# VeeraKarthick609/ImageCaptioner

Hardware: NVIDIA B200
Metric: kd_train_samples_per_sec (higher is better)
Workload: dtype bf16

## Files before the change

### imagecaptioner_b200/csrc/api.cu

```cuda
#include <stdlib.h>
#include "gemm.cuh"
#include "loss_kernels.cuh"
#include "decoder_kernels.cuh"
#include "recurrent.cuh"
#include "recur_cluster.cuh"
#include "refine_kernels.cuh"
#include "mha_mma.cuh"
#include "optim_kernels.cuh"

using namespace b2c;

namespace {

constexpr int MAXL = B2C_MAX_LAYERS;
constexpr int COLSUM_RS = 160;

int check_device() {
  static int cached = 1;
  if (cached <= 0) return cached;
  int dev = 0;
  B2C_CUDA(cudaGetDevice(&dev));
  int major = 0;
  B2C_CUDA(cudaDeviceGetAttribute(&major, cudaDevAttrComputeCapabilityMajor, dev));
  if (major != 10) { cached = B2C_EARCH; return set_err(B2C_EARCH, "b2c kernels are built for sm_100a only; device has compute capability major %d", major); }
// ... 184 lines not shown
    const int gx = cdiv(cols, 256);
    int rs = (int)((rows + 31) / 32); if (rs > 592 / gx) rs = 592 / gx; if (rs > COLSUM_RS) rs = COLSUM_RS; if (rs < 1) rs = 1;
    colsum_vec_kernel<T, false><<<dim3(gx, rs), 256, 0, st>>>(const_cast<T*>(A), (const T*)nullptr, rows, cols, 1.f, partial);
    B2C_LAUNCH_CHECK("colsum_vec_kernel");
    colsum_final_kernel<<<cdiv(cols, 256), 256, 0, st>>>(partial, rs, cols, out, out2, unperm_h);
    B2C_LAUNCH_CHECK("colsum_final_kernel");
    return 0;
  }
  int rs = (int)((rows + 255) / 256); if (rs > COLSUM_RS) rs = COLSUM_RS; if (rs < 1) rs = 1;
  colsum_partial_kernel<T><<<dim3(cdiv(cols, 32), rs), 256, 0, st>>>(A, rows, cols, ld, partial);
  B2C_LAUNCH_CHECK("colsum_partial_kernel");
  colsum_final_kernel<<<cdiv(cols, 256), 256, 0, st>>>(partial, rs, cols, out, out2, unperm_h);
  B2C_LAUNCH_CHECK("colsum_final_kernel");
  return 0;
}

template <typename K> int set_smem(K kern, size_t bytes) {
  B2C_CHECK_ARG(bytes <= 227 * 1024, "kernel needs %zu bytes of shared memory (> 227 KB): shape too large for this path", bytes);
  if (bytes > 48 * 1024) B2C_CUDA(cudaFuncSetAttribute(kern, cudaFuncAttributeMaxDynamicSharedMemorySize, (int)bytes));
  return 0;
}

template <typename T>
int attn_fwd(cudaStream_t st, const B2CShape& s, const float* P, const T* F, const float* u, T* ctx, long ldctx, float* attw,
             long ldu = 0, float* u_save = nullptr) {
  if (ldu == 0) ldu = s.E;
  const size_t smem = (size_t)s.S * s.E * sizeof(T) + (size_t)(s.E + s.S) * 4;
  const int nq = s.S <= ATT_MAXTOK * (ATT_THREADS / 32) ? cdiv(s.E / 4, 32) : 4;
#define B2C_ATT_(NQ, KA) do { B2C_TRY(set_smem(attn_step_fwd_kernel<T, NQ, KA>, smem)); \
    B2C_CUDA(launch_pdl(attn_step_fwd_kernel<T, NQ, KA>, dim3(s.B), dim3(ATT_THREADS), smem, st, P, F, u, ldu, s.S, s.E, ctx, ldctx, attw, u_save)); } while (0)
  if (nq == 1) B2C_ATT_(1, 4); else if (nq == 2) B2C_ATT_(2, 4); else if (nq == 3) B2C_ATT_(3, ATT_MAXTOK); else B2C_ATT_(0, ATT_MAXTOK);
#undef B2C_ATT_
  B2C_LAUNCH_CHECK("attn_step_fwd_kernel");
  return 0;
}

template <typename T>
int attn_bwd(cudaStream_t st, int B, int S, int E, const float* P, const T* F, const float* u, const float* attw, const float* dctx, long lddctx,
             float* ds, T* du) {
  const size_t smem = (size_t)S * E * sizeof(T) + (size_t)(E + 2 * S) * 4;
  constexpr int PB = 13;
#define B2C_ATTB(PB, SMALL) do { B2C_TRY(set_smem(attn_step_bwd_kernel<T, PB, SMALL>, smem)); \
    B2C_CUDA(launch_pdl(attn_step_bwd_kernel<T, PB, SMALL>, dim3(B), dim3(ATT_THREADS), smem, st, P, F, u, (long)E, attw, dctx, lddctx, S, E, ds, du, (long)E)); } while (0)
  if (E <= 256) B2C_ATTB(PB, true); else B2C_ATTB(PB, false);
#undef B2C_ATTB
  B2C_LAUNCH_CHECK("attn_step_bwd_kernel");
  return 0;
}

template <typename T>
int lstm_layer_fwd(cudaStream_t st, const B2CShape& s, const Weights<T>& w, int k, const T* xh_t, const T* addend,
                   const float* c_prev, float* c_out, T* gates_out, T* h_rec, T* h_next, T* h_top,
                   const B2CDropout& dr, long row_base, const float* rec32 = nullptr, long ld_rec32 = 0) {
  const int in = in_dim(s, k), ld = in + s.H;
  LstmEpi le{};
  le.addend32 = rec32; le.ld_addend32 = ld_rec32;
  le.enabled = 1; le.H = s.H; le.addend = addend; le.bias = (k == 0) ? nullptr : w.bcat[k];
  le.c_prev = c_prev; le.c_out = c_out; le.gates_out = gates_out;
  le.h_rec = h_rec; le.ld_rec = ld; le.h_next = h_next; le.ld_next = 2 * s.H; le.h_top = h_top; le.ld_top = s.H;
  le.drop_p = dr.p; le.seed = dr.seed; le.site = (unsigned)k; le.row_base = row_base; le.seed_dev = (const unsigned long long*)dr.seed_dev;
  return gemm_lstm<T>(st, s.B, s.H, rec32 ? in : ld, xh_t, ld, w.Wcat[k], ld, le);
}

constexpr int MAX_SUB = 5;
struct SubStreams { cudaStream_t s[MAX_SUB]; cudaEvent_t fork; cudaEvent_t join[MAX_SUB]; cudaEvent_t ev[4]; };
constexpr int MAX_DEVICES = 64;
int get_substreams(SubStreams** out) {
  static SubStreams all[MAX_DEVICES]; static bool all_ready[MAX_DEVICES] = {false};
  int dev = 0;
  B2C_CUDA(cudaGetDevice(&dev));
  B2C_CHECK_ARG(dev >= 0 && dev < MAX_DEVICES, "device index %d outside [0,%d)", dev, MAX_DEVICES);
  SubStreams& ss = all[dev]; bool& ready = all_ready[dev];
  if (!ready) {
    for (int i = 0; i < MAX_SUB; ++i) {
      B2C_CUDA(cudaStreamCreateWithFlags(&ss.s[i], cudaStreamNonBlocking));
      B2C_CUDA(cudaEventCreateWithFlags(&ss.join[i], cudaEventDisableTiming));
    }
    B2C_CUDA(cudaEventCreateWithFlags(&ss.fork, cudaEventDisableTiming));
    for (int i = 0; i < 4; ++i) B2C_CUDA(cudaEventCreateWithFlags(&ss.ev[i], cudaEventDisableTiming));
    ready = true;
  }
  *out = &ss;
  return 0;
}
inline int pick_sub_batches(int B) {
  static int want = -1;
  if (want < 0) { const char* e = getenv("B2C_SUB_BATCHES"); want = e ? atoi(e) : 1; if (want != 2 && want != 4) want = 1; }
  if (want > 1 && B >= 32 * want && B % want == 0) return want;
  return 1;
}
struct SubPlan { int ns; cudaStream_t st[MAX_SUB]; int b0[MAX_SUB]; int bn[MAX_SUB]; SubStreams* ss; cudaStream_t main; };
int fork_subs(SubPlan& sp, int B, cudaStream_t st) {
  sp.ns = pick_sub_batches(B); sp.main = st; sp.ss = nullptr;
  if (sp.ns == 1) { sp.st[0] = st; sp.b0[0] = 0; sp.bn[0] = B; return 0; }
  B2C_TRY(get_substreams(&sp.ss));
  B2C_CUDA(cudaEventRecord(sp.ss->fork, st));
  for (int i = 0; i < sp.ns; ++i) {
    sp.st[i] = sp.ss->s[i]; sp.bn[i] = B / sp.ns; sp.b0[i] = i * sp.bn[i];
    B2C_CUDA(cudaStreamWaitEvent(sp.st[i], sp.ss->fork, 0));
  }
  return 0;
}
int join_subs(SubPlan& sp) {
  if (sp.ns == 1) return 0;
  for (int i = 0; i < sp.ns; ++i) {
    B2C_CUDA(cudaEventRecord(sp.ss->join[i], sp.st[i]));
    B2C_CUDA(cudaStreamWaitEvent(sp.main, sp.ss->join[i], 0));
  }
  return 0;
}

struct RecurTrace { unsigned long long* dev; size_t n; int grid, T; };
inline RecurTrace& recur_trace_state() { static RecurTrace t{nullptr, 0, 0, 0}; return t; }
inline unsigned long long* recur_trace_buffer(size_t n) {
  static const bool on = getenv("B2C_RECUR_TRACE") != nullptr;
  if (!on) return nullptr;
  RecurTrace& t = recur_trace_state();
  if (t.n < n) { if (t.dev) cudaFree(t.dev); t.dev = nullptr; if (cudaMalloc(&t.dev, n * 8) != cudaSuccess) { t.n = 0; return nullptr; } t.n = n; }
  return t.dev;
}

template <typename T> int recur_forward(cudaStream_t, const B2CShape&, const RecurPlan&, const TrainWs<T>&, const T*, T*, float*, const B2CDropout&) {
  return set_err(B2C_EINVAL, "the persistent recurrence kernel is bf16 only");
}
template <>
int recur_forward<bf16>(cudaStream_t st, const B2CShape& s, const RecurPlan& pl, const TrainWs<bf16>& W, const bf16* feats, bf16* hid_top, float* attw,
                        const B2CDropout& dr) {
  RecurMaps maps; RecurParams p{};
  p.B = s.B; p.T = s.T; p.S = s.S; p.E = s.E; p.H = s.H; p.L = s.L;
  p.tiles_m = pl.tiles_m; p.tiles_n = pl.tiles_n; p.u_tiles_n = pl.u_tiles_n; p.n_fbuf = pl.n_fbuf; p.f_resident = pl.f_resident; p.tmem_cols = pl.tmem_cols;
  p.P = W.P; p.EP = W.EP; p.F = feats; p.u = W.u; p.attw = attw; p.G0 = W.G0; p.hid_top = hid_top;
  p.trace = recur_trace_buffer((size_t)pl.grid * s.T * 16);
  for (int k = 0; k < s.L; ++k) {
    const int in = in_dim(s, k), ld = in + s.H;
    p.xh[k] = W.xh[k]; p.ld[k] = ld; p.in[k] = in; p.bias[k] = (k == 0) ? nullptr : W.w.bcat[k]; p.c[k] = W.c[k]; p.gates[k] = W.gates[k];
    B2C_TRY(make_tmap_bf16_3d(&maps.a[k], W.xh[k], ld, s.B, s.T + 1, ld, TC_BM));
    B2C_TRY(make_tmap_bf16(&maps.w[k], W.w.Wcat[k], ld, 4 * s.H, ld, RC_BN));
  }
  for (int k = s.L; k < RC_MAXL; ++k) { maps.a[k] = maps.a[0]; maps.w[k] = maps.w[0]; }
  B2C_TRY(make_tmap_bf16(&maps.wh, W.w.Wh, s.H, s.E, s.H, RC_BNU));
  p.drop_p = dr.p; p.seed = dr.seed; p.seed_dev = (const unsigned long long*)dr.seed_dev;
  { const char* e = getenv("B2C_RECUR_EARLY"); p.early = (e && e[0] == '0') ? 0 : 1; }
  { const char* e = getenv("B2C_RECUR_EPNC"); p.ep_nc = (e && e[0] == '1') ? 1 : 0; }
  p.barrier = W.sync; p.flags = W.sync + 128;
  B2C_CHECK_ARG(pl.grid <= 160, "unexpected grid %d", pl.grid);
  B2C_CUDA(cudaMemsetAsync(W.sync, 0, (128 + 160 * 32) * sizeof(unsigned int), st));
  void (*kern)(const RecurMaps, const RecurParams) = pl.nq == 1 ? recur_fwd_kernel<1> : (pl.nq == 2 ? recur_fwd_kernel<2> : recur_fwd_kernel<3>);
  B2C_CUDA(cudaFuncSetAttribute(kern, cudaFuncAttributeMaxDynamicSharedMemorySize, (int)pl.smem));
  cudaLaunchConfig_t cfg{};
  cfg.gridDim = dim3(pl.grid); cfg.blockDim = dim3(RC_THREADS); cfg.dynamicSmemBytes = pl.smem; cfg.stream = st;
  cudaLaunchAttribute attr[1];
  attr[0].id = cudaLaunchAttributeCooperative; attr[0].val.cooperative = 1;
  cfg.attrs = attr; cfg.numAttrs = 1;
  B2C_CUDA(cudaLaunchKernelEx(&cfg, kern, maps, p));
  B2C_LAUNCH_CHECK("recur_fwd_kernel");
  recur_trace_state().grid = pl.grid; recur_trace_state().T = s.T;
  return 0;
}

template <typename T> int cluster_forward(cudaStream_t, const B2CShape&, int, const TrainWs<T>&, const T*, T*, float*) {
  return set_err(B2C_EINVAL, "the cluster recurrence kernel is bf16 only");
}
template <>
int cluster_forward<bf16>(cudaStream_t st, const B2CShape& s, int ncl, const TrainWs<bf16>& W, const bf16* feats, bf16* hid_top, float* attw) {
  ClusterMaps maps; ClusterParams p{};
  p.B = s.B; p.T = s.T; p.S = s.S; p.ncl = ncl;
  p.P = W.P; p.EP = W.EP; p.F = feats; p.u = W.u; p.attw = attw; p.xh0 = W.xh[0]; p.xh1 = W.xh[1];
  p.G0T = W.G0T; p.bias1 = W.w.bcat[1]; p.c0 = W.c[0]; p.c1 = W.c[1]; p.gates0 = W.gates[0]; p.gates1 = W.gates[1]; p.hid_top = hid_top;
  p.trace = recur_trace_buffer((size_t)ncl * CR_CL * s.T * 8);
  const long rows = (long)(s.T + 1) * s.B;
  B2C_TRY(make_tmap_bf16(&maps.w0, W.w.Wcat[0], CR_E + CR_H, 4 * CR_H, CR_E + CR_H, 128));
  B2C_TRY(make_tmap_bf16(&maps.w1, W.w.Wcat[1], 2 * CR_H, 4 * CR_H, 2 * CR_H, 128));
  B2C_TRY(make_tmap_bf16(&maps.wh, W.w.Wh, CR_H, CR_E, CR_H, CR_UCOLS));
  B2C_TRY(make_tmap_bf16(&maps.h0, W.xh[0], CR_E + CR_H, rows, CR_E + CR_H, CR_RMAX));
  B2C_TRY(make_tmap_bf16(&maps.h1, W.xh[1], 2 * CR_H, rows, 2 * CR_H, CR_RMAX));
  B2C_TRY(make_tmap_bf16(&maps.ctx, W.xh[0], CR_E + CR_H, rows, CR_E + CR_H, CR_SPC));
  B2C_CUDA(cudaFuncSetAttribute(recur_cluster_fwd_kernel, cudaFuncAttributeMaxDynamicSharedMemorySize, CR_SMEM_BYTES));
  cudaLaunchConfig_t cfg{};
  cfg.gridDim = dim3(ncl * CR_CL); cfg.blockDim = dim3(CR_THREADS); cfg.dynamicSmemBytes = CR_SMEM_BYTES; cfg.stream = st;
  cudaLaunchAttribute attr[1];
  attr[0].id = cudaLaunchAttributeClusterDimension; attr[0].val.clusterDim.x = CR_CL; attr[0].val.clusterDim.y = 1; attr[0].val.clusterDim.z = 1;
  cfg.attrs = attr; cfg.numAttrs = 1;
  B2C_CUDA(cudaLaunchKernelEx(&cfg, recur_cluster_fwd_kernel, maps, p));
  B2C_LAUNCH_CHECK("recur_cluster_fwd_kernel");
  recur_trace_state().grid = ncl * CR_CL; recur_trace_state().T = s.T;
  return 0;
}

template <typename T>
int decoder_prepare_impl(const B2CShape& s, const B2CParams& p, const int64_t* cap, void* ws, size_t ws_bytes, cudaStream_t st) {
  TrainWs<T> W; W.carve(ws, s);
  B2C_CHECK_ARG(ws_bytes >= W.bytes, "workspace too small: %zu < %zu", ws_bytes, W.bytes);
  const int B = s.B, Tn = s.T, E = s.E, H = s.H, L = s.L, V = s.V;
  const long TB = (long)Tn * B;
  B2C_TRY(pack_params<T>(s, p, W.w, st));
  embedding_gather_kernel<T><<<ew_grid(TB * E / 4), 256, 0, st>>>(p.embedding, cap, TB, E, V, W.emb, E);
  B2C_LAUNCH_CHECK("embedding_gather_kernel");
  for (int k = 0; k < L; ++k) {
    B2C_CUDA(cudaMemsetAsync(W.xh[k], 0, (size_t)B * (in_dim(s, k) + H) * sizeof(T), st));
    B2C_CUDA(cudaMemsetAsync(W.c[k], 0, (size_t)B * H * sizeof(float), st));
  }
  B2C_TRY((gemm<T, T>(st, (int)TB, 4 * H, E, W.emb, E, 0, W.w.We, E, 0, W.G0, 4 * H, 0.f, W.w.bx)));
  if constexpr (sizeof(T) == 2) {
    if (const int ncl = cluster_plan(s)) {
      g0_cluster_layout_kernel<<<dim3(4 * H / 64, ncl, Tn), 256, 0, st>>>(reinterpret_cast<const bf16*>(W.G0), B, Tn, ncl, reinterpret_cast<bf16*>(W.G0T));
      B2C_LAUNCH_CHECK("g0_cluster_layout_kernel");
    }
  }
  return 0;
}

template <typename T>
int set_initial_state_impl(const B2CShape& s, const float* h0, const float* c0, void* ws, size_t ws_bytes, cudaStream_t st) {
  TrainWs<T> W; W.carve(ws, s);
  B2C_CHECK_ARG(ws_bytes >= W.bytes, "workspace too small: %zu < %zu", ws_bytes, W.bytes);
  for (int k = 0; k < s.L; ++k) {
    const int in = in_dim(s, k);
    initial_state_kernel<T><<<ew_grid((long)s.B * s.H), 256, 0, st>>>(h0 + (size_t)k * s.B * s.H, c0 + (size_t)k * s.B * s.H, s.B, s.H,
                                                                     W.xh[k] + in, in + s.H, W.c[k]);
    B2C_LAUNCH_CHECK("initial_state_kernel");
  }
  return 0;
}

struct EvalOut { const float* teacher; const int64_t* targets; float temperature; float* row_kl; float* row_ce; int* argmax; };

template <typename T>
int decoder_forward_impl(const B2CShape& s, const B2CParams& p, const T* feats, const int64_t* cap, T* logits, T* hid_top,
                         float* attw, void* ws, size_t ws_bytes, const B2CDropout& dr, cudaStream_t st, bool prepared,
                         const EvalOut* ev = nullptr) {
  TrainWs<T> W; W.carve(ws, s);
  B2C_CHECK_ARG(ws_bytes >= W.bytes, "workspace too small: %zu < %zu", ws_bytes, W.bytes);
  const int B = s.B, Tn = s.T, S = s.S, E = s.E, H = s.H, L = s.L, V = s.V;
  const long TB = (long)Tn * B;
  if (!prepared) B2C_TRY(decoder_prepare_impl<T>(s, p, cap, ws, ws_bytes, st));
  B2C_TRY((gemm<T, float>(st, B * S, E, E, feats, E, 0, W.w.Wf, E, 0, W.P, E, 0.f, p.attn_b)));
  const int inL = in_dim(s, L - 1), ldL = inL + H;
  SubPlan sp;
  B2C_TRY(fork_subs(sp, B, st));
  pdl_full_dependency_next();
  static const bool merge_rec = []() { const char* e = getenv("B2C_MERGE_REC"); return !(e && e[0] == '0'); }();
  RecurPlan rplan{}; rplan.ok = false;
  int ncl = 0;
  if (sizeof(T) == 2 && sp.ns == 1 && !(dr.p > 0.f)) ncl = cluster_plan(s);
  if (ncl > 0) { B2C_TRY(cluster_forward<T>(st, s, ncl, W, feats, hid_top, attw)); rplan.ok = true; }
  else {
  if (sizeof(T) == 2 && sp.ns == 1) rplan = recur_plan(s);
  if (rplan.ok) B2C_TRY(recur_forward<T>(st, s, rplan, W, feats, hid_top, attw, dr));
  }
  for (int t = 0; t < (rplan.ok ? 0 : Tn); ++t) {
    for (int i = 0; i < sp.ns; ++i) {
      cudaStream_t ss = sp.st[i];
      const long b0 = sp.b0[i];
      B2CShape sh = s; sh.B = sp.bn[i];
      const long row = (long)t * B + b0;
      const T* q = W.xh[L - 1] + row * ldL + inL;
      float* u_t = W.u + row * E;
      const bool merged = merge_rec && sizeof(T) == 2;
      const long ldur = E + 4 * H;
      float* ur = W.UR + b0 * ldur;
      if (merged) {
        B2C_TRY((gemm<T, float>(ss, sh.B, E + 4 * H, H, q, ldL, 0, W.w.Wuh, H, 0, ur, ldur)));
        B2C_TRY(attn_fwd<T>(ss, sh, W.P + b0 * S * E, feats + b0 * S * E, ur, W.xh[0] + row * (E + H), E + H, attw + row * S, ldur, u_t));
      } else {
        B2C_TRY((gemm<T, float>(ss, sh.B, E, H, q, ldL, 0, W.w.Wh, H, 0, u_t, E)));
        B2C_TRY(attn_fwd<T>(ss, sh, W.P + b0 * S * E, feats + b0 * S * E, u_t, W.xh[0] + row * (E + H), E + H, attw + row * S));
      }
      for (int k = 0; k < L; ++k) {
        const int in = in_dim(s, k), ld = in + H;
        const bool rec = merged && k == L - 1;
        B2C_TRY(lstm_layer_fwd<T>(ss, sh, W.w, k, W.xh[k] + row * ld, k == 0 ? W.G0 + row * 4 * H : (const T*)nullptr,
                                  W.c[k] + row * H, W.c[k] + (row + B) * H,
                                  W.gates[k] + row * 4 * H, W.xh[k] + (row + B) * ld + in,
                                  k + 1 < L ? W.xh[k + 1] + row * 2 * H : nullptr, k == L - 1 ? hid_top + row * H : nullptr,
                                  dr, row, rec ? ur + E : nullptr, ldur));
      }
    }
  }
  B2C_TRY(join_subs(sp));
  B2C_TRY((gemm<T, T>(st, (int)TB, E, H, hid_top, H, 0, W.w.W1, H, 0, W.o1, E, 0.f, p.out0_b, 1)));
  if (dr.p > 0.f) {
    dropout_inplace_kernel<T><<<ew_grid(TB * E), 256, 0, st>>>(W.o1, TB * E, dr.p, dr.seed, 100u, (const unsigned long long*)dr.seed_dev);
    B2C_LAUNCH_CHECK("dropout_inplace_kernel");
  }
  if (ev) {
    GemmArgs gv{(int)TB, V, E, 1.f, 0.f, W.o1, (long)E, 0, W.w.W2, (long)E, 0, nullptr, (long)V, p.out3_b, 0};
    B2C_CHECK_ARG(sizeof(T) == 2 && tc_eligible(gv), "the logits-free validation forward needs bf16 mode and a TMA-describable vocabulary head");
    EvalEpi ee{ev->teacher, ev->targets, W.evalp, 1.0f / ev->temperature, 0, 0};
    gv.eval = &ee;
    B2C_TRY((Gemm<T, float>::run(gv, st)));
    kd_eval_combine_kernel<<<cdiv(TB, 8), 256, 0, st>>>(W.evalp, ee.nparts, TB, V, ev->targets, 1.0f / ev->temperature, ev->row_kl, ev->row_ce, ev->argmax);
    B2C_LAUNCH_CHECK("kd_eval_combine_kernel");
    return 0;
  }
  B2C_TRY((gemm<T, T>(st, (int)TB, V, E, W.o1, E, 0, W.w.W2, E, 0, logits, V, 0.f, p.out3_b)));
  return 0;
}



inline int bg_ctas() { static int v = -1; if (v < 0) { const char* e = getenv("B2C_BG_CTAS"); v = e ? atoi(e) : 10; } return v; }
inline bool attn_post_occ3() { static int v = -1; if (v < 0) { const char* e = getenv("B2C_POST_OCC3"); v = (e && e[0] == '0') ? 0 : 1; } return v != 0; }
inline int wgrad_chunks() { static int v = -1; if (v < 0) { const char* e = getenv("B2C_WGRAD_CHUNKS"); v = e ? atoi(e) : 0; } return v; }

template <typename T>
int decoder_backward_impl(const B2CShape& s, const B2CParams& p, const T* feats, const int64_t* cap, const T* hid_top,
                          const float* attw, const T* dlogits, const T* dhid, const B2CGrads& g, float* dfeats,
                          void* ws, size_t ws_bytes, const B2CDropout& dr, cudaStream_t st, int flags) {
  TrainWs<T> W; W.carve(ws, s);
  B2C_CHECK_ARG(ws_bytes >= W.bytes, "workspace too small: %zu < %zu", ws_bytes, W.bytes);
  B2C_CHECK_ARG(g.embedding && g.attn_w && g.attn_b && g.comb_w && g.comb_b && g.out0_w && g.out0_b && g.out3_w && g.out3_b && dfeats, "NULL gradient pointer");
  const int B = s.B, Tn = s.T, S = s.S, E = s.E, H = s.H, L = s.L, V = s.V;
  const long TB = (long)Tn * B;
  const float inv_keep = dr.p > 0.f ? 1.0f / (1.0f - dr.p) : 1.0f;
  SubStreams* hs = nullptr;
  B2C_TRY(get_substreams(&hs));
  cudaStream_t side = hs->s[MAX_SUB - 1];
  for (int k = 0; k < L; ++k) B2C_CHECK_ARG(g.w_ih[k] && g.w_hh[k] && g.b_ih[k] && g.b_hh[k], "NULL LSTM gradient pointer (layer %d)", k);
  B2C_CUDA(cudaEventRecord(hs->ev[3], st));
  B2C_CUDA(cudaStreamWaitEvent(side, hs->ev[3], 0));
  B2C_CUDA(cudaMemsetAsync(W.dxh0, 0, (size_t)TB * (E + H) * sizeof(float), side));
  for (int k = 1; k < L; ++k) B2C_CUDA(cudaMemsetAsync(W.dxh[k], 0, (size_t)TB * 2 * H * sizeof(float), side));
  B2C_CUDA(cudaEventRecord(hs->ev[3], side));
  B2C_TRY((gemm<T, T>(st, (int)TB, E, V, dlogits, V, 0, W.w.W2, E, 1, W.do1, E)));
  relu_bwd_inplace_kernel<T><<<ew_grid(TB * E), 256, 0, st>>>(W.do1, W.o1, TB * E, inv_keep);
  B2C_LAUNCH_CHECK("relu_bwd_inplace_kernel");
  B2C_CUDA(cudaEventRecord(hs->fork, st));
  B2C_CUDA(cudaStreamWaitEvent(side, hs->fork, 0));
  {
    GemmCapScope bg(bg_ctas());
    B2C_TRY((gemm<T, float>(side, V, E, (int)TB, dlogits, V, 1, W.o1, E, 1, g.out3_w, E)));
    B2C_TRY(colsum<T>(side, dlogits, TB, V, V, W.partial_side, g.out3_b));
    B2C_TRY((gemm<T, float>(side, E, H, (int)TB, W.do1, E, 1, hid_top, H, 1, g.out0_w, H)));
    B2C_TRY(colsum<T>(side, W.do1, TB, E, E, W.partial_side, g.out0_b));
  }
  B2C_CUDA(cudaEventRecord(hs->join[MAX_SUB - 1], side));
  B2C_TRY((gemm<T, float>(st, (int)TB, H, E, W.do1, E, 0, W.w.W1, H, 1, W.dHext, H)));
  B2C_CUDA(cudaStreamWaitEvent(st, hs->ev[3], 0));
  SubPlan sp;
  B2C_TRY(fork_subs(sp, B, st));
  auto weight_grads = [&](cudaStream_t s2, long r0, long r1, float beta) -> int {
    const int K = (int)(r1 - r0);
    for (int k = 1; k < L; ++k) {
      const int in = in_dim(s, k), ld = in + H;
      B2C_TRY((gemm<T, float>(s2, 4 * H, in, K, W.dgates[k] + r0 * 4 * H, 4 * H, 1, W.xh[k] + r0 * ld, ld, 1, g.w_ih[k], in, beta, nullptr, 0, 1.f, H)));
      B2C_TRY((gemm<T, float>(s2, 4 * H, H, K, W.dgates[k] + r0 * 4 * H, 4 * H, 1, W.xh[k] + r0 * ld + in, ld, 1, g.w_hh[k], H, beta, nullptr, 0, 1.f, H)));
    }
    B2C_TRY((gemm<T, float>(s2, 4 * H, E, K, W.dgates[0] + r0 * 4 * H, 4 * H, 1, W.xh[0] + r0 * (E + H), E + H, 1, W.dWx32, E, beta)));
    B2C_TRY((gemm<T, float>(s2, 4 * H, E, K, W.dgates[0] + r0 * 4 * H, 4 * H, 1, W.emb + r0 * E, E, 1, W.dWe32, E, beta)));
    B2C_TRY((gemm<T, float>(s2, 4 * H, H, K, W.dgates[0] + r0 * 4 * H, 4 * H, 1, W.xh[0] + r0 * (E + H) + E, E + H, 1, g.w_hh[0], H, beta, nullptr, 0, 1.f, H)));
    return 0;
  };
  const int n_chunks = (sp.ns == 1 && bg_ctas() > 0) ? wgrad_chunks() : 0;
  const int chunk_steps = n_chunks > 0 ? cdiv(Tn, n_chunks) : 0;
  long wg_done_from = TB;
  bool wg_any = false;
  pdl_full_dependency_next();
  for (int t = Tn - 1; t >= 0; --t) {
    const bool last = (t == Tn - 1);
    for (int i = 0; i < sp.ns; ++i) {
      cudaStream_t ss = sp.st[i];
      const long b0 = sp.b0[i];
      const int Bh = sp.bn[i];
      const long row = (long)t * B + b0;
      for (int k = L - 1; k >= 0; --k) {
        const int in = in_dim(s, k), ld = in + H;
        const float* carry = last ? nullptr : (k == 0 ? W.dxh0 + (row + B) * (E + H) + E : W.dxh[k] + (row + B) * 2 * H + H);
        const float* above = (k < L - 1) ? W.dxh[k + 1] + row * 2 * H : nullptr;
        const bool top = (k == L - 1);
        B2C_CUDA(launch_pdl(lstm_pointwise_bwd_kernel<T>, dim3(ew_grid((long)Bh * H)), dim3(256), 0, ss,
            (const T*)(W.gates[k] + row * 4 * H), (const float*)(W.c[k] + row * H), (const float*)(W.c[k] + (row + B) * H), W.dc[k] + b0 * H, last ? 1 : 0,
            carry, (long)ld, above, (long)(2 * H), (const float*)(top ? W.dHext + row * H : nullptr), (const T*)((top && dhid) ? dhid + row * H : nullptr),
            (const T*)((top && !last) ? W.dq + b0 * H : nullptr), (long)H, W.dgates[k] + row * 4 * H, Bh, H, dr.p, dr.seed, (uint32_t)k, row, (const unsigned long long*)dr.seed_dev));
        B2C_LAUNCH_CHECK("lstm_pointwise_bwd_kernel");
        float* out = (k == 0) ? W.dxh0 + row * (E + H) : W.dxh[k] + row * 2 * H;
        B2C_TRY((gemm<T, float>(ss, Bh, ld, 4 * H, W.dgates[k] + row * 4 * H, 4 * H, 0, W.w.Wcat[k], ld, 1, out, ld, 1.f)));
      }
      const float* dctx_t = W.dxh0 + row * (E + H);
      T* du_t = W.du + row * E;
      B2C_TRY(attn_bwd<T>(ss, Bh, S, E, W.P + b0 * S * E, feats + b0 * S * E, W.u + row * E, attw + row * S, dctx_t, (long)(E + H), W.ds + row * S, du_t));
      if (t > 0) B2C_TRY((gemm<T, T>(ss, Bh, H, E, du_t, E, 0, W.w.Wh, H, 1, W.dq + b0 * H, H)));
    }
    if (chunk_steps > 0 && t > 0 && (Tn - t) % chunk_steps == 0 && t >= chunk_steps) {
      B2C_CUDA(cudaEventRecord(hs->ev[0], st));
      B2C_CUDA(cudaStreamWaitEvent(side, hs->ev[0], 0));
      GemmCapScope bg(bg_ctas());
      B2C_TRY(weight_grads(side, (long)t * B, wg_done_from, wg_any ? 1.f : 0.f));
      wg_done_from = (long)t * B; wg_any = true;
    }
  }
  B2C_TRY(join_subs(sp));
  B2C_CUDA(cudaEventRecord(hs->ev[1], st));
  B2C_CUDA(cudaStreamWaitEvent(side, hs->ev[1], 0));
  B2C_TRY(weight_grads(side, 0, wg_done_from, wg_any ? 1.f : 0.f));
  for (int k = 0; k < L; ++k) B2C_TRY(colsum<T>(side, W.dgates[k], TB, 4 * H, 4 * H, W.partial_side, g.b_ih[k], g.b_hh[k], H));
  {
    cast_f32_kernel<T><<<ew_grid((long)4 * H * E / 8), 256, 0, side>>>(W.dWx32, W.dWxT, (long)4 * H * E);
    B2C_LAUNCH_CHECK("cast_f32_kernel");
    cast_f32_kernel<T><<<ew_grid((long)4 * H * E / 8), 256, 0, side>>>(W.dWe32, W.dWeT, (long)4 * H * E);
    B2C_LAUNCH_CHECK("cast_f32_kernel");
    B2C_TRY((gemm<T, float>(side, 4 * H, E, E, W.dWxT, E, 0, W.w.Wcc, E, 0, g.w_ih[0], E, 0.f, nullptr, 0, 1.f, H)));
    B2C_TRY((gemm<T, float>(side, 4 * H, E, E, W.dWeT, E, 0, W.w.Wce, E, 0, g.w_ih[0], E, 1.f, nullptr, 0, 1.f, H)));
    rank1_add_kernel<<<ew_grid((long)4 * H * E), 256, 0, side>>>(g.w_ih[0], g.b_ih[0], p.comb_b, (long)4 * H, E);
    B2C_LAUNCH_CHECK("rank1_add_kernel");
    B2C_TRY((gemm<T, float>(side, E, E, 4 * H, W.w.Wih0, E, 1, W.dWeT, E, 1, g.comb_w, 2 * E)));
    B2C_TRY((gemm<T, float>(side, E, E, 4 * H, W.w.Wih0, E, 1, W.dWxT, E, 1, g.comb_w + E, 2 * E)));
    B2C_CUDA(cudaMemsetAsync(g.comb_b, 0, (size_t)E * sizeof(float), side));
    bias_fold_bwd_kernel<<<dim3(cdiv(E, 32), 32), 256, 0, side>>>(p.w_ih[0], g.b_ih[0], 4 * H, E, g.comb_b);
    B2C_LAUNCH_CHECK("bias_fold_bwd_kernel");
    B2C_TRY((gemm<T, float>(side, (int)TB, E, 4 * H, W.dgates[0], 4 * H, 0, W.w.We, E, 1, W.demb, E)));
    B2C_CUDA(cudaMemsetAsync(g.embedding, 0, (size_t)V * E * sizeof(float), side));
    embedding_scatter_add_kernel<<<ew_grid(TB * E), 256, 0, side>>>(W.demb, cap, TB, E, V, g.embedding);
    B2C_LAUNCH_CHECK("embedding_scatter_add_kernel");
  }
  const int inL = in_dim(s, L - 1), ldL = inL + H;
  B2C_TRY((gemm<T, float>(side, E, H, (int)TB, W.du, E, 1, W.xh[L - 1] + inL, ldL, 1, g.attn_w, H + E)));
  if (Tn <= 24) {
    const int splits = 1, per = cdiv(S, splits), TP = (Tn + 3) & ~3;
    const size_t psmem = (size_t)2 * per * TP * 4;
    if (Tn <= 20 && attn_post_occ3()) {
      B2C_TRY(set_smem(attn_post_reg_kernel<T, 20>, psmem));
      attn_post_reg_kernel<T, 20><<<dim3(B, splits), ATT_THREADS, psmem, st>>>(W.P, W.u, W.dxh0, (long)(E + H), attw, W.ds, Tn, B, S, E, W.dP, dfeats);
    } else {
      B2C_TRY(set_smem(attn_post_reg_kernel<T, 24>, psmem));
      attn_post_reg_kernel<T, 24><<<dim3(B, splits), ATT_THREADS, psmem, st>>>(W.P, W.u, W.dxh0, (long)(E + H), attw, W.ds, Tn, B, S, E, W.dP, dfeats);
    }
    B2C_LAUNCH_CHECK("attn_post_reg_kernel");
  } else {
    const size_t smem = (size_t)Tn * (2 * E + 2 * S) * 4;
    B2C_TRY(set_smem(attn_post_kernel<T>, smem));
    attn_post_kernel<T><<<B, ATT_THREADS, smem, st>>>(W.P, W.u, W.dxh0, (long)(E + H), attw, W.ds, Tn, B, S, E, W.dP, dfeats);
    B2C_LAUNCH_CHECK("attn_post_kernel");
  }
  B2C_CUDA(cudaEventRecord(hs->ev[2], st));
  B2C_TRY((gemm<T, float>(st, B * S, E, E, W.dP, E, 0, W.w.Wf, E, 1, dfeats, E, 1.f)));
  B2C_CUDA(cudaStreamWaitEvent(side, hs->ev[2], 0));
  B2C_TRY((gemm<T, float>(side, E, E, B * S, W.dP, E, 1, feats, E, 1, g.attn_w + H, H + E)));
  B2C_TRY(colsum<T>(side, W.dP, (long)B * S, E, E, W.partial_side, g.attn_b));
  B2C_CUDA(cudaEventRecord(hs->join[MAX_SUB - 1], side));
  if (flags & B2C_BWD_DEFER_JOIN) return 0;
  B2C_CUDA(cudaStreamWaitEvent(st, hs->join[MAX_SUB - 1], 0));
  return 0;
}


inline bool fuse_argmax_off() { static const bool off = getenv("B2C_DECODE_LOGITS") != nullptr; return off; }

template <typename T>
int greedy_decode_impl(const B2CShape& s, const B2CParams& p, const T* feats, int64_t start_id, int64_t end_id,
                       int64_t* tokens, int32_t* lengths, void* ws, size_t ws_bytes, cudaStream_t st) {
  DecodeWs<T> W; W.carve(ws, s);
  B2C_CHECK_ARG(ws_bytes >= W.bytes, "workspace too small: %zu < %zu", ws_bytes, W.bytes);
  const int B = s.B, Tn = s.T, S = s.S, E = s.E, H = s.H, L = s.L, V = s.V;
  const B2CDropout nodrop{0.f, 0, nullptr};
  B2C_TRY(pack_params<T>(s, p, W.w, st));
  B2C_TRY((gemm<T, float>(st, B * S, E, E, feats, E, 0, W.w.Wf, E, 0, W.P, E, 0.f, p.attn_b)));
  for (int k = 0; k < L; ++k) {
    B2C_CUDA(cudaMemsetAsync(W.xh[k], 0, (size_t)2 * B * (in_dim(s, k) + H) * sizeof(T), st));
    B2C_CUDA(cudaMemsetAsync(W.c[k], 0, (size_t)B * H * sizeof(float), st));
  }
  fill_i64_kernel<<<ew_grid(B), 256, 0, st>>>(W.cur, B, start_id);
  B2C_LAUNCH_CHECK("fill_i64_kernel");
  const int inL = in_dim(s, L - 1), ldL = inL + H;
  for (int t = 0; t < Tn; ++t) {
    const int pcur = t & 1, pnxt = pcur ^ 1;
    auto slot = [&](int k, int which) { return W.xh[k] + (size_t)which * B * (in_dim(s, k) + H); };
    embedding_gather_kernel<T><<<ew_grid((long)B * E / 4), 256, 0, st>>>(p.embedding, W.cur, B, E, V, W.emb, E);
    B2C_LAUNCH_CHECK("embedding_gather_kernel");
    B2C_TRY((gemm<T, T>(st, B, 4 * H, E, W.emb, E, 0, W.w.We, E, 0, W.G0, 4 * H, 0.f, W.w.bx)));
    B2C_TRY((gemm<T, float>(st, B, E, H, slot(L - 1, pcur) + inL, ldL, 0, W.w.Wh, H, 0, W.u, E)));
    B2C_TRY(attn_fwd<T>(st, s, W.P, feats, W.u, slot(0, pcur), E + H, nullptr));
    for (int k = 0; k < L; ++k) {
      const int in = in_dim(s, k);
      B2C_TRY(lstm_layer_fwd<T>(st, s, W.w, k, slot(k, pcur), k == 0 ? W.G0 : (const T*)nullptr, W.c[k], W.c[k], (T*)nullptr, slot(k, pnxt) + in,
                                k + 1 < L ? slot(k + 1, pcur) : nullptr, (T*)nullptr, nodrop, 0));
    }
    B2C_TRY((gemm<T, T>(st, B, E, H, slot(L - 1, pnxt) + inL, ldL, 0, W.w.W1, H, 0, W.o1, E, 0.f, p.out0_b, 1)));
    GemmArgs gv{B, V, E, 1.f, 0.f, W.o1, (long)E, 0, W.w.W2, (long)E, 0, W.logits, (long)V, p.out3_b, 0};
    if (sizeof(T) == 2 && tc_eligible(gv) && !fuse_argmax_off()) {
      ArgmaxEpi ae{W.amax_v, W.amax_i, 0, 0};
      gv.amax = &ae;
      B2C_TRY((Gemm<T, float>::run(gv, st)));
      argmax_parts_feedback_kernel<<<cdiv(B, 8), 256, 0, st>>>(W.amax_v, W.amax_i, ae.nparts, B, end_id, t, W.cur, tokens + (long)t * B, lengths, W.done);
      B2C_LAUNCH_CHECK("argmax_parts_feedback_kernel");
    } else {
      B2C_TRY((Gemm<T, float>::run(gv, st)));
      argmax_feedback_kernel<<<B, 256, 0, st>>>(W.logits, V, V, end_id, t, W.cur, tokens + (long)t * B, lengths, W.done);
      B2C_LAUNCH_CHECK("argmax_feedback_kernel");
    }
  }
  finish_lengths_kernel<<<cdiv(B, 256), 256, 0, st>>>(lengths, B, Tn);
  B2C_LAUNCH_CHECK("finish_lengths_kernel");
  return 0;
}


template <typename T> struct AttnWs {
  T *Wh, *Wf; float *P, *u; size_t bytes;
  void carve(void* base, const B2CShape& s) {
    Carver c{reinterpret_cast<unsigned char*>(base), 0};
    Wh = c.take<T>((size_t)s.E * s.H); Wf = c.take<T>((size_t)s.E * s.E);
    P = c.take<float>((size_t)s.B * s.S * s.E); u = c.take<float>((size_t)s.B * s.E);
    bytes = align_up(c.off, 256);
  }
};

template <typename T>
int attention_step_impl(const B2CShape& s, const float* attn_w, const float* attn_b, const T* hidden, const T* feats,
                        T* context, float* weights, void* ws, size_t ws_bytes, cudaStream_t st) {
  AttnWs<T> W; W.carve(ws, s);
  B2C_CHECK_ARG(ws_bytes >= W.bytes, "workspace too small: %zu < %zu", ws_bytes, W.bytes);
  const int B = s.B, S = s.S, E = s.E, H = s.H;
  PackTable tab; tab.n = 2;
  tab.seg[0] = PackSeg{attn_w, W.Wh, nullptr, E, H, (long)H + E, (long)H, 0};
  tab.seg[1] = PackSeg{attn_w + H, W.Wf, nullptr, E, E, (long)H + E, (long)E, 0};
  pack_params_kernel<T><<<dim3(32, 2), 256, 0, st>>>(tab);
  B2C_LAUNCH_CHECK("pack_params_kernel");
  B2C_TRY((gemm<T, float>(st, B * S, E, E, feats, E, 0, W.Wf, E, 0, W.P, E, 0.f, attn_b)));
  pdl_full_dependency_next();
  B2C_TRY((gemm<T, float>(st, B, E, H, hidden, H, 0, W.Wh, H, 0, W.u, E)));
  return attn_fwd<T>(st, s, W.P, feats, W.u, context, (long)s.E, weights);
}

constexpr int LN_GRID = 148 * 3;
template <typename T> struct RefineWs {
  T *Win, *Wo, *W1, *W2;
  T *x, *qkv, *probs, *attn, *proj, *x1, *f1, *f2;
  float *mean1, *rstd1, *mean2, *rstd2;
  T *dz2, *df1, *dz1, *dattn, *dqkv; float *dz1f, *lnpart, *partial;
  float *x1f, *dz2f;
  size_t bytes;
  void carve(void* base, const B2CShape& s) {
    Carver c{reinterpret_cast<unsigned char*>(base), 0};
    const size_t R = (size_t)s.B * s.S, E = s.E, heads = s.H;
    Win = c.take<T>(3 * E * E); Wo = c.take<T>(E * E); W1 = c.take<T>(2 * E * E); W2 = c.take<T>(2 * E * E);
    x = c.take<T>(R * E); qkv = c.take<T>(R * 3 * E); probs = c.take<T>((size_t)s.B * heads * s.S * (s.S > 64 ? s.S : 64)) ; attn = c.take<T>(R * E);
    proj = c.take<T>(R * E); x1 = c.take<T>(R * E); f1 = c.take<T>(R * 2 * E); f2 = c.take<T>(R * E);
    mean1 = c.take<float>(R); rstd1 = c.take<float>(R); mean2 = c.take<float>(R); rstd2 = c.take<float>(R);
    dz2 = c.take<T>(R * E); df1 = c.take<T>(R * 2 * E); dz1 = c.take<T>(R * E); dattn = c.take<T>(R * E); dqkv = c.take<T>(R * 3 * E);
    dz1f = c.take<float>(R * E); lnpart = c.take<float>((size_t)LN_GRID * 3 * E); partial = c.take<float>((size_t)COLSUM_RS * 3 * E);
    x1f = c.take<float>(R * E); dz2f = c.take<float>(R * E);
    bytes = align_up(c.off, 256);
  }
};

int check_refine_shape(const B2CShape* s) {
  B2C_CHECK_ARG(s != nullptr, "shape is NULL");
  B2C_CHECK_ARG(s->B > 0 && s->S > 0 && s->E > 0 && s->H > 0, "bad refinement shape B=%d S=%d E=%d heads=%d", s->B, s->S, s->E, s->H);
  B2C_CHECK_ARG(s->E % 8 == 0 && s->E <= 256 * LN_MAXC && s->E % s->H == 0, "E=%d must be a multiple of 8 and of heads=%d, and <= %d", s->E, s->H, 256 * LN_MAXC);
  const size_t hd = s->E / s->H;
  B2C_CHECK_ARG(hd % 4 == 0, "head_dim=%zu must be a multiple of 4", hd);
  B2C_CHECK_ARG((4 * (size_t)s->S * mha_pitch((int)hd) + 3 * (size_t)s->S * mha_pitch(s->S)) * 4 <= 200 * 1024, "S=%d x head_dim=%zu does not fit the attention core's shared memory", s->S, hd);
  return 0;
}

template <typename TX, typename TR, typename TY>
int ln_fwd(cudaStream_t st, const TX* x, const TR* res, const float* g, const float* b, TY* y, float* y32, float* mean, float* rstd, long R, int E) {
  long grid = (R + 7) / 8; if (grid > 148 * 8) grid = 148 * 8;
  if (E <= 256) ln_fwd_kernel<TX, TR, TY, 1><<<(unsigned)grid, LN_THREADS, 0, st>>>(x, res, g, b, y, y32, mean, rstd, R, E, 1e-5f);
  else ln_fwd_kernel<TX, TR, TY, 2><<<(unsigned)grid, LN_THREADS, 0, st>>>(x, res, g, b, y, y32, mean, rstd, R, E, 1e-5f);
  B2C_LAUNCH_CHECK("ln_fwd_kernel");
  return 0;
}
template <typename TX, typename TR, typename TDY, typename TDZ>
int ln_bwd(cudaStream_t st, const TDY* dy, const float* dpool, int L, int O, const TX* x, const TR* res, const float* mean, const float* rstd,
           const float* gamma, TDZ* dz, float* dz32, float* part, float* dgamma, float* dbeta, float* dbias_prev, long R, int E) {
  long grid = (R + 7) / 8; if (grid > LN_GRID) grid = LN_GRID;
  const size_t smem = (size_t)(LN_THREADS / 32) * 3 * E * 4;
#define B2C_LNB(POOLED, NC) do { B2C_TRY(set_smem(ln_bwd_kernel<TX, TR, TDY, TDZ, POOLED, NC>, smem)); \
    ln_bwd_kernel<TX, TR, TDY, TDZ, POOLED, NC><<<(unsigned)grid, LN_THREADS, smem, st>>>(dy, dpool, L, O, x, res, mean, rstd, gamma, dz, dz32, part, R, E); } while (0)
  if (dpool) { if (E <= 256) B2C_LNB(true, 1); else B2C_LNB(true, 2); }
  else { if (E <= 256) B2C_LNB(false, 1); else B2C_LNB(false, 2); }
#undef B2C_LNB
  B2C_LAUNCH_CHECK("ln_bwd_kernel");
  ln_param_grad_kernel<<<dim3(cdiv(E, 32), 3), 256, 0, st>>>(part, (int)grid, E, dgamma, dbeta, dbias_prev);
  B2C_LAUNCH_CHECK("ln_param_grad_kernel");
  return 0;
}

template <typename T>
int colsum_vec(cudaStream_t st, T* A, const T* act, long rows, int cols, float inv_keep, float* partial, float* out) {
  const int gx = cdiv(cols, 256);
  int rs = (int)((rows + 31) / 32); if (rs > 592 / gx) rs = 592 / gx; if (rs > COLSUM_RS) rs = COLSUM_RS; if (rs < 1) rs = 1;
  dim3 grid(gx, rs);
  if (act) colsum_vec_kernel<T, true><<<grid, 256, 0, st>>>(A, act, rows, cols, inv_keep, partial);
  else colsum_vec_kernel<T, false><<<grid, 256, 0, st>>>(A, act, rows, cols, inv_keep, partial);
  B2C_LAUNCH_CHECK("colsum_vec_kernel");
  colsum_final_kernel<<<cdiv(cols, 256), 256, 0, st>>>(partial, rs, cols, out, nullptr);
  B2C_LAUNCH_CHECK("colsum_final_kernel");
  return 0;
}

template <typename T>
int refine_pack(const B2CShape& s, const B2CRefineParams& p, const RefineWs<T>& W, cudaStream_t st) {
  B2C_CHECK_ARG(p.in_w && p.in_b && p.out_w && p.out_b && p.ffn0_w && p.ffn0_b && p.ffn3_w && p.ffn3_b && p.n1_w && p.n1_b && p.n2_w && p.n2_b, "NULL refinement parameter");
  const int E = s.E;
  PackTable tab; tab.n = 4;
  tab.seg[0] = PackSeg{p.in_w, W.Win, nullptr, 3 * E, E, (long)E, (long)E, 0};
  tab.seg[1] = PackSeg{p.out_w, W.Wo, nullptr, E, E, (long)E, (long)E, 0};
  tab.seg[2] = PackSeg{p.ffn0_w, W.W1, nullptr, 2 * E, E, (long)E, (long)E, 0};
  tab.seg[3] = PackSeg{p.ffn3_w, W.W2, nullptr, E, 2 * E, (long)2 * E, (long)2 * E, 0};
  pack_params_kernel<T><<<dim3(48, 4), 256, 0, st>>>(tab);
  B2C_LAUNCH_CHECK("pack_params_kernel");
  return 0;
}

template <typename T> inline bool mha_use_mma(int S, int hd) { return false; }
template <> inline bool mha_use_mma<bf16>(int S, int hd) {
  static const bool off = getenv("B2C_MHA_FFMA") != nullptr;
  return !off && hd == 64 && S <= 64;
}

template <typename T>
int refinement_forward_impl(const B2CShape& s, const B2CRefineParams& p, const float* x, float* out, void* ws, size_t ws_bytes,
                            const B2CDropout& dr, cudaStream_t st, T* out_compute = nullptr) {
  RefineWs<T> W; W.carve(ws, s);
  B2C_CHECK_ARG(ws_bytes >= W.bytes, "workspace too small: %zu < %zu", ws_bytes, W.bytes);
  const int B = s.B, S = s.S, E = s.E, heads = s.H, hd = E / heads;
  const long R = (long)B * S;
  B2C_TRY(refine_pack<T>(s, p, W, st));
  cast_f32_kernel<T><<<ew_grid(R * E / 4), 256, 0, st>>>(x, W.x, R * E);
  B2C_LAUNCH_CHECK("cast_f32_kernel");
  B2C_TRY((gemm<T, T>(st, (int)R, 3 * E, E, W.x, E, 0, W.Win, E, 0, W.qkv, 3 * E, 0.f, p.in_b)));
  if (mha_use_mma<T>(S, hd)) {
    mha_fwd_mma_kernel<<<dim3(B, heads), MM_THREADS, 0, st>>>((const bf16*)W.qkv, (bf16*)W.attn, (bf16*)W.probs, S, E, heads, 1.0f / sqrtf((float)hd),
                                                             dr.p, dr.seed, MHA_DROP_SITE, (const unsigned long long*)dr.seed_dev);
    B2C_LAUNCH_CHECK("mha_fwd_mma_kernel");
  } else {
    const size_t smem = ((size_t)3 * S * mha_pitch(hd) + (size_t)S * mha_pitch(S)) * 4;
    B2C_TRY(set_smem(mha_fwd_kernel<T>, smem));
    mha_fwd_kernel<T><<<dim3(B, heads), MHA_THREADS, smem, st>>>(W.qkv, W.attn, W.probs, S, E, heads, 1.0f / sqrtf((float)hd), dr.p, dr.seed, (const unsigned long long*)dr.seed_dev);
    B2C_LAUNCH_CHECK("mha_fwd_kernel");
  }
  B2C_TRY((gemm<T, T>(st, (int)R, E, E, W.attn, E, 0, W.Wo, E, 0, W.proj, E, 0.f, p.out_b)));
  B2C_TRY((ln_fwd<float, T, T>(st, x, W.proj, p.n1_w, p.n1_b, W.x1, W.x1f, W.mean1, W.rstd1, R, E)));
  B2C_TRY((gemm<T, T>(st, (int)R, 2 * E, E, W.x1, E, 0, W.W1, E, 0, W.f1, 2 * E, 0.f, p.ffn0_b, 1)));
  if (dr.p > 0.f) {
    dropout_inplace_kernel<T><<<ew_grid(R * 2 * E), 256, 0, st>>>(W.f1, R * 2 * E, dr.p, dr.seed, 201u, (const unsigned long long*)dr.seed_dev);
    B2C_LAUNCH_CHECK("dropout_inplace_kernel");
  }
  B2C_TRY((gemm<T, T>(st, (int)R, E, 2 * E, W.f1, 2 * E, 0, W.W2, 2 * E, 0, W.f2, E, 0.f, p.ffn3_b)));
  if (out_compute) B2C_TRY((ln_fwd<float, T, T>(st, W.x1f, W.f2, p.n2_w, p.n2_b, out_compute, out, W.mean2, W.rstd2, R, E)));
  else B2C_TRY((ln_fwd<float, T, float>(st, W.x1f, W.f2, p.n2_w, p.n2_b, (float*)nullptr, out, W.mean2, W.rstd2, R, E)));
  return 0;
}

template <typename T>
int refinement_backward_impl(const B2CShape& s, const B2CRefineParams& p, const float* x, const float* dout, const B2CRefineGrads& g, float* dx,
                             void* ws, size_t ws_bytes, const B2CDropout& dr, cudaStream_t st) {
  RefineWs<T> W; W.carve(ws, s);
  B2C_CHECK_ARG(ws_bytes >= W.bytes, "workspace too small: %zu < %zu", ws_bytes, W.bytes);
  B2C_CHECK_ARG(g.in_w && g.in_b && g.out_w && g.out_b && g.ffn0_w && g.ffn0_b && g.ffn3_w && g.ffn3_b && g.n1_w && g.n1_b && g.n2_w && g.n2_b && dx, "NULL refinement gradient");
  const int B = s.B, S = s.S, E = s.E, heads = s.H, hd = E / heads;
  const long R = (long)B * S;
  const float inv_keep = dr.p > 0.f ? 1.0f / (1.0f - dr.p) : 1.0f;
  B2C_TRY((ln_bwd<float, T, float, T>(st, dout, nullptr, 0, 0, W.x1f, W.f2, W.mean2, W.rstd2, p.n2_w, W.dz2, W.dz2f, W.lnpart, g.n2_w, g.n2_b, g.ffn3_b, R, E)));
  B2C_TRY((gemm<T, float>(st, E, 2 * E, (int)R, W.dz2, E, 1, W.f1, 2 * E, 1, g.ffn3_w, 2 * E)));
  B2C_TRY((gemm<T, T>(st, (int)R, 2 * E, E, W.dz2, E, 0, W.W2, 2 * E, 1, W.df1, 2 * E)));
  B2C_TRY(colsum_vec<T>(st, W.df1, W.f1, R, 2 * E, inv_keep, W.partial, g.ffn0_b));
  B2C_TRY((gemm<T, float>(st, 2 * E, E, (int)R, W.df1, 2 * E, 1, W.x1, E, 1, g.ffn0_w, E)));
  B2C_TRY((gemm<T, float>(st, (int)R, E, 2 * E, W.df1, 2 * E, 0, W.W1, E, 1, W.dz2f, E, 1.f)));
  B2C_TRY((ln_bwd<float, T, float, T>(st, W.dz2f, nullptr, 0, 0, x, W.proj, W.mean1, W.rstd1, p.n1_w, W.dz1, W.dz1f, W.lnpart, g.n1_w, g.n1_b, g.out_b, R, E)));
  B2C_TRY((gemm<T, float>(st, E, E, (int)R, W.dz1, E, 1, W.attn, E, 1, g.out_w, E)));
  B2C_TRY((gemm<T, T>(st, (int)R, E, E, W.dz1, E, 0, W.Wo, E, 1, W.dattn, E)));
  if (mha_use_mma<T>(S, hd)) {
    const size_t smem = (size_t)(dr.p > 0.f ? 7 : 6) * MM_TILE * sizeof(bf16);
    B2C_TRY(set_smem(mha_bwd_mma_kernel, smem));
    mha_bwd_mma_kernel<<<dim3(B, heads), MM_THREADS, smem, st>>>((const bf16*)W.qkv, (const bf16*)W.probs, (const bf16*)W.dattn, (bf16*)W.dqkv, S, E, heads,
                                                                1.0f / sqrtf((float)hd), dr.p, dr.seed, MHA_DROP_SITE, (const unsigned long long*)dr.seed_dev);
    B2C_LAUNCH_CHECK("mha_bwd_mma_kernel");
  } else {
    const size_t smem = ((size_t)4 * S * mha_pitch(hd) + (size_t)(dr.p > 0.f ? 3 : 2) * S * mha_pitch(S)) * 4;
    B2C_TRY(set_smem(mha_bwd_kernel<T>, smem));
    mha_bwd_kernel<T><<<dim3(B, heads), MHA_THREADS, smem, st>>>(W.qkv, W.probs, W.dattn, W.dqkv, S, E, heads, 1.0f / sqrtf((float)hd), dr.p, dr.seed, (const unsigned long long*)dr.seed_dev);
    B2C_LAUNCH_CHECK("mha_bwd_kernel");
  }
  B2C_TRY((gemm<T, float>(st, 3 * E, E, (int)R, W.dqkv, 3 * E, 1, W.x, E, 1, g.in_w, E)));
  B2C_TRY(colsum_vec<T>(st, W.dqkv, (const T*)nullptr, R, 3 * E, 1.f, W.partial, g.in_b));
  B2C_CUDA(cudaMemcpyAsync(dx, W.dz1f, (size_t)R * E * sizeof(float), cudaMemcpyDeviceToDevice, st));
  B2C_TRY((gemm<T, float>(st, (int)R, E, 3 * E, W.dqkv, 3 * E, 0, W.Win, E, 1, dx, E, 1.f)));
  return 0;
}

template <typename T> struct ProjWs {
// ... 479 lines not shown
```

### imagecaptioner_b200/csrc/common.cuh

```cuda
#pragma once
#include <cuda_runtime.h>
#include <cuda_bf16.h>
#include <cuda.h>
#include <stdint.h>
#include <stdio.h>
#include <string.h>
#include <math.h>
#include <stdarg.h>
#include <stdlib.h>

#include "../../include/b2c.h"

namespace b2c {

typedef __nv_bfloat16 bf16;

inline char* err_buf() { static thread_local char buf[512] = {0}; return buf; }
inline int set_err(int code, const char* fmt, ...) {
  va_list ap; va_start(ap, fmt); vsnprintf(err_buf(), 512, fmt, ap); va_end(ap); return code;
}
#define B2C_CHECK_ARG(cond, ...) do { if (!(cond)) return b2c::set_err(B2C_EINVAL, __VA_ARGS__); } while (0)
#define B2C_CUDA(expr) do { cudaError_t e_ = (expr); if (e_ != cudaSuccess) \
    return b2c::set_err(B2C_ECUDA, "%s failed: %s (%s:%d)", #expr, cudaGetErrorString(e_), __FILE__, __LINE__); } while (0)
inline unsigned long long& launch_counter() { static unsigned long long n = 0; return n; }
#define B2C_LAUNCH_CHECK(name) do { ++b2c::launch_counter(); cudaError_t e_ = cudaGetLastError(); if (e_ != cudaSuccess) \
    return b2c::set_err(B2C_ECUDA, "launch of %s failed: %s (%s:%d)", name, cudaGetErrorString(e_), __FILE__, __LINE__); } while (0)
#define B2C_TRY(expr) do { int r_ = (expr); if (r_ != 0) return r_; } while (0)

template <typename T> __device__ __forceinline__ float to_f(T v);
template <> __device__ __forceinline__ float to_f<float>(float v) { return v; }
template <> __device__ __forceinline__ float to_f<bf16>(bf16 v) { return __bfloat162float(v); }
template <typename T> __device__ __forceinline__ T from_f(float v);
template <> __device__ __forceinline__ float from_f<float>(float v) { return v; }
template <> __device__ __forceinline__ bf16 from_f<bf16>(float v) { return __float2bfloat16_rn(v); }

template <typename T> struct Math;
template <> struct Math<float> {
  static __device__ __forceinline__ float tanh_(float x) { return tanhf(x); }
  static __device__ __forceinline__ float sigmoid_(float x) { return 1.0f / (1.0f + expf(-x)); }
  static __device__ __forceinline__ float exp_(float x) { return expf(x); }
  static __device__ __forceinline__ float log_(float x) { return logf(x); }
  static __device__ __forceinline__ float dtanh_(float x) { const float t = tanhf(x); return fmaf(-t, t, 1.0f); }
};
__device__ __forceinline__ float ex2_ftz_(float x) { float y; asm("ex2.approx.ftz.f32 %0, %1;" : "=f"(y) : "f"(x)); return y; }
__device__ __forceinline__ float rcp_ftz_(float x) { float y; asm("rcp.approx.ftz.f32 %0, %1;" : "=f"(y) : "f"(x)); return y; }
template <> struct Math<bf16> {
  static __device__ __forceinline__ float tanh_(float x) { return fmaf(-2.0f, rcp_ftz_(1.0f + ex2_ftz_(2.8853900817779268f * x)), 1.0f); }
  static __device__ __forceinline__ float sigmoid_(float x) { return rcp_ftz_(1.0f + ex2_ftz_(-1.4426950408889634f * x)); }
  static __device__ __forceinline__ float exp_(float x) { return ex2_ftz_(1.4426950408889634f * x); }
  static __device__ __forceinline__ float log_(float x) { return __logf(x); }
  static __device__ __forceinline__ float dtanh_(float x) { float t; asm("tanh.approx.f32 %0, %1;" : "=f"(t) : "f"(x)); return fmaf(-t, t, 1.0f); }
};

__device__ __forceinline__ float ex2_ftz(float x) { float y; asm("ex2.approx.ftz.f32 %0, %1;" : "=f"(y) : "f"(x)); return y; }

__device__ __forceinline__ float warp_sum(float v) {
#pragma unroll
  for (int o = 16; o > 0; o >>= 1) v += __shfl_xor_sync(0xffffffffu, v, o);
  return v;
}
__device__ __forceinline__ float warp_max(float v) {
#pragma unroll
  for (int o = 16; o > 0; o >>= 1) v = fmaxf(v, __shfl_xor_sync(0xffffffffu, v, o));
  return v;
}

__device__ __forceinline__ uint32_t mix32(uint64_t seed, uint32_t stream, uint64_t idx) {
  uint64_t z = seed + 0x9E3779B97F4A7C15ull * (idx + 1) + ((uint64_t)stream << 40);
  z = (z ^ (z >> 30)) * 0xBF58476D1CE4E5B9ull;
  z = (z ^ (z >> 27)) * 0x94D049BB133111EBull;
  z = z ^ (z >> 31);
  return (uint32_t)(z >> 32);
}
__device__ __forceinline__ uint64_t drop_seed(uint64_t seed, const unsigned long long* seed_dev) {
  return seed_dev ? seed + 0xD6E8FEB86659FD93ull * __ldg(seed_dev) : seed;
}
__device__ __forceinline__ float dropout_scale(uint64_t seed, uint32_t stream, uint64_t idx, float p, float inv_keep) {
  const uint32_t thr = (uint32_t)(p * 4294967296.0f);
  return mix32(seed, stream, idx) >= thr ? inv_keep : 0.0f;
}

__device__ __forceinline__ void pdl_launch_dependents() { asm volatile("griddepcontrol.launch_dependents;" ::: "memory"); }
__device__ __forceinline__ void pdl_wait() { asm volatile("griddepcontrol.wait;" ::: "memory"); }

inline bool pdl_enabled() {
  static int on = -1;
  if (on < 0) { const char* e = getenv("B2C_PDL"); on = (e && e[0] == '0') ? 0 : 1; }
  return on != 0;
}
inline bool& pdl_full_dependency_flag() { static thread_local bool f = false; return f; }
inline void pdl_full_dependency_next() { pdl_full_dependency_flag() = true; }
template <typename... KArgs, typename... Args>
inline cudaError_t launch_pdl(void (*kern)(KArgs...), dim3 grid, dim3 block, size_t smem, cudaStream_t st, Args... args) {
  cudaLaunchConfig_t cfg{};
  cfg.gridDim = grid; cfg.blockDim = block; cfg.dynamicSmemBytes = smem; cfg.stream = st;
  cudaLaunchAttribute attr[1];
  attr[0].id = cudaLaunchAttributeProgrammaticStreamSerialization;
  attr[0].val.programmaticStreamSerializationAllowed = 1;
  cfg.attrs = attr; cfg.numAttrs = (pdl_enabled() && !pdl_full_dependency_flag()) ? 1 : 0;
  pdl_full_dependency_flag() = false;
  return cudaLaunchKernelEx(&cfg, kern, static_cast<KArgs>(args)...);
}

__device__ __forceinline__ uint32_t smem_u32(const void* p) { return (uint32_t)__cvta_generic_to_shared(p); }

__device__ __forceinline__ void mbar_init(uint64_t* bar, uint32_t count) {
  asm volatile("mbarrier.init.shared::cta.b64 [%0], %1;" :: "r"(smem_u32(bar)), "r"(count) : "memory");
}
__device__ __forceinline__ void fence_barrier_init() {
  asm volatile("fence.mbarrier_init.release.cluster;" ::: "memory");
}
__device__ __forceinline__ void fence_proxy_async() {
  asm volatile("fence.proxy.async.shared::cta;" ::: "memory");
}
__device__ __forceinline__ void mbar_arrive_expect_tx(uint64_t* bar, uint32_t bytes) {
  asm volatile("mbarrier.arrive.expect_tx.shared::cta.b64 _, [%0], %1;" :: "r"(smem_u32(bar)), "r"(bytes) : "memory");
}
__device__ __forceinline__ void mbar_arrive(uint64_t* bar) {
  asm volatile("mbarrier.arrive.shared::cta.b64 _, [%0];" :: "r"(smem_u32(bar)) : "memory");
}
__device__ __forceinline__ bool mbar_try_wait(uint64_t* bar, uint32_t parity) {
  uint32_t ok;
  asm volatile(
      "{\n\t.reg .pred p;\n\t"
      "mbarrier.try_wait.parity.shared::cta.b64 p, [%1], %2;\n\t"
      "selp.u32 %0, 1, 0, p;\n\t}"
      : "=r"(ok) : "r"(smem_u32(bar)), "r"(parity) : "memory");
  return ok != 0;
}
__device__ __forceinline__ void mbar_wait(uint64_t* bar, uint32_t parity) {
  for (uint32_t spins = 0; !mbar_try_wait(bar, parity); ++spins) {
    if (spins > (1u << 24)) { printf("b2c: mbarrier wait timed out (block %d,%d thread %d)\n", blockIdx.x, blockIdx.y, threadIdx.x); __trap(); }
  }
}
__device__ __forceinline__ void bulk_g2s(void* smem_dst, const void* gsrc, uint32_t bytes, uint64_t* bar) {
  asm volatile("cp.async.bulk.shared::cluster.global.mbarrier::complete_tx::bytes [%0], [%1], %2, [%3];"
               :: "r"(smem_u32(smem_dst)), "l"(gsrc), "r"(bytes), "r"(smem_u32(bar)) : "memory");
}

__device__ __forceinline__ uint4 ld_nc_v4(const void* p) {
  uint4 r;
  asm volatile("ld.global.nc.L1::no_allocate.v4.u32 {%0,%1,%2,%3}, [%4];" : "=r"(r.x), "=r"(r.y), "=r"(r.z), "=r"(r.w) : "l"(p));
  return r;
}
__device__ __forceinline__ void st_na_v4(void* p, const uint4& v) {
  asm volatile("st.global.L1::no_allocate.v4.u32 [%0], {%1,%2,%3,%4};" :: "l"(p), "r"(v.x), "r"(v.y), "r"(v.z), "r"(v.w) : "memory");
}

__device__ __forceinline__ float bf16_lo(uint32_t u) { return __uint_as_float(u << 16); }
__device__ __forceinline__ float bf16_hi(uint32_t u) { return __uint_as_float(u & 0xffff0000u); }
__device__ __forceinline__ uint32_t pack_bf16(float a, float b) {
  __nv_bfloat162 v = __floats2bfloat162_rn(a, b);
  return *reinterpret_cast<uint32_t*>(&v);
}

template <typename T> struct Vec8;
template <> struct Vec8<bf16> {
  static __device__ __forceinline__ void load(const bf16* p, float (&v)[8]) {
    const uint4 a = *reinterpret_cast<const uint4*>(p);
    v[0] = bf16_lo(a.x); v[1] = bf16_hi(a.x); v[2] = bf16_lo(a.y); v[3] = bf16_hi(a.y);
    v[4] = bf16_lo(a.z); v[5] = bf16_hi(a.z); v[6] = bf16_lo(a.w); v[7] = bf16_hi(a.w);
  }
  static __device__ __forceinline__ void store(bf16* p, const float (&v)[8]) {
    *reinterpret_cast<uint4*>(p) = make_uint4(pack_bf16(v[0], v[1]), pack_bf16(v[2], v[3]), pack_bf16(v[4], v[5]), pack_bf16(v[6], v[7]));
  }
};
template <> struct Vec8<float> {
  static __device__ __forceinline__ void load(const float* p, float (&v)[8]) {
    const float4 a = *reinterpret_cast<const float4*>(p), b = *reinterpret_cast<const float4*>(p + 4);
    v[0] = a.x; v[1] = a.y; v[2] = a.z; v[3] = a.w; v[4] = b.x; v[5] = b.y; v[6] = b.z; v[7] = b.w;
  }
  static __device__ __forceinline__ void store(float* p, const float (&v)[8]) {
    *reinterpret_cast<float4*>(p) = make_float4(v[0], v[1], v[2], v[3]);
    *reinterpret_cast<float4*>(p + 4) = make_float4(v[4], v[5], v[6], v[7]);
  }
};


inline int cdiv(long a, long b) { return (int)((a + b - 1) / b); }
__host__ __device__ inline size_t align_up(size_t x, size_t a) { return (x + a - 1) / a * a; }

}
```

### imagecaptioner_b200/csrc/decoder_kernels.cuh

```cuda
#pragma once
#include "common.cuh"

namespace b2c {

__device__ __forceinline__ void divmod_idx(long i, int d, long& q, int& r) {
  if (i < 0x7fffffffL) { const unsigned qi = (unsigned)i / (unsigned)d; q = (long)qi; r = (int)((unsigned)i - qi * (unsigned)d); }
  else { q = i / d; r = (int)(i - q * d); }
}
struct PackSeg {
  const float* src; void* dst;
  const float* src2;
  int rows, cols; long lds, ldd;
  int as_float;
  int perm_h;
};
constexpr int PACK_MAX_SEGS = 20;
struct PackTable { PackSeg seg[PACK_MAX_SEGS]; int n; };

template <typename T>
__global__ void __launch_bounds__(256) pack_params_kernel(const __grid_constant__ PackTable tab) {
  const PackSeg& s = tab.seg[blockIdx.y];
  const long total = (long)s.rows * s.cols;
  if (!s.src2 && !s.as_float && (s.cols & 3) == 0 && (s.lds & 3) == 0 && (s.ldd & 3) == 0 && (((uintptr_t)s.src) & 15) == 0 &&
      (((uintptr_t)s.dst) & 15) == 0) {
// ... 105 lines not shown
  for (int e = tid; e < E; e += ATT_THREADS) { const float uv = __ldcg(u + (long)b * ldu + e); us[e] = uv; if (u_save) u_save[(long)b * E + e] = uv; }
  __syncthreads();
  auto score = [&](const float4 (&pv)[NQR], int l) {
    float a = 0.f;
#pragma unroll
    for (int j = 0; j < NQR; ++j) {
      const int q = lane + j * 32;
      if (q < E4) {
        const float4 p = pv[j];
        const float4 uu = *reinterpret_cast<const float4*>(us + q * 4);
        a += Math<T>::tanh_(p.x + uu.x) + Math<T>::tanh_(p.y + uu.y) + Math<T>::tanh_(p.z + uu.z) + Math<T>::tanh_(p.w + uu.w);
      }
    }
    a = warp_sum(a);
    if (lane == 0) sc[l] = a;
  };
  if constexpr (fast) {
    float4 pb[KB][NQR];
    if (KA < ATT_MAXTOK) {
#pragma unroll
      for (int k = 0; k < KB; ++k) {
        const int l = warp + (KA + k) * nwarp;
#pragma unroll
        for (int j = 0; j < NQR; ++j) {
          const int q = lane + j * 32;
          if (l < S && q < E4) pb[k][j] = __ldg(Pb + l * E4 + q);
        }
      }
    }
#pragma unroll
    for (int k = 0; k < KA; ++k) { const int l = warp + k * nwarp; if (l < S) score(pa[k], l); }
    if (KA < ATT_MAXTOK) {
#pragma unroll
      for (int k = 0; k < KB; ++k) { const int l = warp + (KA + k) * nwarp; if (l < S) score(pb[k], l); }
    }
  } else if constexpr (!fast) {
    for (int l = warp; l < S; l += nwarp) {
      float a = 0.f;
      for (int q = lane; q < E4; q += 32) {
        const float4 p = __ldg(Pb + l * E4 + q);
        const float4 uu = *reinterpret_cast<const float4*>(us + q * 4);
        a += Math<T>::tanh_(p.x + uu.x) + Math<T>::tanh_(p.y + uu.y) + Math<T>::tanh_(p.z + uu.z) + Math<T>::tanh_(p.w + uu.w);
      }
      a = warp_sum(a);
      if (lane == 0) sc[l] = a;
    }
  }
  __syncthreads();
  if (warp == 0) {
    float m = -INFINITY;
    for (int l = lane; l < S; l += 32) m = fmaxf(m, sc[l]);
    m = warp_max(m);
    float s = 0.f;
    for (int l = lane; l < S; l += 32) { const float e = Math<T>::exp_(sc[l] - m); sc[l] = e; s += e; }
    s = warp_sum(s);
    const float inv = 1.0f / s;
    for (int l = lane; l < S; l += 32) { const float wv = sc[l] * inv; sc[l] = wv; if (attw) attw[(long)b * S + l] = wv; }
  }
  __syncthreads();
  mbar_wait(&bar, 0);
  for (int e = tid; e < E; e += ATT_THREADS) {
    float a = 0.f;
    for (int l = 0; l < S; ++l) a = fmaf(sc[l], to_f<T>(Fs[l * E + e]), a);
    ctx[(long)b * ldctx + e] = from_f<T>(a);
  }
}

template <typename T, int PB, bool E256 = false>
__global__ void __launch_bounds__(ATT_THREADS, 4)
attn_step_bwd_kernel(const float* __restrict__ P, const T* __restrict__ F, const float* __restrict__ u, long ldu,
                     const float* __restrict__ attw, const float* __restrict__ dctx, long lddctx,
                     int S, int E, float* __restrict__ ds_out, T* __restrict__ du, long lddu) {
  extern __shared__ __align__(128) unsigned char att_smem[];
  const int SE = S * E;
  T* Fs = reinterpret_cast<T*>(att_smem);
  float* dcs = reinterpret_cast<float*>(Fs + SE);
  float* dw = dcs + E;
  float* ws = dw + S;
  __shared__ __align__(8) uint64_t bar;
  const int tid = threadIdx.x, lane = tid & 31, warp = tid >> 5, nwarp = ATT_THREADS / 32;
  const int b = blockIdx.x;
  const float* Pb = P + (long)b * SE;
  pdl_launch_dependents();
  if (tid == 0) { mbar_init(&bar, 1); fence_barrier_init(); }
  for (int l = tid; l < S; l += ATT_THREADS) ws[l] = attw[(long)b * S + l];
  float cur[PB];
  float ue0 = 0.f;
  if (tid < E) {
    ue0 = u[(long)b * ldu + tid];
#pragma unroll
    for (int i = 0; i < PB; ++i) if (i < S) cur[i] = __ldg(Pb + (long)i * E + tid);
  }
  __syncthreads();
  if (tid == 0) {
    const uint32_t fb = (uint32_t)(SE * sizeof(T));
    mbar_arrive_expect_tx(&bar, fb);
    bulk_g2s(Fs, F + (long)b * SE, fb, &bar);
  }
  pdl_wait();
  for (int e = tid; e < E; e += ATT_THREADS) dcs[e] = __ldcg(dctx + (long)b * lddctx + e);
  __syncthreads();
  mbar_wait(&bar, 0);
  if (E256 || E <= 256) {
    float d[8];
    const int c = lane * 8;
    const bool on = c < E;
    if (on) Vec8<float>::load(dcs + c, d);
    for (int l = warp; l < S; l += nwarp) {
      float a = 0.f;
      if (on) {
        float f[8];
        Vec8<T>::load(Fs + l * E + c, f);
#pragma unroll
        for (int i = 0; i < 8; ++i) a = fmaf(d[i], f[i], a);
      }
      a = warp_sum(a);
      if (lane == 0) dw[l] = a;
    }
  } else if constexpr (!E256) {
    for (int l = warp; l < S; l += nwarp) {
      float a = 0.f;
      for (int c = lane * 8; c < E; c += 256) {
        float f[8], d[8];
        Vec8<T>::load(Fs + l * E + c, f);
        Vec8<float>::load(dcs + c, d);
#pragma unroll
        for (int i = 0; i < 8; ++i) a = fmaf(d[i], f[i], a);
      }
      a = warp_sum(a);
      if (lane == 0) dw[l] = a;
    }
  }
  __syncthreads();
  if (warp == 0) {
    float dot = 0.f;
    for (int l = lane; l < S; l += 32) dot = fmaf(ws[l], dw[l], dot);
    dot = warp_sum(dot);
    for (int l = lane; l < S; l += 32) { const float v = ws[l] * (dw[l] - dot); dw[l] = v; ds_out[(long)b * S + l] = v; }
  }
  __syncthreads();
  for (int e = tid; e < E; e += ATT_THREADS) {
    float ue = ue0;
    if (e != tid) {
      ue = u[(long)b * ldu + e];
#pragma unroll
      for (int i = 0; i < PB; ++i) if (i < S) cur[i] = __ldg(Pb + (long)i * E + e);
    }
    float a = 0.f;
    for (int l0 = 0; l0 < S; l0 += PB) {
      float nxt[PB];
      if (l0 + PB < S) {
#pragma unroll
        for (int i = 0; i < PB; ++i) if (l0 + PB + i < S) nxt[i] = __ldg(Pb + (long)(l0 + PB + i) * E + e);
      }
#pragma unroll
      for (int i = 0; i < PB; ++i) {
        if (l0 + i < S) a = fmaf(dw[l0 + i], Math<T>::dtanh_(cur[i] + ue), a);
      }
#pragma unroll
      for (int i = 0; i < PB; ++i) cur[i] = nxt[i];
    }
    du[(long)b * lddu + e] = from_f<T>(a);
  }
}

template <typename T>
__global__ void __launch_bounds__(ATT_THREADS)
attn_post_kernel(const float* __restrict__ P, const float* __restrict__ u , const float* __restrict__ dctx , long lddctx,
                 const float* __restrict__ attw , const float* __restrict__ ds ,
                 int Tn, int B, int S, int E, T* __restrict__ dP, float* __restrict__ dF) {
  extern __shared__ __align__(128) unsigned char att_smem[];
  float* us = reinterpret_cast<float*>(att_smem);
  float* dcs = us + (long)Tn * E;
  float* ws = dcs + (long)Tn * E;
  float* dss = ws + (long)Tn * S;
  const int tid = threadIdx.x, b = blockIdx.x;
  for (int i = tid; i < Tn * E; i += ATT_THREADS) { const int t = i / E, e = i - t * E; us[i] = u[((long)t * B + b) * E + e]; dcs[i] = dctx[((long)t * B + b) * lddctx + e]; }
  for (int i = tid; i < Tn * S; i += ATT_THREADS) { const int t = i / S, l = i - t * S; ws[i] = attw[((long)t * B + b) * S + l]; dss[i] = ds[((long)t * B + b) * S + l]; }
  __syncthreads();
  const long base = (long)b * S * E;
  for (int idx = tid; idx < S * E; idx += ATT_THREADS) {
    const int l = idx / E, e = idx - l * E;
    const float p = P[base + idx];
    float aP = 0.f, aF = 0.f;
    for (int t = 0; t < Tn; ++t) {
      aP = fmaf(dss[t * S + l], Math<T>::dtanh_(p + us[t * E + e]), aP);
      aF = fmaf(ws[t * S + l], dcs[t * E + e], aF);
    }
    dP[base + idx] = from_f<T>(aP);
    dF[base + idx] = aF;
  }
}

template <typename T, int TMAX>
__global__ void __launch_bounds__(ATT_THREADS, TMAX <= 20 ? 4 : 2)
attn_post_reg_kernel(const float* __restrict__ P, const float* __restrict__ u , const float* __restrict__ dctx , long lddctx,
                     const float* __restrict__ attw , const float* __restrict__ ds ,
                     int Tn, int B, int S, int E, T* __restrict__ dP, float* __restrict__ dF) {
  extern __shared__ __align__(128) unsigned char att_smem[];
  const int tid = threadIdx.x, b = blockIdx.x;
  const int per = (S + gridDim.y - 1) / gridDim.y, l0 = blockIdx.y * per, l1 = min(S, l0 + per), nl = l1 - l0;
  if (nl <= 0) return;
  const int TP = (Tn + 3) & ~3;
  float* dsT = reinterpret_cast<float*>(att_smem);
  float* wT = dsT + per * TP;
  for (int i = tid; i < nl * TP; i += ATT_THREADS) {
    const int ll = i / TP, t = i - ll * TP;
    const long g = ((long)t * B + b) * S + l0 + ll;
    dsT[i] = t < Tn ? ds[g] : 0.f;
    wT[i] = t < Tn ? attw[g] : 0.f;
  }
  __syncthreads();
  const long base = (long)b * S * E;
  for (int e = tid; e < E; e += ATT_THREADS) {
    float ur[TMAX], dcr[TMAX];
#pragma unroll
    for (int t = 0; t < TMAX; ++t) {
      ur[t] = t < Tn ? u[((long)t * B + b) * E + e] : 0.f;
      dcr[t] = t < Tn ? dctx[((long)t * B + b) * lddctx + e] : 0.f;
    }
    float p_next = P[base + (long)l0 * E + e];
#pragma unroll 1
    for (int l = l0; l < l1; ++l) {
      const float p = p_next;
      if (l + 1 < l1) p_next = P[base + (long)(l + 1) * E + e];
      const float4* d4p = reinterpret_cast<const float4*>(dsT + (l - l0) * TP);
      const float4* w4p = reinterpret_cast<const float4*>(wT + (l - l0) * TP);
      float aP = 0.f, aF = 0.f;
#pragma unroll
      for (int t4 = 0; t4 < TMAX; t4 += 4) {
        if (t4 < TP) {
          const float4 d4 = d4p[t4 >> 2], w4 = w4p[t4 >> 2];
          const float dd[4] = {d4.x, d4.y, d4.z, d4.w}, ww[4] = {w4.x, w4.y, w4.z, w4.w};
#pragma unroll
          for (int j = 0; j < 4; ++j) {
            aP = fmaf(dd[j], Math<T>::dtanh_(p + ur[t4 + j]), aP);
            aF = fmaf(ww[j], dcr[t4 + j], aF);
          }
        }
      }
      dP[base + (long)l * E + e] = from_f<T>(aP);
      dF[base + (long)l * E + e] = aF;
    }
  }
}

__global__ void __launch_bounds__(256)
bias_fold_kernel(const float* __restrict__ w_ih0, const float* __restrict__ b_c, const float* __restrict__ b_ih, const float* __restrict__ b_hh,
                 int H, int E, float* __restrict__ bx) {
  const int warp = (blockIdx.x * blockDim.x + threadIdx.x) >> 5, lane = threadIdx.x & 31;
  if (warp >= 4 * H) return;
  const int src = (warp & 3) * H + (warp >> 2);
  float a = 0.f;
  for (int e = lane; e < E; e += 32) a = fmaf(w_ih0[(long)src * E + e], b_c[e], a);
  a = warp_sum(a);
  if (lane == 0) bx[warp] = a + b_ih[src] + b_hh[src];
}
__global__ void __launch_bounds__(256)
bias_fold_bwd_kernel(const float* __restrict__ w_ih0, const float* __restrict__ dbx, int H4, int E, float* __restrict__ db_c) {
  __shared__ float red[8][33];
  const int tx = threadIdx.x & 31, ty = threadIdx.x >> 5, e = blockIdx.x * 32 + tx;
  const int per = (H4 + gridDim.y - 1) / gridDim.y, n0 = blockIdx.y * per, n1 = min(H4, n0 + per);
  float a = 0.f;
  if (e < E) for (int n = n0 + ty; n < n1; n += 8) a = fmaf(w_ih0[(long)n * E + e], dbx[n], a);
  red[ty][tx] = a;
  __syncthreads();
  if (ty == 0 && e < E) { float s = 0.f; for (int i = 0; i < 8; ++i) s += red[i][tx]; atomicAdd(db_c + e, s); }
}
__global__ void __launch_bounds__(256)
rank1_add_kernel(float* __restrict__ dW, const float* __restrict__ dbx, const float* __restrict__ b_c, long rows, int E) {
  for (long i = (long)blockIdx.x * blockDim.x + threadIdx.x; i < rows * E; i += (long)gridDim.x * blockDim.x) {
    long n; int e; divmod_idx(i, E, n, e);
    dW[i] = fmaf(dbx[n], b_c[e], dW[i]);
  }
}

template <typename T> struct Gate4;
template <> struct Gate4<bf16> {
  static __device__ __forceinline__ void load(const bf16* p, float (&v)[4]) {
    const uint2 a = *reinterpret_cast<const uint2*>(p);
    v[0] = bf16_lo(a.x); v[1] = bf16_hi(a.x); v[2] = bf16_lo(a.y); v[3] = bf16_hi(a.y);
  }
  static __device__ __forceinline__ void store(bf16* p, const float (&v)[4]) {
    *reinterpret_cast<uint2*>(p) = make_uint2(pack_bf16(v[0], v[1]), pack_bf16(v[2], v[3]));
  }
};
template <> struct Gate4<float> {
  static __device__ __forceinline__ void load(const float* p, float (&v)[4]) {
    const float4 a = *reinterpret_cast<const float4*>(p); v[0] = a.x; v[1] = a.y; v[2] = a.z; v[3] = a.w;
  }
  static __device__ __forceinline__ void store(float* p, const float (&v)[4]) { *reinterpret_cast<float4*>(p) = make_float4(v[0], v[1], v[2], v[3]); }
};

template <typename T>
__global__ void __launch_bounds__(256)
lstm_pointwise_bwd_kernel(const T* __restrict__ gates, const float* __restrict__ c_prev, const float* __restrict__ c_cur,
                          float* __restrict__ dc, int dc_is_zero,
                          const float* __restrict__ dh_carry, long ld_carry, const float* __restrict__ dh_above, long ld_above,
                          const float* __restrict__ dh_ext, const T* __restrict__ dh_hid, const T* __restrict__ dh_q, long ld_q,
                          T* __restrict__ dgates, int B, int H, float drop_p, uint64_t seed, uint32_t site, long row_base,
                          const unsigned long long* __restrict__ seed_dev) {
  pdl_launch_dependents();
  if (drop_p > 0.f) seed = drop_seed(seed, seed_dev);
  const long total = (long)B * H;
  const float inv_keep = drop_p > 0.f ? 1.0f / (1.0f - drop_p) : 1.0f;
  struct Saved { float gt[4]; float tc, cp, dh_fixed, mask; };
  auto load_saved = [&](long idx, Saved& sv) {
    const long b = (long)((unsigned)idx / (unsigned)H); const int j = (int)(idx - b * H);
    Gate4<T>::load(gates + b * 4 * H + 4 * j, sv.gt);
    sv.tc = Math<T>::tanh_(c_cur[idx]);
    sv.cp = c_prev[idx];
    float d = 0.f;
    if (dh_ext) d += dh_ext[idx];
    if (dh_hid) d += to_f<T>(dh_hid[idx]);
    sv.dh_fixed = d;
    sv.mask = (dh_above && drop_p > 0.f) ? dropout_scale(seed, site, (uint64_t)((row_base + b) * H + j), drop_p, inv_keep) : 1.0f;
  };
  const long idx0 = (long)blockIdx.x * blockDim.x + threadIdx.x;
  Saved sv;
  if (idx0 < total) load_saved(idx0, sv);
  pdl_wait();
  for (long idx = idx0; idx < total; idx += (long)gridDim.x * blockDim.x) {
    if (idx != idx0) load_saved(idx, sv);
    const long b = (long)((unsigned)idx / (unsigned)H); const int j = (int)(idx - b * H);
    float dh = sv.dh_fixed;
    if (dh_carry) dh += __ldcg(dh_carry + b * ld_carry + j);
    if (dh_above) dh += __ldcg(dh_above + b * ld_above + j) * sv.mask;
    if (dh_q) dh += to_f<T>(dh_q[b * ld_q + j]);
    const float i = sv.gt[0], f = sv.gt[1], g = sv.gt[2], o = sv.gt[3], tc = sv.tc;
    const float dcc = (dc_is_zero ? 0.f : __ldcg(dc + idx)) + dh * o * (1.0f - tc * tc);
    const float dg[4] = {dcc * g * i * (1.0f - i), dcc * sv.cp * f * (1.0f - f), dcc * i * (1.0f - g * g), dh * tc * o * (1.0f - o)};
    Gate4<T>::store(dgates + b * 4 * H + 4 * j, dg);
    dc[idx] = dcc * f;
  }
}

template <typename T>
__global__ void __launch_bounds__(256) dropout_inplace_kernel(T* __restrict__ x, long n, float p, uint64_t seed, uint32_t site,
                                                              const unsigned long long* __restrict__ seed_dev) {
  seed = drop_seed(seed, seed_dev);
  const float inv_keep = 1.0f / (1.0f - p);
  const long n8 = (((uintptr_t)x) & 15) == 0 ? (n >> 3) : 0;
  for (long i = (long)blockIdx.x * blockDim.x + threadIdx.x; i < n8; i += (long)gridDim.x * blockDim.x) {
    float v[8];
    Vec8<T>::load(x + i * 8, v);
#pragma unroll
    for (int j = 0; j < 8; ++j) v[j] *= dropout_scale(seed, site, (uint64_t)(i * 8 + j), p, inv_keep);
    Vec8<T>::store(x + i * 8, v);
  }
  for (long i = n8 * 8 + (long)blockIdx.x * blockDim.x + threadIdx.x; i < n; i += (long)gridDim.x * blockDim.x)
    x[i] = from_f<T>(to_f<T>(x[i]) * dropout_scale(seed, site, (uint64_t)i, p, inv_keep));
}
template <typename T>
__global__ void __launch_bounds__(256) relu_bwd_inplace_kernel(T* __restrict__ d, const T* __restrict__ act, long n, float inv_keep) {
  const long n8 = ((((uintptr_t)d) & 15) == 0 && (((uintptr_t)act) & 15) == 0) ? (n >> 3) : 0;
  for (long i = (long)blockIdx.x * blockDim.x + threadIdx.x; i < n8; i += (long)gridDim.x * blockDim.x) {
    float dv[8], av[8];
    Vec8<T>::load(d + i * 8, dv); Vec8<T>::load(act + i * 8, av);
#pragma unroll
    for (int j = 0; j < 8; ++j) dv[j] = av[j] > 0.f ? dv[j] * inv_keep : 0.f;
    Vec8<T>::store(d + i * 8, dv);
  }
  for (long i = n8 * 8 + (long)blockIdx.x * blockDim.x + threadIdx.x; i < n; i += (long)gridDim.x * blockDim.x)
    d[i] = from_f<T>(to_f<T>(act[i]) > 0.f ? to_f<T>(d[i]) * inv_keep : 0.f);
}

template <typename T>
__global__ void __launch_bounds__(256) colsum_partial_kernel(const T* __restrict__ A, long rows, int cols, long ld, float* __restrict__ partial) {
  __shared__ float red[8][33];
  const int tx = threadIdx.x & 31, ty = threadIdx.x >> 5;
  const int col = blockIdx.x * 32 + tx;
  const long per = (rows + gridDim.y - 1) / gridDim.y;
  const long r0 = (long)blockIdx.y * per, r1 = (r0 + per < rows) ? r0 + per : rows;
  float a = 0.f;
  if (col < cols) for (long r = r0 + ty; r < r1; r += 8) a += to_f<T>(A[r * ld + col]);
  red[ty][tx] = a;
  __syncthreads();
  if (ty == 0 && col < cols) {
    float s = 0.f;
#pragma unroll
    for (int i = 0; i < 8; ++i) s += red[i][tx];
    partial[(long)blockIdx.y * cols + col] = s;
  }
}
__global__ void __launch_bounds__(256) colsum_final_kernel(const float* __restrict__ partial, int RS, int cols, float* __restrict__ out, float* __restrict__ out2,
                                                           int unperm_h = 0) {
  const int col = blockIdx.x * blockDim.x + threadIdx.x;
  if (col >= cols) return;
  float s = 0.f;
  for (int r = 0; r < RS; ++r) s += partial[(long)r * cols + col];
  const int oc = unperm_h ? (col & 3) * unperm_h + (col >> 2) : col;
  out[oc] = s;
  if (out2) out2[oc] = s;
}

__global__ void __launch_bounds__(256)
argmax_feedback_kernel(const float* __restrict__ logits, int V, long ld, int64_t end_id, int t,
                       int64_t* __restrict__ cur_tok, int64_t* __restrict__ tokens_t, int32_t* __restrict__ lengths, int32_t* __restrict__ done) {
  __shared__ float bv[8]; __shared__ int bi[8];
  const int b = blockIdx.x, tid = threadIdx.x, lane = tid & 31, warp = tid >> 5;
  const float* row = logits + (long)b * ld;
  float best = -INFINITY; int besti = 0x7fffffff;
  for (int v = tid; v < V; v += 256) { const float x = row[v]; if (x > best || (x == best && v < besti)) { best = x; besti = v; } }
#pragma unroll
  for (int o = 16; o > 0; o >>= 1) {
    const float ob = __shfl_xor_sync(0xffffffffu, best, o); const int oi = __shfl_xor_sync(0xffffffffu, besti, o);
    if (ob > best || (ob == best && oi < besti)) { best = ob; besti = oi; }
  }
  if (lane == 0) { bv[warp] = best; bi[warp] = besti; }
  __syncthreads();
  if (tid == 0) {
    for (int i = 1; i < 8; ++i) if (bv[i] > best || (bv[i] == best && bi[i] < besti)) { best = bv[i]; besti = bi[i]; }
    if (besti == 0x7fffffff) besti = 0;
    cur_tok[b] = besti; tokens_t[b] = besti;
    if (t == 0) { done[b] = 0; lengths[b] = -1; }
    if (besti == end_id && !done[b]) { done[b] = 1; lengths[b] = t; }
  }
}
__global__ void __launch_bounds__(256)
argmax_parts_feedback_kernel(const float* __restrict__ pmax, const int* __restrict__ pidx, int nparts, int B, int64_t end_id, int t,
                             int64_t* __restrict__ cur_tok, int64_t* __restrict__ tokens_t, int32_t* __restrict__ lengths, int32_t* __restrict__ done) {
  const int b = blockIdx.x * (blockDim.x >> 5) + (threadIdx.x >> 5), lane = threadIdx.x & 31;
  if (b >= B) return;
  float best = -INFINITY; int besti = 0x7fffffff;
  for (int p = lane; p < nparts; p += 32) {
    const float x = pmax[(long)b * nparts + p]; const int i = pidx[(long)b * nparts + p];
    if (x > best || (x == best && i < besti)) { best = x; besti = i; }
  }
#pragma unroll
  for (int o = 16; o > 0; o >>= 1) {
    const float ob = __shfl_xor_sync(0xffffffffu, best, o); const int oi = __shfl_xor_sync(0xffffffffu, besti, o);
    if (ob > best || (ob == best && oi < besti)) { best = ob; besti = oi; }
  }
  if (lane == 0) {
    if (besti == 0x7fffffff) besti = 0;
    cur_tok[b] = besti; tokens_t[b] = besti;
    if (t == 0) { done[b] = 0; lengths[b] = -1; }
    if (besti == end_id && !done[b]) { done[b] = 1; lengths[b] = t; }
  }
}
__global__ void bump_counter_kernel(unsigned long long* c) { *c += 1ull; }
__global__ void fill_i64_kernel(int64_t* p, long n, int64_t v) { for (long i = (long)blockIdx.x * blockDim.x + threadIdx.x; i < n; i += (long)gridDim.x * blockDim.x) p[i] = v; }
__global__ void finish_lengths_kernel(int32_t* lengths, int B, int T) { const int b = blockIdx.x * blockDim.x + threadIdx.x; if (b < B && lengths[b] < 0) lengths[b] = T; }

}
```

### imagecaptioner_b200/csrc/gemm.cuh

```cuda
#pragma once
#include "common.cuh"

namespace b2c {

struct LstmEpi {
  int enabled, H;
  const void* addend;
  const float* bias;
  const float* c_prev; float* c_out;
  void* gates_out;
  void* h_rec; long ld_rec; void* h_next; long ld_next; void* h_top; long ld_top;
  float drop_p; unsigned long long seed; unsigned int site; long row_base;
  const unsigned long long* seed_dev;
  const float* addend32; long ld_addend32;
};

constexpr int EVAL_PART_FLOATS = 8;
struct EvalEpi { const float* teacher; const int64_t* targets; float* parts; float inv_temp; int nparts; int cols_per_part; };

struct ArgmaxEpi { float* pmax; int* pidx; int nparts; int cols_per_part; };
inline LstmEpi pack_argmax(const ArgmaxEpi& a) {
  LstmEpi le{};
  le.enabled = 2; le.H = a.nparts; le.c_out = a.pmax; le.gates_out = a.pidx; le.ld_rec = a.cols_per_part;
  return le;
}
inline LstmEpi pack_eval(const EvalEpi& e) {
  LstmEpi le{};
  le.enabled = 3; le.H = e.nparts; le.c_out = e.parts; le.addend = e.teacher; le.h_rec = const_cast<int64_t*>(e.targets);
  le.ld_rec = e.cols_per_part; le.drop_p = e.inv_temp;
  return le;
}

template <typename TL>
__device__ __forceinline__ void lstm_cell_unit(const float (&pre)[4], float c_prev, float (&act)[4], float& c, float& h) {
  act[0] = Math<TL>::sigmoid_(pre[0]); act[1] = Math<TL>::sigmoid_(pre[1]);
  act[2] = Math<TL>::tanh_(pre[2]);    act[3] = Math<TL>::sigmoid_(pre[3]);
  c = fmaf(act[1], c_prev, act[0] * act[2]);
  h = act[3] * Math<TL>::tanh_(c);
}

constexpr int SG_BM = 64, SG_BN = 64, SG_BK = 16;

template <typename TA, typename TB, typename TC>
__global__ void __launch_bounds__(256)
gemm_simt_kernel(int M, int N, int K, float alpha, const TA* __restrict__ A, long lda, int a_mn,
                 const TB* __restrict__ B, long ldb, int b_mn, float beta, TC* __restrict__ C, long ldc,
                 const float* __restrict__ bias, int relu, int row_unperm_h, const __grid_constant__ LstmEpi le) {
  __shared__ float As[SG_BK][SG_BM + 4];
  __shared__ float Bs[SG_BK][SG_BN + 4];
  pdl_launch_dependents();
  pdl_wait();
  const int tid = threadIdx.x;
  const int m0 = blockIdx.y * SG_BM, n0 = blockIdx.x * SG_BN;
  const int tx = tid & 15, ty = tid >> 4;
  float acc[4][4];
#pragma unroll
  for (int i = 0; i < 4; ++i)
#pragma unroll
    for (int j = 0; j < 4; ++j) acc[i][j] = 0.f;

  for (int k0 = 0; k0 < K; k0 += SG_BK) {
#pragma unroll
    for (int it = 0; it < (SG_BM * SG_BK) / 256; ++it) {
      const int idx = tid + it * 256;
      int mm, kk;
      if (a_mn) { kk = idx / SG_BM; mm = idx % SG_BM; } else { mm = idx / SG_BK; kk = idx % SG_BK; }
      const int gm = m0 + mm, gk = k0 + kk;
      float v = 0.f;
      if (gm < M && gk < K) v = to_f<TA>(a_mn ? A[(long)gk * lda + gm] : A[(long)gm * lda + gk]);
      As[kk][mm] = v;
    }
#pragma unroll
    for (int it = 0; it < (SG_BN * SG_BK) / 256; ++it) {
      const int idx = tid + it * 256;
      int nn, kk;
      if (b_mn) { kk = idx / SG_BN; nn = idx % SG_BN; } else { nn = idx / SG_BK; kk = idx % SG_BK; }
      const int gn = n0 + nn, gk = k0 + kk;
      float v = 0.f;
      if (gn < N && gk < K) v = to_f<TB>(b_mn ? B[(long)gk * ldb + gn] : B[(long)gn * ldb + gk]);
      Bs[kk][nn] = v;
    }
    __syncthreads();
#pragma unroll
    for (int kk = 0; kk < SG_BK; ++kk) {
      float a[4], b[4];
#pragma unroll
      for (int i = 0; i < 4; ++i) a[i] = As[kk][ty * 4 + i];
#pragma unroll
      for (int j = 0; j < 4; ++j) b[j] = Bs[kk][tx * 4 + j];
#pragma unroll
      for (int i = 0; i < 4; ++i)
#pragma unroll
        for (int j = 0; j < 4; ++j) acc[i][j] = fmaf(a[i], b[j], acc[i][j]);
    }
    __syncthreads();
  }
  if (le.enabled) {
    const int gn = n0 + tx * 4, unit = gn >> 2, H = le.H;
    if (gn >= N) return;
    const float inv_keep = le.drop_p > 0.f ? 1.0f / (1.0f - le.drop_p) : 1.0f;
    const uint64_t dseed = le.drop_p > 0.f ? drop_seed(le.seed, le.seed_dev) : 0;
#pragma unroll
    for (int i = 0; i < 4; ++i) {
      const int gm = m0 + ty * 4 + i;
      if (gm >= M) continue;
      float pre[4], act[4], c, h;
#pragma unroll
      for (int j = 0; j < 4; ++j) {
        pre[j] = acc[i][j];
        if (le.bias) pre[j] += le.bias[gn + j];
        if (le.addend) pre[j] += to_f<TA>(reinterpret_cast<const TA*>(le.addend)[(long)gm * N + gn + j]);
      }
      lstm_cell_unit<TA>(pre, le.c_prev[(long)gm * H + unit], act, c, h);
      le.c_out[(long)gm * H + unit] = c;
      if (le.gates_out) {
#pragma unroll
        for (int j = 0; j < 4; ++j) reinterpret_cast<TA*>(le.gates_out)[(long)gm * N + gn + j] = from_f<TA>(act[j]);
      }
      if (le.h_rec) reinterpret_cast<TA*>(le.h_rec)[(long)gm * le.ld_rec + unit] = from_f<TA>(h);
      if (le.h_next) {
        const float m = le.drop_p > 0.f ? dropout_scale(dseed, le.site, (uint64_t)((le.row_base + gm) * H + unit), le.drop_p, inv_keep) : 1.0f;
        reinterpret_cast<TA*>(le.h_next)[(long)gm * le.ld_next + unit] = from_f<TA>(h * m);
      }
      if (le.h_top) reinterpret_cast<TA*>(le.h_top)[(long)gm * le.ld_top + unit] = from_f<TA>(h);
    }
    return;
  }
#pragma unroll
  for (int i = 0; i < 4; ++i) {
    const int gm = m0 + ty * 4 + i;
    if (gm >= M) continue;
    const long orow = row_unperm_h ? (long)(gm & 3) * row_unperm_h + (gm >> 2) : (long)gm;
#pragma unroll
    for (int j = 0; j < 4; ++j) {
      const int gn = n0 + tx * 4 + j;
      if (gn >= N) continue;
      float v = alpha * acc[i][j];
      if (bias) v += bias[gn];
      if (relu) v = fmaxf(v, 0.f);
      if (beta != 0.f) v += beta * to_f<TC>(C[orow * ldc + gn]);
      C[orow * ldc + gn] = from_f<TC>(v);
    }
  }
}

constexpr int TC_BM = 128, TC_BK = 64, TC_THREADS = 320;
constexpr uint32_t TC_A_BYTES = TC_BM * TC_BK * 2;

__device__ __forceinline__ void tma_load_2d(void* smem_dst, const CUtensorMap* map, int c0, int c1, uint64_t* bar) {
  asm volatile("cp.async.bulk.tensor.2d.shared::cluster.global.mbarrier::complete_tx::bytes [%0], [%1, {%3, %4}], [%2];"
               :: "r"(smem_u32(smem_dst)), "l"(map), "r"(smem_u32(bar)), "r"(c0), "r"(c1) : "memory");
}
__device__ __forceinline__ void tma_prefetch_desc(const CUtensorMap* map) {
  asm volatile("prefetch.tensormap [%0];" :: "l"(map) : "memory");
}
__device__ __forceinline__ void tc_fence_before() { asm volatile("tcgen05.fence::before_thread_sync;" ::: "memory"); }
__device__ __forceinline__ void tc_fence_after() { asm volatile("tcgen05.fence::after_thread_sync;" ::: "memory"); }
__device__ __forceinline__ void tc_commit(uint64_t* bar) {
  asm volatile("tcgen05.commit.cta_group::1.mbarrier::arrive::one.shared::cluster.b64 [%0];" :: "r"(smem_u32(bar)) : "memory");
}
__device__ __forceinline__ void tc_mma_bf16(uint32_t tmem_d, uint64_t adesc, uint64_t bdesc, uint32_t idesc, uint32_t accumulate) {
  asm volatile(
      "{\n\t.reg .pred p;\n\t"
      "setp.ne.b32 p, %4, 0;\n\t"
      "tcgen05.mma.cta_group::1.kind::f16 [%0], %1, %2, %3, p;\n\t}"
      :: "r"(tmem_d), "l"(adesc), "l"(bdesc), "r"(idesc), "r"(accumulate) : "memory");
}
__device__ __forceinline__ void tmem_ld32(uint32_t taddr, float (&v)[32]) {
  uint32_t r[32];
  asm volatile(
      "tcgen05.ld.sync.aligned.32x32b.x32.b32 "
      "{%0, %1, %2, %3, %4, %5, %6, %7, %8, %9, %10, %11, %12, %13, %14, %15, "
      "%16, %17, %18, %19, %20, %21, %22, %23, %24, %25, %26, %27, %28, %29, %30, %31}, [%32];\n"
      : "=r"(r[0]), "=r"(r[1]), "=r"(r[2]), "=r"(r[3]), "=r"(r[4]), "=r"(r[5]), "=r"(r[6]), "=r"(r[7]),
        "=r"(r[8]), "=r"(r[9]), "=r"(r[10]), "=r"(r[11]), "=r"(r[12]), "=r"(r[13]), "=r"(r[14]), "=r"(r[15]),
        "=r"(r[16]), "=r"(r[17]), "=r"(r[18]), "=r"(r[19]), "=r"(r[20]), "=r"(r[21]), "=r"(r[22]), "=r"(r[23]),
        "=r"(r[24]), "=r"(r[25]), "=r"(r[26]), "=r"(r[27]), "=r"(r[28]), "=r"(r[29]), "=r"(r[30]), "=r"(r[31])
      : "r"(taddr));
  asm volatile("tcgen05.wait::ld.sync.aligned;" ::: "memory");
#pragma unroll
  for (int i = 0; i < 32; ++i) v[i] = __uint_as_float(r[i]);
}

__device__ __forceinline__ uint64_t make_smem_desc(uint32_t saddr, uint32_t lbo_bytes, uint32_t sbo_bytes) {
  uint64_t d = 0;
  d |= (uint64_t)((saddr & 0x3FFFFu) >> 4);
  d |= (uint64_t)((lbo_bytes >> 4) & 0x3FFFu) << 16;
  d |= (uint64_t)((sbo_bytes >> 4) & 0x3FFFu) << 32;
  d |= (uint64_t)1 << 46;
  d |= (uint64_t)2 << 61;
  return d;
}

constexpr int TC_EPI_PITCH = 144;
constexpr int TC_EPI_WARPS = 8;
constexpr int TC_EPI_BYTES = TC_EPI_WARPS * 32 * TC_EPI_PITCH;

template <int BN> struct TcCfg {
#ifndef B2C_STAGES64
#define B2C_STAGES64 4
#endif
#ifndef B2C_STAGES128
#define B2C_STAGES128 4
#endif
  static constexpr int STAGES = BN == 256 ? 3 : (BN == 128 ? B2C_STAGES128 : B2C_STAGES64);
  static constexpr uint32_t B_BYTES = BN * TC_BK * 2;
  static constexpr uint32_t STAGE_BYTES = TC_A_BYTES + B_BYTES;
  static constexpr uint32_t TMEM_COLS = 2 * BN;
  static constexpr size_t SMEM_BYTES = (size_t)STAGES * STAGE_BYTES + 1024  + 256  + TC_EPI_BYTES;
};

__device__ __forceinline__ uint4 epi_combine_bf16(uint4 acc, uint4 old, float beta) {
  uint4 o;
  o.x = pack_bf16(bf16_lo(acc.x) + beta * bf16_lo(old.x), bf16_hi(acc.x) + beta * bf16_hi(old.x));
  o.y = pack_bf16(bf16_lo(acc.y) + beta * bf16_lo(old.y), bf16_hi(acc.y) + beta * bf16_hi(old.y));
  o.z = pack_bf16(bf16_lo(acc.z) + beta * bf16_lo(old.z), bf16_hi(acc.z) + beta * bf16_hi(old.z));
  o.w = pack_bf16(bf16_lo(acc.w) + beta * bf16_lo(old.w), bf16_hi(acc.w) + beta * bf16_hi(old.w));
  return o;
}
__device__ __forceinline__ uint4 epi_combine_f32(uint4 acc, uint4 old, float beta) {
  uint4 o;
  o.x = __float_as_uint(__uint_as_float(acc.x) + beta * __uint_as_float(old.x));
  o.y = __float_as_uint(__uint_as_float(acc.y) + beta * __uint_as_float(old.y));
  o.z = __float_as_uint(__uint_as_float(acc.z) + beta * __uint_as_float(old.z));
  o.w = __float_as_uint(__uint_as_float(acc.w) + beta * __uint_as_float(old.w));
  return o;
}

template <int BN, bool A_MN, bool B_MN, typename TC, int EPI = 0>
__global__ void __launch_bounds__(TC_THREADS, 1)
gemm_tc_kernel(const __grid_constant__ CUtensorMap tmA, const __grid_constant__ CUtensorMap tmB,
               int M, int N, int K, float alpha, float beta, TC* __restrict__ C, long ldc,
               const float* __restrict__ bias, int relu, int kb_per_split, int tiles_m, int tiles_n, int splits,
               int row_unperm_h, const __grid_constant__ LstmEpi le) {
  constexpr bool LSTM = (EPI == 1 || EPI == 5);
  constexpr bool LSTM_DROP = (EPI == 1);
  using Cfg = TcCfg<BN>;
  constexpr int TC_STAGES = Cfg::STAGES;
  extern __shared__ unsigned char smem_dyn[];
  unsigned char* base = reinterpret_cast<unsigned char*>(((uintptr_t)smem_dyn + 1023) & ~(uintptr_t)1023);
  uint64_t* full_bar = reinterpret_cast<uint64_t*>(base + (size_t)TC_STAGES * Cfg::STAGE_BYTES);
  uint64_t* empty_bar = full_bar + TC_STAGES;
  uint64_t* tfull_bar = empty_bar + TC_STAGES;
  uint64_t* tempty_bar = tfull_bar + 2;
  uint32_t* tmem_slot = reinterpret_cast<uint32_t*>(tempty_bar + 2);
  unsigned char* epi_stage = base + (size_t)TC_STAGES * Cfg::STAGE_BYTES + 256;

  const int warp = threadIdx.x >> 5, lane = threadIdx.x & 31;
  const int num_kb_total = (K + TC_BK - 1) / TC_BK;
  const int tiles_mn = tiles_m * tiles_n;
  const int total = tiles_mn * splits;
  const bool split = splits > 1;

  pdl_launch_dependents();
  if (warp == 0 && lane == 0) { tma_prefetch_desc(&tmA); tma_prefetch_desc(&tmB); }
  if (warp == 1) {
    if (lane == 0) {
      for (int i = 0; i < TC_STAGES; ++i) { mbar_init(&full_bar[i], 1); mbar_init(&empty_bar[i], 1); }
      for (int i = 0; i < 2; ++i) { mbar_init(&tfull_bar[i], 1); mbar_init(&tempty_bar[i], TC_EPI_WARPS); }
      fence_barrier_init();
    }
    __syncwarp();
    asm volatile("tcgen05.alloc.cta_group::1.sync.aligned.shared::cta.b32 [%0], %1;" :: "r"(smem_u32(tmem_slot)), "r"(Cfg::TMEM_COLS) : "memory");
    asm volatile("tcgen05.relinquish_alloc_permit.cta_group::1.sync.aligned;" ::: "memory");
  }
  tc_fence_before();
  __syncthreads();
  tc_fence_after();
  const uint32_t tmem_base = *tmem_slot;
  pdl_wait();

  if (warp == 0) {
    if (lane == 0) {
      int it = 0;
      for (int w = blockIdx.x; w < total; w += gridDim.x) {
        const int sp = w / tiles_mn, rem = w - sp * tiles_mn;
        const int m0 = (rem / tiles_n) * TC_BM, n0 = (rem % tiles_n) * BN;
        const int kb_begin = sp * kb_per_split, kb_end = min(num_kb_total, kb_begin + kb_per_split);
        for (int kb = kb_begin; kb < kb_end; ++kb, ++it) {
          const int s = it % TC_STAGES; const uint32_t ph = (it / TC_STAGES) & 1;
          mbar_wait(&empty_bar[s], ph ^ 1);
          unsigned char* sa = base + (size_t)s * Cfg::STAGE_BYTES;
          unsigned char* sb = sa + TC_A_BYTES;
          mbar_arrive_expect_tx(&full_bar[s], Cfg::STAGE_BYTES);
          const int k0 = kb * TC_BK;
          if (!A_MN) {
            tma_load_2d(sa, &tmA, k0, m0, &full_bar[s]);
          } else {
#pragma unroll
            for (int j = 0; j < TC_BM / 64; ++j) tma_load_2d(sa + j * 8192, &tmA, m0 + j * 64, k0, &full_bar[s]);
          }
          if (!B_MN) {
            tma_load_2d(sb, &tmB, k0, n0, &full_bar[s]);
          } else {
#pragma unroll
            for (int j = 0; j < BN / 64; ++j) tma_load_2d(sb + j * 8192, &tmB, n0 + j * 64, k0, &full_bar[s]);
          }
        }
      }
    }
  } else if (warp == 1) {
    if (lane == 0) {
      constexpr uint32_t idesc = (1u << 4) | (1u << 7) | (1u << 10) | ((A_MN ? 1u : 0u) << 15) | ((B_MN ? 1u : 0u) << 16) |
                                 ((uint32_t)(BN >> 3) << 17) | ((uint32_t)(TC_BM >> 4) << 24);
      int it = 0, t = 0;
      for (int w = blockIdx.x; w < total; w += gridDim.x, ++t) {
        const int sp = w / tiles_mn;
        const int kb_begin = sp * kb_per_split, kb_end = min(num_kb_total, kb_begin + kb_per_split);
        const int as = t & 1; const uint32_t aph = (t >> 1) & 1;
        mbar_wait(&tempty_bar[as], aph ^ 1);
        tc_fence_after();
        const uint32_t tacc = tmem_base + (uint32_t)(as * BN);
        for (int kb = kb_begin; kb < kb_end; ++kb, ++it) {
          const int s = it % TC_STAGES; const uint32_t ph = (it / TC_STAGES) & 1;
          mbar_wait(&full_bar[s], ph);
          tc_fence_after();
          const uint32_t sa = smem_u32(base + (size_t)s * Cfg::STAGE_BYTES);
          const uint32_t sb = sa + TC_A_BYTES;
#pragma unroll
          for (int k = 0; k < TC_BK / 16; ++k) {
            const uint64_t adesc = A_MN ? make_smem_desc(sa + k * 2048, 8192, 1024) : make_smem_desc(sa + k * 32, 16, 1024);
            const uint64_t bdesc = B_MN ? make_smem_desc(sb + k * 2048, 8192, 1024) : make_smem_desc(sb + k * 32, 16, 1024);
            tc_mma_bf16(tacc, adesc, bdesc, idesc, (kb > kb_begin || k > 0) ? 1u : 0u);
          }
          tc_commit(&empty_bar[s]);
        }
        tc_commit(&tfull_bar[as]);
      }
    }
  } else {
    const int q = warp & 3;
    const int half = (warp - 2) >> 2;
    unsigned char* my = epi_stage + (size_t)(warp - 2) * 32 * TC_EPI_PITCH;
    constexpr int PER = 16 / (int)sizeof(TC);
    constexpr int CH = 128 / (int)sizeof(TC);
    const bool vec_ok = (((uintptr_t)C) % 16 == 0) && ((ldc * (long)sizeof(TC)) % 16 == 0);
    int t = 0;
    for (int w = blockIdx.x; w < total; w += gridDim.x, ++t) {
    const int sp = w / tiles_mn, rem = w - sp * tiles_mn;
    const int m0 = (rem / tiles_n) * TC_BM, n0 = (rem % tiles_n) * BN;
    const int as = t & 1; const uint32_t aph = (t >> 1) & 1;
    const bool add_bias = (bias != nullptr) && (sp == 0);
    [[maybe_unused]] float4 pre_b[8]; [[maybe_unused]] uint4 pre_a[4]; [[maybe_unused]] float4 pre_c0, pre_c1; [[maybe_unused]] float4 pre_r[8];
    [[maybe_unused]] int pre_ci = -1;
    if constexpr (LSTM) {
      constexpr int NC32 = BN / 32, C32_PER = (NC32 + 1) / 2;
      const int ci = half * C32_PER, col0 = n0 + ci * 32, grow = m0 + q * 32 + lane;
      if (ci < NC32 && col0 < N && grow < M) {
        pre_ci = ci;
        if (le.bias) {
#pragma unroll
          for (int j = 0; j < 8; ++j) pre_b[j] = *reinterpret_cast<const float4*>(le.bias + col0 + 4 * j);
        }
        if (le.addend) {
          const uint4* ap = reinterpret_cast<const uint4*>(reinterpret_cast<const bf16*>(le.addend) + (long)grow * N + col0);
#pragma unroll
          for (int j = 0; j < 4; ++j) pre_a[j] = ap[j];
        }
        if (le.addend32) {
          const float4* rp = reinterpret_cast<const float4*>(le.addend32 + (long)grow * le.ld_addend32 + col0);
#pragma unroll
          for (int j = 0; j < 8; ++j) pre_r[j] = __ldcg(rp + j);
        }
        pre_c0 = *reinterpret_cast<const float4*>(le.c_prev + (long)grow * le.H + (col0 >> 2));
        pre_c1 = *reinterpret_cast<const float4*>(le.c_prev + (long)grow * le.H + (col0 >> 2) + 4);
      }
    }
    mbar_wait(&tfull_bar[as], aph);
    tc_fence_after();
    const uint32_t tacc = tmem_base + (uint32_t)(as * BN) + ((uint32_t)(q * 32) << 16);
    if constexpr (LSTM) {
      const int H = le.H, N4 = N;
      const int grow = m0 + q * 32 + lane;
      [[maybe_unused]] const float inv_keep = (LSTM_DROP && le.drop_p > 0.f) ? 1.0f / (1.0f - le.drop_p) : 1.0f;
      [[maybe_unused]] const uint64_t dseed = (LSTM_DROP && le.drop_p > 0.f) ? drop_seed(le.seed, le.seed_dev) : 0;
      constexpr int NC32 = BN / 32, C32_PER = (NC32 + 1) / 2;
#pragma unroll 1
      for (int ci = half * C32_PER; ci < (half + 1) * C32_PER && ci < NC32; ++ci) {
        const int col0 = n0 + ci * 32;
        if (col0 >= N) break;
        float v[32];
        tmem_ld32(tacc + (uint32_t)(ci * 32), v);
        if (grow < M) {
          const bool pre = (ci == pre_ci);
          if (le.bias) {
#pragma unroll
            for (int j = 0; j < 32; j += 4) {
              const float4 b4 = pre ? pre_b[j >> 2] : *reinterpret_cast<const float4*>(le.bias + col0 + j);
              v[j] += b4.x; v[j + 1] += b4.y; v[j + 2] += b4.z; v[j + 3] += b4.w;
            }
          }
          if (le.addend) {
            const uint4* ap = reinterpret_cast<const uint4*>(reinterpret_cast<const bf16*>(le.addend) + (long)grow * N4 + col0);
#pragma unroll
            for (int j = 0; j < 4; ++j) {
              const uint4 a = pre ? pre_a[j] : ap[j];
              v[j * 8 + 0] += bf16_lo(a.x); v[j * 8 + 1] += bf16_hi(a.x); v[j * 8 + 2] += bf16_lo(a.y); v[j * 8 + 3] += bf16_hi(a.y);
              v[j * 8 + 4] += bf16_lo(a.z); v[j * 8 + 5] += bf16_hi(a.z); v[j * 8 + 6] += bf16_lo(a.w); v[j * 8 + 7] += bf16_hi(a.w);
            }
          }
          if (le.addend32) {
            const float4* rp = reinterpret_cast<const float4*>(le.addend32 + (long)grow * le.ld_addend32 + col0);
#pragma unroll
            for (int j = 0; j < 8; ++j) {
              const float4 r4 = pre ? pre_r[j] : __ldcg(rp + j);
              v[4 * j] += r4.x; v[4 * j + 1] += r4.y; v[4 * j + 2] += r4.z; v[4 * j + 3] += r4.w;
            }
          }
          const int u0 = col0 >> 2;
          const float4 cp0 = pre ? pre_c0 : *reinterpret_cast<const float4*>(le.c_prev + (long)grow * H + u0);
          const float4 cp1 = pre ? pre_c1 : *reinterpret_cast<const float4*>(le.c_prev + (long)grow * H + u0 + 4);
          const float cp[8] = {cp0.x, cp0.y, cp0.z, cp0.w, cp1.x, cp1.y, cp1.z, cp1.w};
          float cn[8], hn[8];
#pragma unroll
          for (int u = 0; u < 8; ++u) {
            float pre[4] = {v[4 * u], v[4 * u + 1], v[4 * u + 2], v[4 * u + 3]}, act[4];
            lstm_cell_unit<bf16>(pre, cp[u], act, cn[u], hn[u]);
            v[4 * u] = act[0]; v[4 * u + 1] = act[1]; v[4 * u + 2] = act[2]; v[4 * u + 3] = act[3];
          }
          *reinterpret_cast<float4*>(le.c_out + (long)grow * H + u0) = make_float4(cn[0], cn[1], cn[2], cn[3]);
          *reinterpret_cast<float4*>(le.c_out + (long)grow * H + u0 + 4) = make_float4(cn[4], cn[5], cn[6], cn[7]);
          if (le.gates_out) {
            uint4* gp = reinterpret_cast<uint4*>(reinterpret_cast<bf16*>(le.gates_out) + (long)grow * N4 + col0);
#pragma unroll
            for (int j = 0; j < 4; ++j)
              gp[j] = make_uint4(pack_bf16(v[j * 8], v[j * 8 + 1]), pack_bf16(v[j * 8 + 2], v[j * 8 + 3]), pack_bf16(v[j * 8 + 4], v[j * 8 + 5]), pack_bf16(v[j * 8 + 6], v[j * 8 + 7]));
          }
          const uint4 hp = make_uint4(pack_bf16(hn[0], hn[1]), pack_bf16(hn[2], hn[3]), pack_bf16(hn[4], hn[5]), pack_bf16(hn[6], hn[7]));
          if (le.h_rec) *reinterpret_cast<uint4*>(reinterpret_cast<bf16*>(le.h_rec) + (long)grow * le.ld_rec + u0) = hp;
          if (le.h_top) *reinterpret_cast<uint4*>(reinterpret_cast<bf16*>(le.h_top) + (long)grow * le.ld_top + u0) = hp;
          if (le.h_next) {
            uint4 hd = hp;
            if (LSTM_DROP && le.drop_p > 0.f) {
              float hm[8];
#pragma unroll
              for (int u = 0; u < 8; ++u) hm[u] = hn[u] * dropout_scale(dseed, le.site, (uint64_t)((le.row_base + grow) * H + u0 + u), le.drop_p, inv_keep);
              hd = make_uint4(pack_bf16(hm[0], hm[1]), pack_bf16(hm[2], hm[3]), pack_bf16(hm[4], hm[5]), pack_bf16(hm[6], hm[7]));
            }
            *reinterpret_cast<uint4*>(reinterpret_cast<bf16*>(le.h_next) + (long)grow * le.ld_next + u0) = hd;
          }
        }
      }
      tc_fence_before();
      __syncwarp();
      if (lane == 0) mbar_arrive(&tempty_bar[as]);
      continue;
    } else {
    constexpr int NCHUNK = BN / CH;
    constexpr int C_PER = (NCHUNK + 1) / 2;
    if constexpr (EPI == 3) {
      const float* zt = reinterpret_cast<const float*>(le.addend);
      const int64_t* tg = reinterpret_cast<const int64_t*>(le.h_rec);
      float* parts = le.c_out;
      const int nparts = le.H, grow = m0 + q * 32 + lane;
      const float inv_temp = le.drop_p, L2E = 1.4426950408889634f, kT = inv_temp * L2E;
      const bool row_ok = grow < M;
      const long tcol = row_ok ? (long)tg[grow] : -1;
      float my = -INFINITY, s1 = 0.f, sT = 0.f, mz = -INFINITY, sZ = 0.f, sA = 0.f, ytgt = 0.f; int bidx = 0x7fffffff;
#pragma unroll 1
      for (int ci = half * C_PER; ci < (half + 1) * C_PER && ci < NCHUNK; ++ci) {
#pragma unroll 1
        for (int h = 0; h < CH / 32; ++h) {
          const int colb = n0 + ci * CH + h * 32;
          if (colb >= N) break;
          float v[32], z[32];
          tmem_ld32(tacc + (uint32_t)(ci * CH + h * 32), v);
          const bool full = colb + 32 <= N;
          const float* zr = zt + (long)(row_ok ? grow : 0) * N + colb;
          if (full && ((((uintptr_t)zr) & 15) == 0)) {
#pragma unroll
            for (int j = 0; j < 8; ++j) { const float4 t4 = __ldg(reinterpret_cast<const float4*>(zr) + j); z[4 * j] = t4.x; z[4 * j + 1] = t4.y; z[4 * j + 2] = t4.z; z[4 * j + 3] = t4.w; }
          } else {
#pragma unroll
            for (int j = 0; j < 32; ++j) z[j] = (colb + j < N) ? __ldg(zr + j) : -INFINITY;
          }
#pragma unroll
          for (int j = 0; j < 32; ++j) v[j] = (colb + j < N) ? fmaf(alpha, v[j], bias != nullptr ? __ldg(bias + colb + j) : 0.f) : -INFINITY;
          float cmy = v[0], cmz = z[0];
#pragma unroll
          for (int j = 1; j < 32; ++j) { cmy = fmaxf(cmy, v[j]); cmz = fmaxf(cmz, z[j]); }
          if (cmy > my) {
#pragma unroll
            for (int j = 31; j >= 0; --j) if (v[j] == cmy) bidx = colb + j;
          }
          const float nmy = fmaxf(my, cmy), nmz = fmaxf(mz, cmz);
          const float ry = my - nmy, rz = (mz - nmz) * inv_temp;
          const float c1 = ex2_ftz(ry * L2E), cT = ex2_ftz(ry * kT), cZ = ex2_ftz(rz * L2E);
          sA = (sZ > 0.f) ? cZ * (sA + sZ * (rz - ry * inv_temp)) : 0.f;
          s1 *= c1; sT *= cT; sZ *= cZ;
          my = nmy; mz = nmz;
#pragma unroll
          for (int j = 0; j < 32; ++j) {
            const float yd = v[j] - my, zd = (z[j] - mz) * inv_temp;
            const float eT = ex2_ftz(yd * kT), e1 = ex2_ftz(yd * L2E), ez = ex2_ftz(zd * L2E);
            s1 += e1; sT += eT; sZ += ez;
            sA += (ez > 0.f) ? ez * (zd - yd * inv_temp) : 0.f;
          }
          if (tcol >= colb && tcol < colb + 32) {
#pragma unroll
            for (int j = 0; j < 32; ++j) if (colb + j == tcol) ytgt = v[j];
          }
        }
      }
      if (row_ok) {
        const int part = (n0 + half * C_PER * CH) / (C_PER * CH);
        if (part < nparts) {
          float4* o = reinterpret_cast<float4*>(parts + ((long)grow * nparts + part) * EVAL_PART_FLOATS);
          o[0] = make_float4(my, s1, sT, mz);
          o[1] = make_float4(sZ, sA, ytgt, __int_as_float(bidx));
        }
      }
      tc_fence_before();
      __syncwarp();
      if (lane == 0) mbar_arrive(&tempty_bar[as]);
      continue;
    }
    if constexpr (EPI == 2) {
      float* pmax = le.c_out; int* pidx = reinterpret_cast<int*>(le.gates_out);
      const int nparts = le.H, grow = m0 + q * 32 + lane;
      float best = -INFINITY; int bidx = 0x7fffffff;
#pragma unroll 1
      for (int ci = half * C_PER; ci < (half + 1) * C_PER && ci < NCHUNK; ++ci) {
#pragma unroll 1
        for (int h = 0; h < CH / 32; ++h) {
          const int colb = n0 + ci * CH + h * 32;
          if (colb >= N) break;
          float v[32];
          tmem_ld32(tacc + (uint32_t)(ci * CH + h * 32), v);
          if (colb + 32 <= N && bias != nullptr && (((uintptr_t)bias) & 15) == 0) {
            const float4* b4 = reinterpret_cast<const float4*>(bias + colb);
#pragma unroll
            for (int j = 0; j < 8; ++j) {
              const float4 bb = __ldg(b4 + j);
              v[4 * j] = fmaf(alpha, v[4 * j], bb.x); v[4 * j + 1] = fmaf(alpha, v[4 * j + 1], bb.y);
              v[4 * j + 2] = fmaf(alpha, v[4 * j + 2], bb.z); v[4 * j + 3] = fmaf(alpha, v[4 * j + 3], bb.w);
            }
          } else {
#pragma unroll
            for (int j = 0; j < 32; ++j) v[j] = fmaf(alpha, v[j], (bias != nullptr && colb + j < N) ? bias[colb + j] : 0.f);
          }
#pragma unroll
          for (int j = 0; j < 32; ++j) if (colb + j < N && v[j] > best) { best = v[j]; bidx = colb + j; }
        }
      }
      if (grow < M) {
        const int part = (n0 + half * C_PER * CH) / (C_PER * CH);
        if (part < nparts) { pmax[(long)grow * nparts + part] = best; pidx[(long)grow * nparts + part] = bidx; }
      }
      tc_fence_before();
      __syncwarp();
      if (lane == 0) mbar_arrive(&tempty_bar[as]);
      continue;
    }
    if constexpr (EPI == 0 || EPI == 4) {
    if (EPI == 4 || ((split ? sizeof(TC) == 4 : beta == 0.f) && vec_ok && m0 + TC_BM <= M && n0 + BN <= N && (((uintptr_t)bias) & 15) == 0)) {
#pragma unroll 1
      for (int ci = half * C_PER; ci < (half + 1) * C_PER && ci < NCHUNK; ++ci) {
        const int c0 = ci * CH;
#pragma unroll
        for (int h = 0; h < CH / 32; ++h) {
          float v[32];
          tmem_ld32(tacc + (uint32_t)(c0 + h * 32), v);
          if (add_bias) {
            const float4* b4 = reinterpret_cast<const float4*>(bias + n0 + c0 + h * 32);
#pragma unroll
            for (int j = 0; j < 8; ++j) {
              const float4 bb = __ldg(b4 + j);
              v[4 * j] = fmaf(alpha, v[4 * j], bb.x); v[4 * j + 1] = fmaf(alpha, v[4 * j + 1], bb.y);
              v[4 * j + 2] = fmaf(alpha, v[4 * j + 2], bb.z); v[4 * j + 3] = fmaf(alpha, v[4 * j + 3], bb.w);
            }
          } else if (alpha != 1.0f) {
#pragma unroll
            for (int j = 0; j < 32; ++j) v[j] *= alpha;
          }
          if (relu) {
#pragma unroll
            for (int j = 0; j < 32; ++j) v[j] = fmaxf(v[j], 0.f);
          }
          unsigned char* dst = my + lane * TC_EPI_PITCH + h * 32 * sizeof(TC);
          if (sizeof(TC) == 2) {
#pragma unroll
            for (int j = 0; j < 32; j += 8)
              *reinterpret_cast<uint4*>(dst + j * 2) = make_uint4(pack_bf16(v[j], v[j + 1]), pack_bf16(v[j + 2], v[j + 3]), pack_bf16(v[j + 4], v[j + 5]), pack_bf16(v[j + 6], v[j + 7]));
          } else {
#pragma unroll
            for (int j = 0; j < 32; j += 4)
              *reinterpret_cast<uint4*>(dst + j * 4) = make_uint4(__float_as_uint(v[j]), __float_as_uint(v[j + 1]), __float_as_uint(v[j + 2]), __float_as_uint(v[j + 3]));
          }
        }
        __syncwarp();
#pragma unroll
        for (int it = 0; it < 8; ++it) {
          const int r = it * 4 + (lane >> 3), grow = m0 + q * 32 + r;
          const long orow = row_unperm_h ? (long)(grow & 3) * row_unperm_h + (grow >> 2) : (long)grow;
          TC* cp = C + orow * ldc + n0 + c0 + (lane & 7) * PER;
          const uint4 acc = *reinterpret_cast<const uint4*>(my + r * TC_EPI_PITCH + (lane & 7) * 16);
          if (split) {
            asm volatile("red.global.add.v4.f32 [%0], {%1, %2, %3, %4};" :: "l"(cp), "f"(__uint_as_float(acc.x)), "f"(__uint_as_float(acc.y)),
                         "f"(__uint_as_float(acc.z)), "f"(__uint_as_float(acc.w)) : "memory");
          } else {
            *reinterpret_cast<uint4*>(cp) = acc;
          }
        }
        __syncwarp();
      }
      tc_fence_before();
      __syncwarp();
      if (lane == 0) mbar_arrive(&tempty_bar[as]);
      continue;
    }
    if constexpr (EPI == 0) {
#pragma unroll 1
    for (int ci = half * C_PER; ci < (half + 1) * C_PER && ci < NCHUNK; ++ci) {
      const int c0 = ci * CH;
      if (n0 + c0 >= N) break;
#pragma unroll
      for (int h = 0; h < CH / 32; ++h) {
        float v[32];
        tmem_ld32(tacc + (uint32_t)(c0 + h * 32), v);
        const int colb = n0 + c0 + h * 32;
#pragma unroll
        for (int j = 0; j < 32; ++j) {
          float x = alpha * v[j];
          if (add_bias && colb + j < N) x += bias[colb + j];
          if (relu) x = fmaxf(x, 0.f);
          v[j] = x;
        }
        unsigned char* dst = my + lane * TC_EPI_PITCH + h * 32 * sizeof(TC);
        if (sizeof(TC) == 2) {
#pragma unroll
          for (int j = 0; j < 32; j += 8)
            *reinterpret_cast<uint4*>(dst + j * 2) = make_uint4(pack_bf16(v[j], v[j + 1]), pack_bf16(v[j + 2], v[j + 3]), pack_bf16(v[j + 4], v[j + 5]), pack_bf16(v[j + 6], v[j + 7]));
        } else {
#pragma unroll
          for (int j = 0; j < 32; j += 4)
            *reinterpret_cast<uint4*>(dst + j * 4) = make_uint4(__float_as_uint(v[j]), __float_as_uint(v[j + 1]), __float_as_uint(v[j + 2]), __float_as_uint(v[j + 3]));
        }
      }
      __syncwarp();
#pragma unroll 1
      for (int it = 0; it < 8; ++it) {
        const int r = it * 4 + (lane >> 3), part = lane & 7;
        const int grow = m0 + q * 32 + r, gcol = n0 + c0 + part * PER;
        if (grow < M && gcol < N) {
          const uint4 acc = *reinterpret_cast<const uint4*>(my + r * TC_EPI_PITCH + part * 16);
          const long orow = row_unperm_h ? (long)(grow & 3) * row_unperm_h + (grow >> 2) : (long)grow;
          TC* cp = C + orow * ldc + gcol;
          if (split) {
            if (vec_ok && gcol + 4 <= N) {
              asm volatile("red.global.add.v4.f32 [%0], {%1, %2, %3, %4};" :: "l"(cp), "f"(__uint_as_float(acc.x)), "f"(__uint_as_float(acc.y)),
                           "f"(__uint_as_float(acc.z)), "f"(__uint_as_float(acc.w)) : "memory");
            } else {
              const float* a = reinterpret_cast<const float*>(&acc);
#pragma unroll
              for (int e = 0; e < 4; ++e) if (gcol + e < N) atomicAdd(reinterpret_cast<float*>(cp) + e, a[e]);
            }
          } else if (vec_ok && gcol + PER <= N) {
            uint4 o = acc;
            if (beta != 0.f) {
              const uint4 old = *reinterpret_cast<const uint4*>(cp);
              o = (sizeof(TC) == 2) ? epi_combine_bf16(acc, old, beta) : epi_combine_f32(acc, old, beta);
            }
            *reinterpret_cast<uint4*>(cp) = o;
          } else {
            const TC* a = reinterpret_cast<const TC*>(&acc);
#pragma unroll
            for (int e = 0; e < PER; ++e) {
              if (gcol + e < N) {
                float x = to_f<TC>(a[e]);
                if (beta != 0.f) x += beta * to_f<TC>(cp[e]);
                cp[e] = from_f<TC>(x);
              }
            }
          }
        }
      }
      __syncwarp();
    }
    tc_fence_before();
    __syncwarp();
    if (lane == 0) mbar_arrive(&tempty_bar[as]);
    }
    }
    }
    }
  }
  tc_fence_before();
  __syncthreads();
  if (warp == 1) {
    __syncwarp();
    asm volatile("tcgen05.dealloc.cta_group::1.sync.aligned.b32 %0, %1;" :: "r"(tmem_base), "r"(Cfg::TMEM_COLS) : "memory");
  }
}

typedef CUresult (*PFN_encodeTiled)(CUtensorMap*, CUtensorMapDataType, cuuint32_t, void*, const cuuint64_t*, const cuuint64_t*,
                                    const cuuint32_t*, const cuuint32_t*, CUtensorMapInterleave, CUtensorMapSwizzle,
                                    CUtensorMapL2promotion, CUtensorMapFloatOOBfill);
inline PFN_encodeTiled get_encode_fn() {
  static PFN_encodeTiled fn = nullptr;
  static bool tried = false;
  if (!tried) {
    tried = true;
    void* p = nullptr;
    cudaDriverEntryPointQueryResult q;
    if (cudaGetDriverEntryPoint("cuTensorMapEncodeTiled", &p, cudaEnableDefault, &q) == cudaSuccess && q == cudaDriverEntryPointSuccess)
      fn = reinterpret_cast<PFN_encodeTiled>(p);
  }
  return fn;
}

inline int make_tmap_bf16(CUtensorMap* map, const void* ptr, long inner, long outer, long ld, int box_outer) {
  PFN_encodeTiled enc = get_encode_fn();
  if (!enc) return set_err(B2C_ECUDA, "cuTensorMapEncodeTiled entry point unavailable");
  cuuint64_t dims[2] = {(cuuint64_t)inner, (cuuint64_t)outer};
  cuuint64_t strides[1] = {(cuuint64_t)ld * 2};
  cuuint32_t box[2] = {64u, (cuuint32_t)box_outer};
  cuuint32_t estr[2] = {1u, 1u};
  CUresult r = enc(map, CU_TENSOR_MAP_DATA_TYPE_BFLOAT16, 2, const_cast<void*>(ptr), dims, strides, box, estr,
                   CU_TENSOR_MAP_INTERLEAVE_NONE, CU_TENSOR_MAP_SWIZZLE_128B, CU_TENSOR_MAP_L2_PROMOTION_L2_256B,
                   CU_TENSOR_MAP_FLOAT_OOB_FILL_NONE);
  if (r != CUDA_SUCCESS) return set_err(B2C_ECUDA, "cuTensorMapEncodeTiled failed (%d): ptr=%p inner=%ld outer=%ld ld=%ld box=%d", (int)r, ptr, inner, outer, ld, box_outer);
  return 0;
}

struct GemmArgs {
  int M, N, K;
  float alpha, beta;
  const void* A; long lda; int a_mn;
  const void* B; long ldb; int b_mn;
  void* C; long ldc;
  const float* bias; int relu;
  int row_unperm_h = 0;
  const LstmEpi* lstm = nullptr;
  ArgmaxEpi* amax = nullptr;
  EvalEpi* eval = nullptr;
};

inline bool tc_eligible(const GemmArgs& g) {
  return ((uintptr_t)g.A % 16 == 0) && ((uintptr_t)g.B % 16 == 0) && (g.lda % 8 == 0) && (g.ldb % 8 == 0);
}

struct TcPlan { int bn, splits, kb_per_split; };
inline TcPlan plan_tc(const GemmArgs& g, int elem_c, int sms) {
  const int num_kb = cdiv(g.K, TC_BK);
  const bool can_split = (elem_c == 4) && !g.relu && (g.beta == 0.f || g.beta == 1.f) && (g.lstm == nullptr) && (g.amax == nullptr) && (g.eval == nullptr);
  TcPlan best{64, 1, num_kb}; double best_cost = 1e30;
  const int cand[3] = {256, 128, 64};
  for (int ci = 0; ci < 3; ++ci) {
    const int bn = cand[ci];
    if (bn > 64 && g.N <= bn / 2) continue;
    const long tiles = (long)cdiv(g.M, TC_BM) * cdiv(g.N, bn);
    int splits = 1;
    if (can_split && tiles < 2L * sms && num_kb >= 16) {
      splits = (int)((2L * sms) / tiles); if (splits > num_kb / 8) splits = num_kb / 8; if (splits < 1) splits = 1;
    }
    const int kbs = cdiv(num_kb, splits); splits = cdiv(num_kb, kbs);
    const long items = tiles * splits;
    const long waves = (items + sms - 1) / sms;
    const double cost = (double)waves * ((double)kbs * (128 + bn) + 6.0 * (128 + bn) + (splits > 1 ? 2.0 : 1.0) * bn * 4.0);
    if (cost < best_cost) { best_cost = cost; best = TcPlan{bn, splits, kbs}; }
  }
  return best;
}

inline bool fast_only_enabled() { static int on = -1; if (on < 0) { const char* e = getenv("B2C_GEMM_FAST_ONLY"); on = (e && e[0] == '0') ? 0 : 1; } return on != 0; }
inline int sm_count() {
  static int n = 0;
  if (n == 0) { int dev = 0; cudaGetDevice(&dev); if (cudaDeviceGetAttribute(&n, cudaDevAttrMultiProcessorCount, dev) != cudaSuccess || n <= 0) n = 148; }
  return n;
}

inline int& gemm_cta_cap() { static thread_local int c = 0; return c; }
struct GemmCapScope {
  int saved;
  explicit GemmCapScope(int cap) : saved(gemm_cta_cap()) { gemm_cta_cap() = cap; }
  ~GemmCapScope() { gemm_cta_cap() = saved; }
};
inline int gemm_sms() { const int n = sm_count(), c = gemm_cta_cap(); return (c > 0 && c < n) ? c : n; }

template <int BN, bool A_MN, bool B_MN, typename TC>
int launch_tc(const GemmArgs& g, const TcPlan& plan, cudaStream_t st) {
  CUtensorMap ta, tb;
  if (!A_MN) B2C_TRY(make_tmap_bf16(&ta, g.A, g.K, g.M, g.lda, TC_BM)); else B2C_TRY(make_tmap_bf16(&ta, g.A, g.M, g.K, g.lda, 64));
  if (!B_MN) B2C_TRY(make_tmap_bf16(&tb, g.B, g.K, g.N, g.ldb, BN)); else B2C_TRY(make_tmap_bf16(&tb, g.B, g.N, g.K, g.ldb, 64));
  constexpr bool CAN_LSTM = !A_MN && !B_MN && sizeof(TC) == 4;
  void (*kern)(const CUtensorMap, const CUtensorMap, int, int, int, float, float, TC*, long, const float*, int, int, int, int, int, int, const LstmEpi) =
      gemm_tc_kernel<BN, A_MN, B_MN, TC, 0>;
  int flavour = g.lstm ? ((g.lstm->drop_p > 0.f && g.lstm->h_next) ? 1 : 5) : (g.amax ? 2 : (g.eval ? 3 : 0));
  if (flavour == 0 && fast_only_enabled() && g.M % TC_BM == 0 && g.N % BN == 0 && (plan.splits > 1 ? sizeof(TC) == 4 : g.beta == 0.f) &&
      ((uintptr_t)g.C) % 16 == 0 && (g.ldc * (long)sizeof(TC)) % 16 == 0 && (((uintptr_t)g.bias) & 15) == 0) {
    flavour = 4;
    kern = gemm_tc_kernel<BN, A_MN, B_MN, TC, 4>;
  }
  if (flavour != 0 && flavour != 4) {
    if constexpr (CAN_LSTM) {
      kern = flavour == 1 ? gemm_tc_kernel<BN, A_MN, B_MN, TC, 1> : (flavour == 5 ? gemm_tc_kernel<BN, A_MN, B_MN, TC, 5> :
             (flavour == 2 ? gemm_tc_kernel<BN, A_MN, B_MN, TC, 2> : gemm_tc_kernel<BN, A_MN, B_MN, TC, 3>));
    } else return set_err(B2C_EINVAL, "the fused LSTM / argmax / validation epilogues need K-major operands and the fp32 instantiation");
  }
  static bool attr_set[6] = {false, false, false, false, false, false};
  if (!attr_set[flavour]) {
    B2C_CUDA(cudaFuncSetAttribute(kern, cudaFuncAttributeMaxDynamicSharedMemorySize, (int)TcCfg<BN>::SMEM_BYTES));
    attr_set[flavour] = true;
  }
  const int kb_per_split = plan.kb_per_split, splits = plan.splits;
  if (splits > 1 && g.beta == 0.f)
    B2C_CUDA(cudaMemset2DAsync(g.C, (size_t)g.ldc * sizeof(TC), 0, (size_t)g.N * sizeof(TC), (size_t)g.M, st));
  const int tiles_m = cdiv(g.M, TC_BM), tiles_n = cdiv(g.N, BN);
  const long total = (long)tiles_m * tiles_n * splits;
  const int grid = (int)(total < gemm_sms() ? total : gemm_sms());
  LstmEpi epi = g.lstm ? *g.lstm : LstmEpi{};
  if (g.amax) {
    B2C_CHECK_ARG(!g.lstm && splits == 1 && g.amax->pmax && g.amax->pidx, "argmax epilogue: no K split, no LSTM epilogue, partial buffers required");
    constexpr int CHc = 128 / (int)sizeof(TC), CPER = (BN / CHc + 1) / 2;
    g.amax->cols_per_part = CPER * CHc;
    g.amax->nparts = cdiv(g.N, g.amax->cols_per_part);
    epi = pack_argmax(*g.amax);
  }
  if (g.eval) {
    B2C_CHECK_ARG(!g.lstm && !g.amax && splits == 1 && g.eval->teacher && g.eval->targets && g.eval->parts, "validation epilogue: no K split, no other epilogue, buffers required");
    constexpr int CHc = 128 / (int)sizeof(TC), CPER = (BN / CHc + 1) / 2;
    g.eval->cols_per_part = CPER * CHc;
    g.eval->nparts = cdiv(g.N, g.eval->cols_per_part);
    epi = pack_eval(*g.eval);
  }
  B2C_CUDA(launch_pdl(kern, dim3(grid), dim3(TC_THREADS), TcCfg<BN>::SMEM_BYTES, st, ta, tb, g.M, g.N, g.K, g.alpha, g.beta, (TC*)g.C, g.ldc,
                      g.bias, g.relu, kb_per_split, tiles_m, tiles_n, splits, g.row_unperm_h, epi));
  B2C_LAUNCH_CHECK("gemm_tc_kernel");
  return 0;
}

template <int BN, typename TC>
int launch_tc_major(const GemmArgs& g, const TcPlan& plan, cudaStream_t st) {
  if (!g.a_mn && !g.b_mn) return launch_tc<BN, false, false, TC>(g, plan, st);
  if (!g.a_mn && g.b_mn) return launch_tc<BN, false, true, TC>(g, plan, st);
  if (g.a_mn && g.b_mn) return launch_tc<BN, true, true, TC>(g, plan, st);
  return launch_tc<BN, true, false, TC>(g, plan, st);
}

template <typename TC>
int gemm_bf16_tc(const GemmArgs& g, cudaStream_t st) {
  const TcPlan plan = plan_tc(g, (int)sizeof(TC), gemm_sms());
  if (plan.bn == 256) return launch_tc_major<256, TC>(g, plan, st);
  if (plan.bn == 128) return launch_tc_major<128, TC>(g, plan, st);
  return launch_tc_major<64, TC>(g, plan, st);
}

template <typename TA, typename TB, typename TC>
int gemm_simt(const GemmArgs& g, cudaStream_t st) {
  dim3 grid(cdiv(g.N, SG_BN), cdiv(g.M, SG_BM));
  B2C_CUDA(launch_pdl(gemm_simt_kernel<TA, TB, TC>, grid, dim3(256), 0, st, g.M, g.N, g.K, g.alpha, (const TA*)g.A, g.lda, g.a_mn,
                      (const TB*)g.B, g.ldb, g.b_mn, g.beta, (TC*)g.C, g.ldc, g.bias, g.relu, g.row_unperm_h, g.lstm ? *g.lstm : LstmEpi{}));
  B2C_LAUNCH_CHECK("gemm_simt_kernel");
  return 0;
}

template <typename T, typename TC> struct Gemm;
template <typename TC> struct Gemm<float, TC> {
  static int run(const GemmArgs& g, cudaStream_t st) { return gemm_simt<float, float, TC>(g, st); }
};
template <typename TC> struct Gemm<bf16, TC> {
  static int run(const GemmArgs& g, cudaStream_t st) {
    if (tc_eligible(g)) return gemm_bf16_tc<TC>(g, st);
    return gemm_simt<bf16, bf16, TC>(g, st);
  }
};

}
```

### imagecaptioner_b200/csrc/recur_cluster.cuh

```cuda
#pragma once
#include "gemm.cuh"

namespace b2c {

constexpr int CR_CL = 8;
constexpr int CR_H = 512, CR_E = 256, CR_L = 2;
constexpr int CR_RMAX = 40;
constexpr int CR_N = 48;
constexpr int CR_SPC = CR_RMAX / CR_CL;
constexpr int CR_UNITS = CR_H / CR_CL;
constexpr int CR_UCOLS = CR_E / CR_CL;
constexpr int CR_STAGES = 6;
constexpr int CR_STAGE_BYTES = 16384;
constexpr int CR_THREADS = 384, CR_WORKERS = 256;
constexpr int CR_HALF = CR_RMAX * 128;
constexpr int CR_BLOCK = 2 * CR_HALF;
constexpr int CR_SMAX = 64;
constexpr int CR_OFF_BH = 0;
constexpr int CR_OFF_CTX = CR_OFF_BH + CR_CL * CR_BLOCK;
constexpr int CR_OFF_RING = CR_OFF_CTX + (CR_E / 64) * CR_HALF;
constexpr int CR_OFF_HST = CR_OFF_RING + CR_STAGES * CR_STAGE_BYTES;
constexpr int CR_OFF_UIN = CR_OFF_HST + CR_RMAX * 128;
constexpr int CR_OFF_E2U = CR_OFF_UIN + CR_SPC * CR_E * 4;
constexpr int CR_OFF_CACC = CR_OFF_E2U + CR_SPC * CR_E * 4;
constexpr int CR_OFF_SC = CR_OFF_CACC + CR_SPC * CR_E * 4;
constexpr int CR_OFF_BAR = CR_OFF_SC + CR_SPC * CR_SMAX * 4;
constexpr int CR_SMEM_BYTES = CR_OFF_BAR + 256 + 1024;
static_assert(CR_OFF_RING % 1024 == 0 && CR_OFF_CTX % 1024 == 0, "swizzled tiles need 1024-byte alignment");
static_assert(CR_SMEM_BYTES <= 227 * 1024, "shared memory budget");
constexpr uint32_t CR_TM_ACC0 = 0, CR_TM_ACC1 = 96, CR_TM_U = 192, CR_TM_COLS = 256;

struct ClusterParams {
  int B, T, S, ncl;
  const float* P;
  float* EP;
  const bf16* F;
  float* u;
  float* attw;
  bf16* xh0; bf16* xh1;
  const bf16* G0T;
  const float* bias1;
  float* c0; float* c1;
  bf16* gates0; bf16* gates1;
  bf16* hid_top;
  unsigned long long* trace;
};
struct ClusterMaps { CUtensorMap w0, w1, wh, h0, h1, ctx; };

__device__ __forceinline__ uint32_t cr_cluster_rank() { uint32_t r; asm volatile("mov.u32 %0, %%cluster_ctarank;" : "=r"(r)); return r; }
__device__ __forceinline__ void cr_cluster_sync() { asm volatile("barrier.cluster.arrive.release.aligned;\n\tbarrier.cluster.wait.acquire.aligned;" ::: "memory"); }
__device__ __forceinline__ uint32_t cr_mapa(uint32_t addr, uint32_t rank) { uint32_t r; asm volatile("mapa.shared::cluster.u32 %0, %1, %2;" : "=r"(r) : "r"(addr), "r"(rank)); return r; }
__device__ __forceinline__ void cr_tma_mc(void* dst, const CUtensorMap* map, int c0, int c1, uint64_t* bar, uint16_t mask) {
  asm volatile("cp.async.bulk.tensor.2d.shared::cluster.global.mbarrier::complete_tx::bytes.multicast::cluster [%0], [%1, {%4, %5}], [%2], %3;"
               :: "r"(smem_u32(dst)), "l"(map), "r"(smem_u32(bar)), "h"(mask), "r"(c0), "r"(c1) : "memory");
}
__device__ __forceinline__ void cr_st_async_v4(uint32_t remote_addr, float a, float b, float c, float d, uint32_t remote_bar) {
  asm volatile("st.async.weak.shared::cluster.mbarrier::complete_tx::bytes.v4.f32 [%0], {%1, %2, %3, %4}, [%5];"
               :: "r"(remote_addr), "f"(a), "f"(b), "f"(c), "f"(d), "r"(remote_bar) : "memory");
}
__device__ __noinline__ void cr_wait_slow(uint64_t* bar, uint32_t parity, int id, int t) {
  for (uint32_t spins = 0; !mbar_try_wait(bar, parity); ++spins) {
    if (spins == (threadIdx.x < 128 ? (1u << 22) : (1u << 18)) && (threadIdx.x < 128 || (threadIdx.x & 31) == 0)) printf("b2c cluster kernel: wait %d stuck at step %d (block %d = cluster %d rank %d, thread %d)\n", id, t, blockIdx.x, blockIdx.x / CR_CL, blockIdx.x % CR_CL, threadIdx.x);
    if (spins > (1u << 24)) __trap();
  }
}
__device__ __forceinline__ void cr_wait(uint64_t* bar, uint32_t parity, int id, int t) {
  if (!mbar_try_wait(bar, parity)) cr_wait_slow(bar, parity, id, t);
}
__device__ __forceinline__ void cr_fence_proxy_global() { asm volatile("fence.proxy.async.global;" ::: "memory"); }
__device__ __forceinline__ void cr_bar_workers() { asm volatile("bar.sync 1, 256;" ::: "memory"); }
__device__ __forceinline__ void cr_tmem_ld16(uint32_t taddr, float* v) {
  uint32_t r[16];
  asm volatile("tcgen05.ld.sync.aligned.32x32b.x16.b32 {%0, %1, %2, %3, %4, %5, %6, %7, %8, %9, %10, %11, %12, %13, %14, %15}, [%16];\n"
               : "=r"(r[0]), "=r"(r[1]), "=r"(r[2]), "=r"(r[3]), "=r"(r[4]), "=r"(r[5]), "=r"(r[6]), "=r"(r[7]),
                 "=r"(r[8]), "=r"(r[9]), "=r"(r[10]), "=r"(r[11]), "=r"(r[12]), "=r"(r[13]), "=r"(r[14]), "=r"(r[15]) : "r"(taddr));
  asm volatile("tcgen05.wait::ld.sync.aligned;" ::: "memory");
#pragma unroll
  for (int i = 0; i < 16; ++i) v[i] = __uint_as_float(r[i]);
}
__device__ __forceinline__ void cr_quad_transpose(float (&a)[4], int q) {
  const bool b0 = q & 1, b1 = q & 2;
  { const float s0 = b0 ? a[0] : a[1], s1 = b0 ? a[2] : a[3];
    const float r0 = __shfl_xor_sync(0xffffffffu, s0, 1), r1 = __shfl_xor_sync(0xffffffffu, s1, 1);
    if (b0) { a[0] = r0; a[2] = r1; } else { a[1] = r0; a[3] = r1; } }
  { const float s0 = b1 ? a[0] : a[2], s1 = b1 ? a[1] : a[3];
    const float r0 = __shfl_xor_sync(0xffffffffu, s0, 2), r1 = __shfl_xor_sync(0xffffffffu, s1, 2);
    if (b1) { a[0] = r0; a[1] = r1; } else { a[2] = r0; a[3] = r1; } }
}

__host__ __device__ inline void cr_rows(int B, int ncl, int i, int& r0, int& n) {
  const int q = B / ncl, rem = B % ncl;
  n = q + (i < rem ? 1 : 0);
  r0 = i * q + (i < rem ? i : rem);
}

__global__ void __launch_bounds__(256) g0_cluster_layout_kernel(const bf16* __restrict__ G0, int B, int T, int ncl, bf16* __restrict__ out) {
  __shared__ bf16 tile[CR_RMAX][64 + 2];
  const int t = blockIdx.z, i = blockIdx.y, g0 = blockIdx.x * 64;
  int r0, n; cr_rows(B, ncl, i, r0, n);
  for (int idx = threadIdx.x; idx < CR_RMAX * 64; idx += 256) {
    const int s = idx >> 6, g = idx & 63;
    tile[s][g] = s < n ? G0[((long)t * B + r0 + s) * (4 * CR_H) + g0 + g] : __float2bfloat16(0.f);
  }
  __syncthreads();
  bf16* o = out + (((long)t * ncl + i) * (4 * CR_H) + g0) * CR_RMAX;
  for (int idx = threadIdx.x; idx < 64 * CR_RMAX; idx += 256) {
    const int g = idx / CR_RMAX, s = idx % CR_RMAX;
    o[idx] = tile[s][g];
  }
}

__global__ void __launch_bounds__(CR_THREADS, 1)
recur_cluster_fwd_kernel(const __grid_constant__ ClusterMaps maps, const __grid_constant__ ClusterParams p) {
  extern __shared__ unsigned char smem_dyn[];
  unsigned char* base = reinterpret_cast<unsigned char*>(((uintptr_t)smem_dyn + 1023) & ~(uintptr_t)1023);
  uint64_t* bars = reinterpret_cast<uint64_t*>(base + CR_OFF_BAR);
  uint64_t* full_bar = bars;
  uint64_t* empty_bar = bars + CR_STAGES;
  uint64_t* bar_h1 = bars + 2 * CR_STAGES + 0;
  uint64_t* bar_h0 = bars + 2 * CR_STAGES + 1;
  uint64_t* bar_ctx = bars + 2 * CR_STAGES + 2;
  uint64_t* bar_uin = bars + 2 * CR_STAGES + 3;
  uint64_t* bar_u = bars + 2 * CR_STAGES + 4;
  uint64_t* bar_early = bars + 2 * CR_STAGES + 5;
  uint64_t* bar_acc0 = bars + 2 * CR_STAGES + 6;
  uint64_t* bar_acc1 = bars + 2 * CR_STAGES + 7;
  uint32_t* tmem_slot = reinterpret_cast<uint32_t*>(bars + 2 * CR_STAGES + 8);

  const int tid = threadIdx.x, warp = tid >> 5, lane = tid & 31;
  const int c = (int)cr_cluster_rank();
  const int ci = blockIdx.x / CR_CL;
  const int B = p.B, T = p.T, S = p.S;
  int r0, n; cr_rows(B, p.ncl, ci, r0, n);
  const int nv = max(0, min(CR_SPC, n - CR_SPC * c));
  constexpr uint32_t H_TILE_BYTES = CR_CL * CR_HALF;
  constexpr uint32_t CTX_TILE_BYTES = CR_CL * (CR_E / 64) * CR_SPC * 128;
  const uint32_t uin_bytes = (uint32_t)nv * CR_E * 4;

  if (tid == 0) {
    tma_prefetch_desc(&maps.w0); tma_prefetch_desc(&maps.w1); tma_prefetch_desc(&maps.wh);
    tma_prefetch_desc(&maps.h0); tma_prefetch_desc(&maps.h1); tma_prefetch_desc(&maps.ctx);
    for (int i = 0; i < CR_STAGES; ++i) { mbar_init(&full_bar[i], 1); mbar_init(&empty_bar[i], 1); }
    for (int i = 0; i < 8; ++i) mbar_init(&bars[2 * CR_STAGES + i], 1);
    fence_barrier_init();
    mbar_arrive_expect_tx(bar_h1, H_TILE_BYTES);
    mbar_arrive_expect_tx(bar_h0, H_TILE_BYTES);
    mbar_arrive_expect_tx(bar_ctx, CTX_TILE_BYTES);
    mbar_arrive_expect_tx(bar_uin, uin_bytes);
  }
  if (warp == 1) {
    asm volatile("tcgen05.alloc.cta_group::1.sync.aligned.shared::cta.b32 [%0], %1;" :: "r"(smem_u32(tmem_slot)), "r"(CR_TM_COLS) : "memory");
    asm volatile("tcgen05.relinquish_alloc_permit.cta_group::1.sync.aligned;" ::: "memory");
  }
  tc_fence_before();
  __syncthreads();
  tc_fence_after();
  const uint32_t tmem_base = *tmem_slot;
  cr_cluster_sync();
  pdl_wait();

  if (warp == 0) {
    if (lane == 0) {
      cr_tma_mc(base + CR_OFF_BH + c * CR_BLOCK, &maps.h1, CR_H + 64 * c, r0, bar_h1, 0xFF);
      cr_tma_mc(base + CR_OFF_BH + c * CR_BLOCK + CR_HALF, &maps.h0, CR_E + 64 * c, r0, bar_h0, 0xFF);
      uint32_t it = 0;
      auto acquire = [&]() -> unsigned char* {
        const int s = it % CR_STAGES; const uint32_t ph = (it / CR_STAGES) & 1;
        cr_wait(&empty_bar[s], ph ^ 1, 100 + s, (int)(it / 58));
        mbar_arrive_expect_tx(&full_bar[s], CR_STAGE_BYTES);
        return base + CR_OFF_RING + s * CR_STAGE_BYTES;
      };
      const int row0 = 256 * c;
      for (int t = 0; t < T; ++t) {
        for (int s2 = 0; s2 < 2; ++s2) {
          unsigned char* sa = acquire(); uint64_t* fb = &full_bar[it % CR_STAGES];
          for (int i = 0; i < 4; ++i) tma_load_2d(sa + i * 4096, &maps.wh, 64 * (4 * s2 + i), CR_UCOLS * c, fb);
          ++it;
        }
        for (int kb = 0; kb < CR_H / 64; ++kb) for (int g = 0; g < 2; ++g) {
          unsigned char* sa = acquire(); tma_load_2d(sa, &maps.w1, CR_H + 64 * kb, row0 + 128 * g, &full_bar[it % CR_STAGES]); ++it; }
        for (int kb = 0; kb < CR_H / 64; ++kb) for (int g = 0; g < 2; ++g) {
          unsigned char* sa = acquire(); tma_load_2d(sa, &maps.w0, CR_E + 64 * kb, row0 + 128 * g, &full_bar[it % CR_STAGES]); ++it; }
        for (int kb = 0; kb < CR_E / 64; ++kb) for (int g = 0; g < 2; ++g) {
          unsigned char* sa = acquire(); tma_load_2d(sa, &maps.w0, 64 * kb, row0 + 128 * g, &full_bar[it % CR_STAGES]); ++it; }
        for (int kb = 0; kb < CR_H / 64; ++kb) for (int g = 0; g < 2; ++g) {
          unsigned char* sa = acquire(); tma_load_2d(sa, &maps.w1, 64 * kb, row0 + 128 * g, &full_bar[it % CR_STAGES]); ++it; }
      }
    }
  } else if (warp == 1) {
    if (lane == 0) {
      constexpr uint32_t IDESC_G = (1u << 4) | (1u << 7) | (1u << 10) | ((uint32_t)(CR_N >> 3) << 17) | ((uint32_t)(128 >> 4) << 24);
      constexpr uint32_t IDESC_U = (1u << 4) | (1u << 7) | (1u << 10) | ((uint32_t)(CR_UCOLS >> 3) << 17) | ((uint32_t)(128 >> 4) << 24);
      const uint32_t bh = smem_u32(base + CR_OFF_BH), bctx = smem_u32(base + CR_OFF_CTX), ring = smem_u32(base + CR_OFF_RING);
      uint32_t it = 0;
      auto stage = [&]() -> uint32_t {
        const int s = it % CR_STAGES; const uint32_t ph = (it / CR_STAGES) & 1;
        cr_wait(&full_bar[s], ph, 200 + s, (int)(it / 58));
        tc_fence_after();
        return ring + s * CR_STAGE_BYTES;
      };
      auto release = [&]() { tc_commit(&empty_bar[it % CR_STAGES]); ++it; };
      auto gate_stage = [&](uint32_t tacc, uint32_t bop, bool first) {
        const uint32_t sa = stage();
#pragma unroll
        for (int k = 0; k < 4; ++k)
          tc_mma_bf16(tacc, make_smem_desc(sa + k * 32, 16, 1024), make_smem_desc(bop + k * 32, 16, 1024), IDESC_G, (first && k == 0) ? 0u : 1u);
        release();
      };
      for (int t = 0; t < T; ++t) {
        cr_wait(bar_h1, t & 1, 1, t);
        if (t + 1 < T) mbar_arrive_expect_tx(bar_h1, H_TILE_BYTES);
        tc_fence_after();
        for (int s2 = 0; s2 < 2; ++s2) {
          const uint32_t sa = stage();
#pragma unroll
          for (int i = 0; i < 4; ++i) {
            const int kb = 4 * s2 + i;
#pragma unroll
            for (int k = 0; k < 4; ++k)
              tc_mma_bf16(tmem_base + CR_TM_U, make_smem_desc(bh + kb * CR_BLOCK + k * 32, 16, 1024), make_smem_desc(sa + i * 4096 + k * 32, 16, 1024),
                          IDESC_U, (kb == 0 && k == 0) ? 0u : 1u);
          }
          release();
        }
        tc_commit(bar_u);
        for (int kb = 0; kb < CR_H / 64; ++kb) for (int g = 0; g < 2; ++g)
          gate_stage(tmem_base + CR_TM_ACC1 + g * CR_N, bh + kb * CR_BLOCK, kb == 0);
        if (t == 0) { cr_wait(bar_h0, 0, 2, t); mbar_arrive_expect_tx(bar_h0, H_TILE_BYTES); tc_fence_after(); }
        for (int kb = 0; kb < CR_H / 64; ++kb) for (int g = 0; g < 2; ++g)
          gate_stage(tmem_base + CR_TM_ACC0 + g * CR_N, bh + kb * CR_BLOCK + CR_HALF, kb == 0);
        tc_commit(bar_early);
        cr_wait(bar_ctx, t & 1, 3, t);
        if (t + 1 < T) mbar_arrive_expect_tx(bar_ctx, CTX_TILE_BYTES);
        tc_fence_after();
        for (int kb = 0; kb < CR_E / 64; ++kb) for (int g = 0; g < 2; ++g)
          gate_stage(tmem_base + CR_TM_ACC0 + g * CR_N, bctx + kb * CR_HALF, false);
        tc_commit(bar_acc0);
        cr_wait(bar_h0, (t + 1) & 1, 4, t);
        if (t + 1 < T) mbar_arrive_expect_tx(bar_h0, H_TILE_BYTES);
        tc_fence_after();
        for (int kb = 0; kb < CR_H / 64; ++kb) for (int g = 0; g < 2; ++g)
          gate_stage(tmem_base + CR_TM_ACC1 + g * CR_N, bh + kb * CR_BLOCK + CR_HALF, false);
        tc_commit(bar_acc1);
      }
    }
  } else if (warp >= 4) {
    const int wt = tid - 128, ww = warp - 4;
    const int grp = ww >> 2, qd = ww & 3;
    const int q = lane & 3;
    const int jl = 8 * qd + (lane >> 2);
    const int unit = CR_UNITS * c + 32 * grp + jl;
    const int grow = 256 * c + 128 * grp + 32 * qd + lane;
    const uint32_t lane_bits = (uint32_t)(32 * qd) << 16;
    float* uin = reinterpret_cast<float*>(base + CR_OFF_UIN);
    float* e2u = reinterpret_cast<float*>(base + CR_OFF_E2U);
    float* cacc = reinterpret_cast<float*>(base + CR_OFF_CACC);
    float* sc = reinterpret_cast<float*>(base + CR_OFF_SC);
    bf16* hst = reinterpret_cast<bf16*>(base + CR_OFF_HST);
    const float act_k = (q == 2) ? 2.f : 1.f, act_a = (q == 2) ? 2.f : 1.f, act_b = (q == 2) ? -1.f : 0.f;
    const float bias1 = p.bias1[grow];
    float cst[CR_L][CR_N / 4];
#pragma unroll
    for (int k = 0; k < CR_L; ++k)
#pragma unroll
      for (int s = 0; s < CR_N / 4; ++s) {
        const int smp = 4 * s + q;
        cst[k][s] = smp < n ? (k == 0 ? p.c0 : p.c1)[(long)(r0 + smp) * CR_H + unit] : 0.f;
      }
    const long SE = (long)S * CR_E;
    for (int sm = 0; sm < nv; ++sm) {
      const long off = (long)(r0 + CR_SPC * c + sm) * SE;
      for (long i = wt * 4; i < SE; i += CR_WORKERS * 4) {
        const float4 v = *reinterpret_cast<const float4*>(p.P + off + i);
        float4 o;
        o.x = ex2_ftz(2.8853900817779268f * v.x); o.y = ex2_ftz(2.8853900817779268f * v.y);
        o.z = ex2_ftz(2.8853900817779268f * v.z); o.w = ex2_ftz(2.8853900817779268f * v.w);
        *reinterpret_cast<float4*>(p.EP + off + i) = o;
      }
    }
    __threadfence_block();
    cr_bar_workers();

    for (int t = 0; t < T; ++t) {
      unsigned long long* tr = (p.trace && wt == 0) ? p.trace + ((size_t)blockIdx.x * T + t) * 8 : nullptr;
      if (tr) tr[0] = clock64();
      cr_wait(bar_u, t & 1, 5, t);
      tc_fence_after();
      if (grp == 0 && qd < 2) {
        const int row = 32 * qd + lane;
        float v[32];
        tmem_ld32(tmem_base + CR_TM_U + lane_bits, v);
        if (row < n) {
          float* ug = p.u + ((long)t * B + r0 + row) * CR_E + CR_UCOLS * c;
          const int dst = row / CR_SPC, slot = row % CR_SPC;
          const uint32_t ra = cr_mapa(smem_u32(uin + slot * CR_E + CR_UCOLS * c), (uint32_t)dst), rb = cr_mapa(smem_u32(bar_uin), (uint32_t)dst);
#pragma unroll
          for (int j = 0; j < 32; j += 4) {
            cr_st_async_v4(ra + j * 4, v[j], v[j + 1], v[j + 2], v[j + 3], rb);
            *reinterpret_cast<float4*>(ug + j) = make_float4(v[j], v[j + 1], v[j + 2], v[j + 3]);
          }
        }
      }
      tc_fence_before();
      if (tr) tr[1] = clock64();
      cr_wait(bar_uin, t & 1, 6, t);
      for (int i = wt; i < nv * CR_E; i += CR_WORKERS) e2u[i] = ex2_ftz(2.8853900817779268f * uin[i]);
      for (int i = wt; i < CR_SPC * CR_E; i += CR_WORKERS) cacc[i] = 0.f;
      cr_bar_workers();
      if (wt == 0 && t + 1 < T) mbar_arrive_expect_tx(bar_uin, uin_bytes);
      if (tr) tr[2] = clock64();
      {
        const int items = nv * S;
        constexpr int BATCH = 8;
        for (int i0 = ww; i0 < items; i0 += 8 * BATCH) {
          float4 pa[BATCH], pb[BATCH];
#pragma unroll
          for (int k = 0; k < BATCH; ++k) {
            const int it = i0 + 8 * k;
            if (it < items) {
              const int sm = it / S, l = it - sm * S;
              const float* ep = p.EP + (long)(r0 + CR_SPC * c + sm) * SE + (long)l * CR_E;
              pa[k] = __ldcg(reinterpret_cast<const float4*>(ep) + lane);
              pb[k] = __ldcg(reinterpret_cast<const float4*>(ep + 128) + lane);
            }
          }
#pragma unroll
          for (int k = 0; k < BATCH; ++k) {
            const int it = i0 + 8 * k;
            if (it < items) {
              const int sm = it / S, l = it - sm * S;
              const float4 ua = *reinterpret_cast<const float4*>(e2u + sm * CR_E + 4 * lane);
              const float4 ub = *reinterpret_cast<const float4*>(e2u + sm * CR_E + 128 + 4 * lane);
              float a = rcp_ftz_(fmaf(pa[k].x, ua.x, 1.f)) + rcp_ftz_(fmaf(pa[k].y, ua.y, 1.f)) + rcp_ftz_(fmaf(pa[k].z, ua.z, 1.f)) + rcp_ftz_(fmaf(pa[k].w, ua.w, 1.f));
              a += rcp_ftz_(fmaf(pb[k].x, ub.x, 1.f)) + rcp_ftz_(fmaf(pb[k].y, ub.y, 1.f)) + rcp_ftz_(fmaf(pb[k].z, ub.z, 1.f)) + rcp_ftz_(fmaf(pb[k].w, ub.w, 1.f));
              a = warp_sum(a);
              if (lane == 0) sc[sm * CR_SMAX + l] = fmaf(-2.f, a, (float)CR_E);
            }
          }
        }
      }
      cr_bar_workers();
      if (ww < nv) {
        float* s_ = sc + ww * CR_SMAX;
        const float v0 = lane < S ? s_[lane] : -INFINITY, v1 = lane + 32 < S ? s_[lane + 32] : -INFINITY;
        const float m = warp_max(fmaxf(v0, v1));
        const float e0 = lane < S ? ex2_ftz(1.4426950408889634f * (v0 - m)) : 0.f, e1 = lane + 32 < S ? ex2_ftz(1.4426950408889634f * (v1 - m)) : 0.f;
        const float inv = 1.0f / warp_sum(e0 + e1);
        float* aw = p.attw + ((long)t * B + r0 + CR_SPC * c + ww) * S;
        if (lane < S) { s_[lane] = e0 * inv; aw[lane] = e0 * inv; }
        if (lane + 32 < S) { s_[lane + 32] = e1 * inv; aw[lane + 32] = e1 * inv; }
      }
      cr_bar_workers();
      if (tr) tr[3] = clock64();
      {
// ... 112 lines not shown
```

Measured before the change: 208,200.

## Fuse LSTM cell adjoint into split-K cluster GEMM epilogue; vectorize pointwise backward

Adds an opt-in split-K tensor-core GEMM that runs in 4-CTA clusters and reduces partial sums through distributed shared memory. Its epilogue computes the next LSTM cell's backward pointwise adjoint directly, removing separate pointwise kernel launches and memsets per timestep. Separately, the standalone pointwise backward kernel now handles four hidden units per thread with float4 loads and stores. The fused path is gated by an environment variable that defaults to off, and it adds cluster-synchronisation complexity.

```diff
diff --git a/imagecaptioner_b200/csrc/api.cu b/imagecaptioner_b200/csrc/api.cu
--- a/imagecaptioner_b200/csrc/api.cu
+++ b/imagecaptioner_b200/csrc/api.cu
@@ -510,6 +510,7 @@
 inline int bg_ctas() { static int v = -1; if (v < 0) { const char* e = getenv("B2C_BG_CTAS"); v = e ? atoi(e) : 10; } return v; }
 inline bool attn_post_occ3() { static int v = -1; if (v < 0) { const char* e = getenv("B2C_POST_OCC3"); v = (e && e[0] == '0') ? 0 : 1; } return v != 0; }
 inline int wgrad_chunks() { static int v = -1; if (v < 0) { const char* e = getenv("B2C_WGRAD_CHUNKS"); v = e ? atoi(e) : 0; } return v; }
+inline bool fused_cell_bwd() { static int v = -1; if (v < 0) { const char* e = getenv("B2C_FUSED_CELL_BWD"); v = (e && e[0] == '1') ? 1 : 0; } return v != 0; }
 
 template <typename T>
 int decoder_backward_impl(const B2CShape& s, const B2CParams& p, const T* feats, const int64_t* cap, const T* hid_top,
@@ -525,10 +526,13 @@
   B2C_TRY(get_substreams(&hs));
   cudaStream_t side = hs->s[MAX_SUB - 1];
   for (int k = 0; k < L; ++k) B2C_CHECK_ARG(g.w_ih[k] && g.w_hh[k] && g.b_ih[k] && g.b_hh[k], "NULL LSTM gradient pointer (layer %d)", k);
+  const bool fuse_ok = sizeof(T) == 2 && fused_cell_bwd() && pick_sub_batches(B) == 1 && ((uintptr_t)dhid & 7) == 0;
+  const bool fuse_q = fuse_ok && Tn > 1 && cell_bwd_plan(B, H, E, H) != 0;
+  const bool fuse_x = fuse_ok && L > 1 && cell_bwd_plan(B, 2 * H, 4 * H, H) != 0;
   B2C_CUDA(cudaEventRecord(hs->ev[3], st));
   B2C_CUDA(cudaStreamWaitEvent(side, hs->ev[3], 0));
   B2C_CUDA(cudaMemsetAsync(W.dxh0, 0, (size_t)TB * (E + H) * sizeof(float), side));
-  for (int k = 1; k < L; ++k) B2C_CUDA(cudaMemsetAsync(W.dxh[k], 0, (size_t)TB * 2 * H * sizeof(float), side));
+  for (int k = 1; k < (fuse_x ? 0 : L); ++k) B2C_CUDA(cudaMemsetAsync(W.dxh[k], 0, (size_t)TB * 2 * H * sizeof(float), side));
   B2C_CUDA(cudaEventRecord(hs->ev[3], side));
   B2C_TRY((gemm<T, T>(st, (int)TB, E, V, dlogits, V, 0, W.w.W2, E, 1, W.do1, E)));
   relu_bwd_inplace_kernel<T><<<ew_grid(TB * E), 256, 0, st>>>(W.do1, W.o1, TB * E, inv_keep);
@@ -571,23 +575,51 @@
       const long b0 = sp.b0[i];
       const int Bh = sp.bn[i];
       const long row = (long)t * B + b0;
+      auto carry_of = [&](int k, long rw, bool lst) -> const float* {
+        return lst ? nullptr : (k == 0 ? W.dxh0 + (rw + B) * (E + H) + E : W.dxh[k] + (rw + B) * 2 * H + H);
+      };
+      auto ld_carry = [&](int k) -> long { return k == 0 ? E + H : 2 * H; };
+      auto cell_epi = [&](int k, long rw, bool lst) {
+        const bool top = (k == L - 1);
+        CellBwdEpi e{};
+        e.H = H; e.n_adj = H;
+        e.gates = reinterpret_cast<const bf16*>(W.gates[k] + rw * 4 * H); e.c_prev = W.c[k] + rw * H; e.c_cur = W.c[k] + (rw + B) * H;
+        e.dc = W.dc[k]; e.dc_is_zero = lst ? 1 : 0;
+        e.carry = carry_of(k, rw, lst); e.ld_carry = ld_carry(k);
+        e.dh_ext = top ? W.dHext + rw * H : nullptr;
+        e.dh_hid = reinterpret_cast<const bf16*>((top && dhid) ? dhid + rw * H : nullptr);
+        e.dgates = reinterpret_cast<bf16*>(W.dgates[k] + rw * 4 * H);
+        e.drop_p = top ? 0.f : dr.p; e.seed = dr.seed; e.site = (unsigned)k; e.row_base = rw; e.seed_dev = (const unsigned long long*)dr.seed_dev;
+        return e;
+      };
       for (int k = L - 1; k >= 0; --k) {
         const int in = in_dim(s, k), ld = in + H;
-        const float* carry = last ? nullptr : (k == 0 ? W.dxh0 + (row + B) * (E + H) + E : W.dxh[k] + (row + B) * 2 * H + H);
-        const float* above = (k < L - 1) ? W.dxh[k + 1] + row * 2 * H : nullptr;
         const bool top = (k == L - 1);
-        B2C_CUDA(launch_pdl(lstm_pointwise_bwd_kernel<T>, dim3(ew_grid((long)Bh * H)), dim3(256), 0, ss,
-            (const T*)(W.gates[k] + row * 4 * H), (const float*)(W.c[k] + row * H), (const float*)(W.c[k] + (row + B) * H), W.dc[k] + b0 * H, last ? 1 : 0,
-            carry, (long)ld, above, (long)(2 * H), (const float*)(top ? W.dHext + row * H : nullptr), (const T*)((top && dhid) ? dhid + row * H : nullptr),
-            (const T*)((top && !last) ? W.dq + b0 * H : nullptr), (long)H, W.dgates[k] + row * 4 * H, Bh, H, dr.p, dr.seed, (uint32_t)k, row, (const unsigned long long*)dr.seed_dev));
-        B2C_LAUNCH_CHECK("lstm_pointwise_bwd_kernel");
+        if (!(top ? (fuse_q && !last) : fuse_x)) {
+          const float* above = (k < L - 1) ? W.dxh[k + 1] + row * 2 * H : nullptr;
+          B2C_CUDA(launch_pdl(lstm_pointwise_bwd_kernel<T>, dim3(ew_grid((long)Bh * H / 4)), dim3(256), 0, ss,
+              (const T*)(W.gates[k] + row * 4 * H), (const float*)(W.c[k] + row * H), (const float*)(W.c[k] + (row + B) * H), W.dc[k] + b0 * H, last ? 1 : 0,
+              carry_of(k, row, last), ld_carry(k), above, (long)(2 * H), (const float*)(top ? W.dHext + row * H : nullptr), (const T*)((top && dhid) ? dhid + row * H : nullptr),
+              (const T*)((top && !last) ? W.dq + b0 * H : nullptr), (long)H, W.dgates[k] + row * 4 * H, Bh, H, dr.p, dr.seed, (uint32_t)k, row, (const unsigned long long*)dr.seed_dev));
+          B2C_LAUNCH_CHECK("lstm_pointwise_bwd_kernel");
+        }
         float* out = (k == 0) ? W.dxh0 + row * (E + H) : W.dxh[k] + row * 2 * H;
-        B2C_TRY((gemm<T, float>(ss, Bh, ld, 4 * H, W.dgates[k] + row * 4 * H, 4 * H, 0, W.w.Wcat[k], ld, 1, out, ld, 1.f)));
+        if (k > 0 && fuse_x) {
+          GemmArgs gx{Bh, ld, 4 * H, 1.f, 0.f, W.dgates[k] + row * 4 * H, 4L * H, 0, W.w.Wcat[k], (long)ld, 1, out, (long)ld, nullptr, 0};
+          B2C_TRY(gemm_cell_bwd(gx, cell_epi(k - 1, row, last), ss));
+        } else {
+          B2C_TRY((gemm<T, float>(ss, Bh, ld, 4 * H, W.dgates[k] + row * 4 * H, 4 * H, 0, W.w.Wcat[k], ld, 1, out, ld, 1.f)));
+        }
       }
       const float* dctx_t = W.dxh0 + row * (E + H);
       T* du_t = W.du + row * E;
       B2C_TRY(attn_bwd<T>(ss, Bh, S, E, W.P + b0 * S * E, feats + b0 * S * E, W.u + row * E, attw + row * S, dctx_t, (long)(E + H), W.ds + row * S, du_t));
-      if (t > 0) B2C_TRY((gemm<T, T>(ss, Bh, H, E, du_t, E, 0, W.w.Wh, H, 1, W.dq + b0 * H, H)));
+      if (t > 0 && fuse_q) {
+        GemmArgs gq{Bh, H, E, 1.f, 0.f, du_t, (long)E, 0, W.w.Wh, (long)H, 1, nullptr, (long)H, nullptr, 0};
+        B2C_TRY(gemm_cell_bwd(gq, cell_epi(L - 1, row - B, false), ss));
+      } else if (t > 0) {
+        B2C_TRY((gemm<T, T>(ss, Bh, H, E, du_t, E, 0, W.w.Wh, H, 1, W.dq + b0 * H, H)));
+      }
     }
     if (chunk_steps > 0 && t > 0 && (Tn - t) % chunk_steps == 0 && t >= chunk_steps) {
       B2C_CUDA(cudaEventRecord(hs->ev[0], st));
diff --git a/imagecaptioner_b200/csrc/common.cuh b/imagecaptioner_b200/csrc/common.cuh
--- a/imagecaptioner_b200/csrc/common.cuh
+++ b/imagecaptioner_b200/csrc/common.cuh
@@ -80,6 +80,13 @@
   return mix32(seed, stream, idx) >= thr ? inv_keep : 0.0f;
 }
 
+__device__ __forceinline__ void lstm_cell_adjoint(float dh, const float (&gt)[4], float tc, float cp, float dc_in, float (&dg)[4], float& dc_out) {
+  const float i = gt[0], f = gt[1], g = gt[2], o = gt[3];
+  const float dcc = dc_in + dh * o * (1.0f - tc * tc);
+  dg[0] = dcc * g * i * (1.0f - i); dg[1] = dcc * cp * f * (1.0f - f); dg[2] = dcc * i * (1.0f - g * g); dg[3] = dh * tc * o * (1.0f - o);
+  dc_out = dcc * f;
+}
+
 __device__ __forceinline__ void pdl_launch_dependents() { asm volatile("griddepcontrol.launch_dependents;" ::: "memory"); }
 __device__ __forceinline__ void pdl_wait() { asm volatile("griddepcontrol.wait;" ::: "memory"); }
 
@@ -91,16 +98,31 @@
 inline bool& pdl_full_dependency_flag() { static thread_local bool f = false; return f; }
 inline void pdl_full_dependency_next() { pdl_full_dependency_flag() = true; }
 template <typename... KArgs, typename... Args>
-inline cudaError_t launch_pdl(void (*kern)(KArgs...), dim3 grid, dim3 block, size_t smem, cudaStream_t st, Args... args) {
+inline cudaError_t launch_pdl_cluster(void (*kern)(KArgs...), dim3 grid, dim3 block, size_t smem, cudaStream_t st, int cluster, Args... args) {
   cudaLaunchConfig_t cfg{};
   cfg.gridDim = grid; cfg.blockDim = block; cfg.dynamicSmemBytes = smem; cfg.stream = st;
-  cudaLaunchAttribute attr[1];
-  attr[0].id = cudaLaunchAttributeProgrammaticStreamSerialization;
-  attr[0].val.programmaticStreamSerializationAllowed = 1;
-  cfg.attrs = attr; cfg.numAttrs = (pdl_enabled() && !pdl_full_dependency_flag()) ? 1 : 0;
+  cudaLaunchAttribute attr[2];
+  int n = 0;
+  if (pdl_enabled() && !pdl_full_dependency_flag()) {
+    attr[n].id = cudaLaunchAttributeProgrammaticStreamSerialization;
+    attr[n++].val.programmaticStreamSerializationAllowed = 1;
+  }
+  if (cluster > 1) {
+    attr[n].id = cudaLaunchAttributeClusterDimension;
+    attr[n].val.clusterDim.x = (unsigned)cluster; attr[n].val.clusterDim.y = 1; attr[n++].val.clusterDim.z = 1;
+  }
+  cfg.attrs = attr; cfg.numAttrs = n;
   pdl_full_dependency_flag() = false;
   return cudaLaunchKernelEx(&cfg, kern, static_cast<KArgs>(args)...);
 }
+template <typename... KArgs, typename... Args>
+inline cudaError_t launch_pdl(void (*kern)(KArgs...), dim3 grid, dim3 block, size_t smem, cudaStream_t st, Args... args) {
+  return launch_pdl_cluster(kern, grid, block, smem, st, 1, args...);
+}
+
+__device__ __forceinline__ uint32_t cr_cluster_rank() { uint32_t r; asm volatile("mov.u32 %0, %%cluster_ctarank;" : "=r"(r)); return r; }
+__device__ __forceinline__ void cr_cluster_sync() { asm volatile("barrier.cluster.arrive.release.aligned;\n\tbarrier.cluster.wait.acquire.aligned;" ::: "memory"); }
+__device__ __forceinline__ uint32_t cr_mapa(uint32_t addr, uint32_t rank) { uint32_t r; asm volatile("mapa.shared::cluster.u32 %0, %1, %2;" : "=r"(r) : "r"(addr), "r"(rank)); return r; }
 
 __device__ __forceinline__ uint32_t smem_u32(const void* p) { return (uint32_t)__cvta_generic_to_shared(p); }
 
diff --git a/imagecaptioner_b200/csrc/decoder_kernels.cuh b/imagecaptioner_b200/csrc/decoder_kernels.cuh
--- a/imagecaptioner_b200/csrc/decoder_kernels.cuh
+++ b/imagecaptioner_b200/csrc/decoder_kernels.cuh
@@ -431,36 +431,52 @@
                           const unsigned long long* __restrict__ seed_dev) {
   pdl_launch_dependents();
   if (drop_p > 0.f) seed = drop_seed(seed, seed_dev);
-  const long total = (long)B * H;
+  const long total = (long)B * H / 4;
   const float inv_keep = drop_p > 0.f ? 1.0f / (1.0f - drop_p) : 1.0f;
-  struct Saved { float gt[4]; float tc, cp, dh_fixed, mask; };
-  auto load_saved = [&](long idx, Saved& sv) {
+  struct Saved { float gt[4][4]; float4 tc, cp, dh_fixed; float mask[4]; };
+  auto load_saved = [&](long g, Saved& sv) {
+    const long idx = 4 * g;
     const long b = (long)((unsigned)idx / (unsigned)H); const int j = (int)(idx - b * H);
-    Gate4<T>::load(gates + b * 4 * H + 4 * j, sv.gt);
-    sv.tc = Math<T>::tanh_(c_cur[idx]);
-    sv.cp = c_prev[idx];
-    float d = 0.f;
-    if (dh_ext) d += dh_ext[idx];
-    if (dh_hid) d += to_f<T>(dh_hid[idx]);
+#pragma unroll
+    for (int u = 0; u < 4; ++u) Gate4<T>::load(gates + b * 4 * H + 4 * (j + u), sv.gt[u]);
+    const float4 c4 = *reinterpret_cast<const float4*>(c_cur + idx);
+    sv.tc = make_float4(Math<T>::tanh_(c4.x), Math<T>::tanh_(c4.y), Math<T>::tanh_(c4.z), Math<T>::tanh_(c4.w));
+    sv.cp = *reinterpret_cast<const float4*>(c_prev + idx);
+    float4 d = dh_ext ? *reinterpret_cast<const float4*>(dh_ext + idx) : make_float4(0.f, 0.f, 0.f, 0.f);
+    if (dh_hid) { d.x += to_f<T>(dh_hid[idx]); d.y += to_f<T>(dh_hid[idx + 1]); d.z += to_f<T>(dh_hid[idx + 2]); d.w += to_f<T>(dh_hid[idx + 3]); }
     sv.dh_fixed = d;
-    sv.mask = (dh_above && drop_p > 0.f) ? dropout_scale(seed, site, (uint64_t)((row_base + b) * H + j), drop_p, inv_keep) : 1.0f;
+#pragma unroll
+    for (int u = 0; u < 4; ++u)
+      sv.mask[u] = (dh_above && drop_p > 0.f) ? dropout_scale(seed, site, (uint64_t)((row_base + b) * H + j + u), drop_p, inv_keep) : 1.0f;
   };
-  const long idx0 = (long)blockIdx.x * blockDim.x + threadIdx.x;
+  const long g0 = (long)blockIdx.x * blockDim.x + threadIdx.x;
   Saved sv;
-  if (idx0 < total) load_saved(idx0, sv);
+  if (g0 < total) load_saved(g0, sv);
   pdl_wait();
-  for (long idx = idx0; idx < total; idx += (long)gridDim.x * blockDim.x) {
-    if (idx != idx0) load_saved(idx, sv);
+  for (long g = g0; g < total; g += (long)gridDim.x * blockDim.x) {
+    if (g != g0) load_saved(g, sv);
+    const long idx = 4 * g;
     const long b = (long)((unsigned)idx / (unsigned)H); const int j = (int)(idx - b * H);
-    float dh = sv.dh_fixed;
-    if (dh_carry) dh += __ldcg(dh_carry + b * ld_carry + j);
-    if (dh_above) dh += __ldcg(dh_above + b * ld_above + j) * sv.mask;
-    if (dh_q) dh += to_f<T>(dh_q[b * ld_q + j]);
-    const float i = sv.gt[0], f = sv.gt[1], g = sv.gt[2], o = sv.gt[3], tc = sv.tc;
-    const float dcc = (dc_is_zero ? 0.f : __ldcg(dc + idx)) + dh * o * (1.0f - tc * tc);
-    const float dg[4] = {dcc * g * i * (1.0f - i), dcc * sv.cp * f * (1.0f - f), dcc * i * (1.0f - g * g), dh * tc * o * (1.0f - o)};
-    Gate4<T>::store(dgates + b * 4 * H + 4 * j, dg);
-    dc[idx] = dcc * f;
+    float dh[4] = {sv.dh_fixed.x, sv.dh_fixed.y, sv.dh_fixed.z, sv.dh_fixed.w};
+    if (dh_carry) { const float4 v = __ldcg(reinterpret_cast<const float4*>(dh_carry + b * ld_carry + j)); dh[0] += v.x; dh[1] += v.y; dh[2] += v.z; dh[3] += v.w; }
+    if (dh_above) {
+      const float4 v = __ldcg(reinterpret_cast<const float4*>(dh_above + b * ld_above + j));
+      dh[0] += v.x * sv.mask[0]; dh[1] += v.y * sv.mask[1]; dh[2] += v.z * sv.mask[2]; dh[3] += v.w * sv.mask[3];
+    }
+    if (dh_q) {
+#pragma unroll
+      for (int u = 0; u < 4; ++u) dh[u] += to_f<T>(dh_q[b * ld_q + j + u]);
+    }
+    const float4 dci = dc_is_zero ? make_float4(0.f, 0.f, 0.f, 0.f) : __ldcg(reinterpret_cast<const float4*>(dc + idx));
+    const float tc[4] = {sv.tc.x, sv.tc.y, sv.tc.z, sv.tc.w}, cp[4] = {sv.cp.x, sv.cp.y, sv.cp.z, sv.cp.w}, dcin[4] = {dci.x, dci.y, dci.z, dci.w};
+    float dco[4];
+#pragma unroll
+    for (int u = 0; u < 4; ++u) {
+      float dg[4];
+      lstm_cell_adjoint(dh[u], sv.gt[u], tc[u], cp[u], dcin[u], dg, dco[u]);
+      Gate4<T>::store(dgates + b * 4 * H + 4 * (j + u), dg);
+    }
+    *reinterpret_cast<float4*>(dc + idx) = make_float4(dco[0], dco[1], dco[2], dco[3]);
   }
 }
 
diff --git a/imagecaptioner_b200/csrc/gemm.cuh b/imagecaptioner_b200/csrc/gemm.cuh
--- a/imagecaptioner_b200/csrc/gemm.cuh
+++ b/imagecaptioner_b200/csrc/gemm.cuh
@@ -1,4 +1,5 @@
 #pragma once
+#include <type_traits>
 #include "common.cuh"
 
 namespace b2c {
@@ -30,6 +31,19 @@
   le.ld_rec = e.cols_per_part; le.drop_p = e.inv_temp;
   return le;
 }
+
+constexpr int CELL_SPLITS = 4;
+struct CellBwdEpi {
+  int H, n_adj;
+  const bf16* gates;
+  const float* c_prev; const float* c_cur;
+  float* dc; int dc_is_zero;
+  const float* carry; long ld_carry;
+  const float* dh_ext; const bf16* dh_hid;
+  bf16* dgates;
+  float drop_p; unsigned long long seed; unsigned int site; long row_base;
+  const unsigned long long* seed_dev;
+};
 
 template <typename TL>
 __device__ __forceinline__ void lstm_cell_unit(const float (&pre)[4], float c_prev, float (&act)[4], float& c, float& h) {
@@ -227,14 +241,17 @@
   return o;
 }
 
+template <int EPI> using TcEpiParam = typename std::conditional<EPI == 6 || EPI == 7, CellBwdEpi, LstmEpi>::type;
 template <int BN, bool A_MN, bool B_MN, typename TC, int EPI = 0>
 __global__ void __launch_bounds__(TC_THREADS, 1)
 gemm_tc_kernel(const __grid_constant__ CUtensorMap tmA, const __grid_constant__ CUtensorMap tmB,
                int M, int N, int K, float alpha, float beta, TC* __restrict__ C, long ldc,
                const float* __restrict__ bias, int relu, int kb_per_split, int tiles_m, int tiles_n, int splits,
-               int row_unperm_h, const __grid_constant__ LstmEpi le) {
+               int row_unperm_h, const __grid_constant__ TcEpiParam<EPI> le) {
   constexpr bool LSTM = (EPI == 1 || EPI == 5);
   constexpr bool LSTM_DROP = (EPI == 1);
+  constexpr bool CELL = (EPI == 6 || EPI == 7);
+  constexpr bool CELL_DROP = (EPI == 6);
   using Cfg = TcCfg<BN>;
   constexpr int TC_STAGES = Cfg::STAGES;
   extern __shared__ unsigned char smem_dyn[];
@@ -251,6 +268,13 @@
   const int tiles_mn = tiles_m * tiles_n;
   const int total = tiles_mn * splits;
   const bool split = splits > 1;
+  auto item = [&](int w, int& sp, int& rem) {
+    if constexpr (CELL) { sp = w % CELL_SPLITS; rem = w / CELL_SPLITS; } else { sp = w / tiles_mn; rem = w - sp * tiles_mn; }
+  };
+  auto krange = [&](int sp, int& kb_begin, int& kb_end) {
+    if constexpr (CELL) { kb_begin = sp * num_kb_total / CELL_SPLITS; kb_end = (sp + 1) * num_kb_total / CELL_SPLITS; }
+    else { kb_begin = sp * kb_per_split; kb_end = min(num_kb_total, kb_begin + kb_per_split); }
+  };
 
   pdl_launch_dependents();
   if (warp == 0 && lane == 0) { tma_prefetch_desc(&tmA); tma_prefetch_desc(&tmB); }
@@ -274,9 +298,9 @@
     if (lane == 0) {
       int it = 0;
       for (int w = blockIdx.x; w < total; w += gridDim.x) {
-        const int sp = w / tiles_mn, rem = w - sp * tiles_mn;
+        int sp, rem, kb_begin, kb_end;
+        item(w, sp, rem); krange(sp, kb_begin, kb_end);
         const int m0 = (rem / tiles_n) * TC_BM, n0 = (rem % tiles_n) * BN;
-        const int kb_begin = sp * kb_per_split, kb_end = min(num_kb_total, kb_begin + kb_per_split);
         for (int kb = kb_begin; kb < kb_end; ++kb, ++it) {
           const int s = it % TC_STAGES; const uint32_t ph = (it / TC_STAGES) & 1;
           mbar_wait(&empty_bar[s], ph ^ 1);
@@ -305,8 +329,8 @@
                                  ((uint32_t)(BN >> 3) << 17) | ((uint32_t)(TC_BM >> 4) << 24);
       int it = 0, t = 0;
       for (int w = blockIdx.x; w < total; w += gridDim.x, ++t) {
-        const int sp = w / tiles_mn;
-        const int kb_begin = sp * kb_per_split, kb_end = min(num_kb_total, kb_begin + kb_per_split);
+        int sp, rem, kb_begin, kb_end;
+        item(w, sp, rem); krange(sp, kb_begin, kb_end);
         const int as = t & 1; const uint32_t aph = (t >> 1) & 1;
         mbar_wait(&tempty_bar[as], aph ^ 1);
         tc_fence_after();
@@ -327,6 +351,108 @@
         }
         tc_commit(&tfull_bar[as]);
       }
+    }
+  } else if constexpr (CELL) {
+    constexpr int TPR = BN / 4, RPP = TC_EPI_WARPS * 32 / TPR, NPASS = 32 / RPP;
+    constexpr int RP = BN + 4;
+    static_assert((size_t)CELL_SPLITS * 32 * RP * 4 <= (size_t)TC_STAGES * Cfg::STAGE_BYTES, "receive area must fit in the TMA ring");
+    float* recv = reinterpret_cast<float*>(base);
+    const uint32_t rank = cr_cluster_rank();
+    const int rem = blockIdx.x / CELL_SPLITS;
+    const int m0 = (rem / tiles_n) * TC_BM, n0 = (rem % tiles_n) * BN;
+    const bool adj = n0 < le.n_adj;
+    const int H = le.H, et = threadIdx.x - 64, uc = (et % TPR) * 4, rl0 = (int)rank * 32 + et / TPR;
+    constexpr int NPF = NPASS < 3 ? NPASS : 3;
+    struct Pass { uint4 g0, g1; float4 tc, cp, dhf, dc; };
+    auto fetch = [&](int p, Pass& v) {
+      const long row = m0 + rl0 + p * RPP, u = n0 + uc;
+      const uint4* gp = reinterpret_cast<const uint4*>(le.gates + row * 4 * H + 4 * u);
+      v.g0 = gp[0]; v.g1 = gp[1];
+      v.tc = *reinterpret_cast<const float4*>(le.c_cur + row * H + u);
+      v.cp = *reinterpret_cast<const float4*>(le.c_prev + row * H + u);
+      float4 d = make_float4(0.f, 0.f, 0.f, 0.f);
+      if (le.dh_ext) d = *reinterpret_cast<const float4*>(le.dh_ext + row * H + u);
+      if (le.dh_hid) {
+        const uint2 hh = *reinterpret_cast<const uint2*>(le.dh_hid + row * H + u);
+        d.x += bf16_lo(hh.x); d.y += bf16_hi(hh.x); d.z += bf16_lo(hh.y); d.w += bf16_hi(hh.y);
+      }
+      if (le.carry) {
+        const float4 c4 = __ldcg(reinterpret_cast<const float4*>(le.carry + row * le.ld_carry + u));
+        d.x += c4.x; d.y += c4.y; d.z += c4.z; d.w += c4.w;
+      }
+      v.dhf = d;
+      v.dc = le.dc_is_zero ? make_float4(0.f, 0.f, 0.f, 0.f) : __ldcg(reinterpret_cast<const float4*>(le.dc + row * H + u));
+      v.tc = make_float4(Math<bf16>::tanh_(v.tc.x), Math<bf16>::tanh_(v.tc.y), Math<bf16>::tanh_(v.tc.z), Math<bf16>::tanh_(v.tc.w));
+    };
+    Pass pf[NPF];
+    [[maybe_unused]] uint32_t keep = 0;
+    [[maybe_unused]] const float inv_keep = CELL_DROP ? 1.0f / (1.0f - le.drop_p) : 1.0f;
+    if (adj) {
+#pragma unroll
+      for (int p = 0; p < NPF; ++p) fetch(p, pf[p]);
+      if constexpr (CELL_DROP) {
+        const uint64_t dseed = drop_seed(le.seed, le.seed_dev);
+#pragma unroll
+        for (int p = 0; p < NPASS; ++p)
+#pragma unroll
+          for (int j = 0; j < 4; ++j)
+            if (dropout_scale(dseed, le.site, (uint64_t)((le.row_base + m0 + rl0 + p * RPP) * H + n0 + uc + j), le.drop_p, 1.0f) != 0.f) keep |= 1u << (4 * p + j);
+      }
+    }
+    mbar_wait(&tfull_bar[0], 0);
+    tc_fence_after();
+    cr_cluster_sync();
+    {
+      const int q = warp & 3, half = (warp - 2) >> 2;
+      const uint32_t tacc = tmem_base + ((uint32_t)(q * 32) << 16);
+      const uint32_t dst = cr_mapa(smem_u32(recv + ((size_t)rank * 32 + lane) * RP), (uint32_t)q);
+#pragma unroll
+      for (int c = 0; c < BN / 64; ++c) {
+        const int col = half * (BN / 2) + c * 32;
+        float v[32];
+        tmem_ld32(tacc + (uint32_t)col, v);
+#pragma unroll
+        for (int j = 0; j < 8; ++j)
+          asm volatile("st.shared::cluster.v4.f32 [%0], {%1, %2, %3, %4};" :: "r"(dst + (uint32_t)(col + 4 * j) * 4u),
+                       "f"(v[4 * j]), "f"(v[4 * j + 1]), "f"(v[4 * j + 2]), "f"(v[4 * j + 3]) : "memory");
+      }
+    }
+    cr_cluster_sync();
+#pragma unroll
+    for (int p = 0; p < NPASS; ++p) {
+      const int rl = et / TPR + p * RPP;
+      const long row = m0 + (int)rank * 32 + rl, u = n0 + uc;
+      float4 a = *reinterpret_cast<const float4*>(recv + (size_t)rl * RP + uc);
+#pragma unroll
+      for (int src = 1; src < CELL_SPLITS; ++src) {
+        const float4 b4 = *reinterpret_cast<const float4*>(recv + ((size_t)src * 32 + rl) * RP + uc);
+        a.x += b4.x; a.y += b4.y; a.z += b4.z; a.w += b4.w;
+      }
+      if (!adj) {
+        *reinterpret_cast<float4*>(C + row * ldc + u) = a;
+        continue;
+      }
+      if constexpr (CELL_DROP) {
+        a.x *= (keep >> (4 * p)) & 1 ? inv_keep : 0.f; a.y *= (keep >> (4 * p + 1)) & 1 ? inv_keep : 0.f;
+        a.z *= (keep >> (4 * p + 2)) & 1 ? inv_keep : 0.f; a.w *= (keep >> (4 * p + 3)) & 1 ? inv_keep : 0.f;
+      }
+      Pass v;
+      if (p < NPF) v = pf[p < NPF ? p : 0]; else fetch(p, v);
+      const float dh[4] = {a.x + v.dhf.x, a.y + v.dhf.y, a.z + v.dhf.z, a.w + v.dhf.w};
+      const float tc[4] = {v.tc.x, v.tc.y, v.tc.z, v.tc.w}, cp[4] = {v.cp.x, v.cp.y, v.cp.z, v.cp.w};
+      const float dci[4] = {v.dc.x, v.dc.y, v.dc.z, v.dc.w};
+      const uint32_t gw[8] = {v.g0.x, v.g0.y, v.g0.z, v.g0.w, v.g1.x, v.g1.y, v.g1.z, v.g1.w};
+      uint32_t ow[8]; float dco[4];
+#pragma unroll
+      for (int k = 0; k < 4; ++k) {
+        const float gt[4] = {bf16_lo(gw[2 * k]), bf16_hi(gw[2 * k]), bf16_lo(gw[2 * k + 1]), bf16_hi(gw[2 * k + 1])};
+        float dg[4];
+        lstm_cell_adjoint(dh[k], gt, tc[k], cp[k], dci[k], dg, dco[k]);
+        ow[2 * k] = pack_bf16(dg[0], dg[1]); ow[2 * k + 1] = pack_bf16(dg[2], dg[3]);
+      }
+      uint4* gp = reinterpret_cast<uint4*>(le.dgates + row * 4 * H + 4 * u);
+      gp[0] = make_uint4(ow[0], ow[1], ow[2], ow[3]); gp[1] = make_uint4(ow[4], ow[5], ow[6], ow[7]);
+      *reinterpret_cast<float4*>(le.dc + row * H + u) = make_float4(dco[0], dco[1], dco[2], dco[3]);
     }
   } else {
     const int q = warp & 3;
@@ -685,6 +811,9 @@
     }
     }
   }
+  if constexpr (CELL) {
+    if (warp < 2) { __syncwarp(); cr_cluster_sync(); cr_cluster_sync(); }
+  }
   tc_fence_before();
   __syncthreads();
   if (warp == 1) {
@@ -846,6 +975,62 @@
   return launch_tc_major<64, TC>(g, plan, st);
 }
 
+template <int BN> int cell_bwd_max_clusters() {
+  static int n = -1;
+  if (n >= 0) return n;
+  n = 0;
+  void (*kern)(const CUtensorMap, const CUtensorMap, int, int, int, float, float, float*, long, const float*, int, int, int, int, int, int, const CellBwdEpi) =
+      gemm_tc_kernel<BN, false, true, float, 7>;
+  if (cudaFuncSetAttribute(kern, cudaFuncAttributeMaxDynamicSharedMemorySize, (int)TcCfg<BN>::SMEM_BYTES) != cudaSuccess) { cudaGetLastError(); return n; }
+  cudaLaunchConfig_t cfg{};
+  cfg.gridDim = dim3(CELL_SPLITS * 64); cfg.blockDim = dim3(TC_THREADS); cfg.dynamicSmemBytes = TcCfg<BN>::SMEM_BYTES;
+  cudaLaunchAttribute at[1];
+  at[0].id = cudaLaunchAttributeClusterDimension; at[0].val.clusterDim.x = CELL_SPLITS; at[0].val.clusterDim.y = 1; at[0].val.clusterDim.z = 1;
+  cfg.attrs = at; cfg.numAttrs = 1;
+  int m = 0;
+  if (cudaOccupancyMaxActiveClusters(&m, kern, &cfg) != cudaSuccess) { cudaGetLastError(); return n; }
+  n = m;
+  if (getenv("B2C_CELL_BWD_INFO")) fprintf(stderr, "b2c: cell-adjoint GEMM BN=%d: %d co-resident clusters of %d CTAs (%zu B of shared memory each)\n", BN, n, CELL_SPLITS, TcCfg<BN>::SMEM_BYTES);
+  return n;
+}
+inline int cell_bwd_plan(int M, int N, int K, int n_adj) {
+  if (M % TC_BM != 0 || cdiv(K, TC_BK) < CELL_SPLITS) return 0;
+  for (int bn : {64, 128}) {
+    if (N % bn != 0 || n_adj % bn != 0) continue;
+    const long clusters = (long)(M / TC_BM) * (N / bn);
+    const int mx = bn == 64 ? cell_bwd_max_clusters<64>() : cell_bwd_max_clusters<128>();
+    if (clusters * CELL_SPLITS <= gemm_sms() && clusters <= mx) return bn;
+  }
+  return 0;
+}
+template <int BN>
+int launch_cell_bwd(const GemmArgs& g, const CellBwdEpi& e, cudaStream_t st) {
+  CUtensorMap ta, tb;
+  B2C_TRY(make_tmap_bf16(&ta, g.A, g.K, g.M, g.lda, TC_BM));
+  B2C_TRY(make_tmap_bf16(&tb, g.B, g.N, g.K, g.ldb, 64));
+  const bool drop = e.drop_p > 0.f;
+  void (*kern)(const CUtensorMap, const CUtensorMap, int, int, int, float, float, float*, long, const float*, int, int, int, int, int, int, const CellBwdEpi) =
+      drop ? gemm_tc_kernel<BN, false, true, float, 6> : gemm_tc_kernel<BN, false, true, float, 7>;
+  static bool attr_set[2] = {false, false};
+  if (!attr_set[drop]) {
+    B2C_CUDA(cudaFuncSetAttribute(kern, cudaFuncAttributeMaxDynamicSharedMemorySize, (int)TcCfg<BN>::SMEM_BYTES));
+    attr_set[drop] = true;
+  }
+  const int tiles_m = g.M / TC_BM, tiles_n = g.N / BN;
+  B2C_CUDA(launch_pdl_cluster(kern, dim3(tiles_m * tiles_n * CELL_SPLITS), dim3(TC_THREADS), TcCfg<BN>::SMEM_BYTES, st, CELL_SPLITS, ta, tb,
+                              g.M, g.N, g.K, 1.f, 0.f, (float*)g.C, g.ldc, (const float*)nullptr, 0, 0, tiles_m, tiles_n, CELL_SPLITS, 0, e));
+  B2C_LAUNCH_CHECK("gemm_tc_kernel");
+  return 0;
+}
+inline int gemm_cell_bwd(const GemmArgs& g, const CellBwdEpi& e, cudaStream_t st) {
+  const int bn = cell_bwd_plan(g.M, g.N, g.K, e.n_adj);
+  auto a16 = [](const void* p) { return ((uintptr_t)p & 15) == 0; };
+  B2C_CHECK_ARG(bn != 0 && tc_eligible(g) && !g.a_mn && g.b_mn, "cell-adjoint GEMM: shape or operands outside its plan (M=%d N=%d K=%d n_adj=%d)", g.M, g.N, g.K, e.n_adj);
+  B2C_CHECK_ARG(a16(e.gates) && a16(e.c_prev) && a16(e.c_cur) && a16(e.dc) && a16(e.dgates) && a16(e.carry) && e.ld_carry % 4 == 0 && a16(e.dh_ext) &&
+                ((uintptr_t)e.dh_hid & 7) == 0 && (e.n_adj == g.N || (a16(g.C) && g.ldc % 4 == 0)), "cell-adjoint GEMM: misaligned operand");
+  return bn == 64 ? launch_cell_bwd<64>(g, e, st) : launch_cell_bwd<128>(g, e, st);
+}
+
 template <typename TA, typename TB, typename TC>
 int gemm_simt(const GemmArgs& g, cudaStream_t st) {
   dim3 grid(cdiv(g.N, SG_BN), cdiv(g.M, SG_BM));
diff --git a/imagecaptioner_b200/csrc/recur_cluster.cuh b/imagecaptioner_b200/csrc/recur_cluster.cuh
--- a/imagecaptioner_b200/csrc/recur_cluster.cuh
+++ b/imagecaptioner_b200/csrc/recur_cluster.cuh
@@ -47,9 +47,6 @@
 };
 struct ClusterMaps { CUtensorMap w0, w1, wh, h0, h1, ctx; };
 
-__device__ __forceinline__ uint32_t cr_cluster_rank() { uint32_t r; asm volatile("mov.u32 %0, %%cluster_ctarank;" : "=r"(r)); return r; }
-__device__ __forceinline__ void cr_cluster_sync() { asm volatile("barrier.cluster.arrive.release.aligned;\n\tbarrier.cluster.wait.acquire.aligned;" ::: "memory"); }
-__device__ __forceinline__ uint32_t cr_mapa(uint32_t addr, uint32_t rank) { uint32_t r; asm volatile("mapa.shared::cluster.u32 %0, %1, %2;" : "=r"(r) : "r"(addr), "r"(rank)); return r; }
 __device__ __forceinline__ void cr_tma_mc(void* dst, const CUtensorMap* map, int c0, int c1, uint64_t* bar, uint16_t mask) {
   asm volatile("cp.async.bulk.tensor.2d.shared::cluster.global.mbarrier::complete_tx::bytes.multicast::cluster [%0], [%1, {%4, %5}], [%2], %3;"
                :: "r"(smem_u32(dst)), "l"(map), "r"(smem_u32(bar)), "h"(mask), "r"(c0), "r"(c1) : "memory");
```

Result: no change. 207,400 (median of 6 runs) (-0.4%).
